# lars-uav/lars-image-processing

Measured on AMD Instinct MI355X. Metric: Mpixels/sec NDVI+stats on 4096x4096 RGNir tiles; achieved HBM GB/s, higher is better.
Workload: dtype f32

## Files before the change

include/lars_hip.h:

```cpp
#ifndef LARS_HIP_H
#define LARS_HIP_H

#include <stddef.h>
#include <stdint.h>

#ifdef __cplusplus
extern "C" {
#endif

#define LARS_ABI_VERSION 1
#define LARS_HIST_BINS 50

typedef enum lars_status {
    LARS_OK = 0,
    LARS_ERR_INVALID = -1,
    LARS_ERR_NO_DEVICE = -2,
    LARS_ERR_HIP = -3,
    LARS_ERR_OOM = -4,
    LARS_ERR_RCCL = -5,
    LARS_ERR_UNSUPPORTED = -6
} lars_status;

#define LARS_U8  1
#define LARS_U16 2

#define LARS_NDVI  0
#define LARS_GNDVI 1
#define LARS_NDWI  2
#define LARS_MASK_NDVI  1u
#define LARS_MASK_GNDVI 2u
#define LARS_MASK_NDWI  4u
#define LARS_MASK_ALL   7u

#define LARS_F_STATS 1u
#define LARS_F_HIST  2u
#define LARS_F_SUMSQ 4u
#define LARS_F_RAW   8u

typedef struct lars_stats {
    double   sum;
    double   sumsq;
    uint64_t count;
    uint64_t above;
    uint64_t nans;
    double   min;
    double   max;
    double   threshold;
    uint32_t index_id;
    uint32_t reserved;
    uint64_t hist[LARS_HIST_BINS];
} lars_stats;

int         lars_abi_version(void);
const char *lars_last_error(void);
int         lars_device_count(int *count);
int         lars_set_device(int ordinal);
int         lars_get_device(int *ordinal);
int         lars_device_name(char *buf, size_t buflen);
int         lars_malloc(void **dptr, size_t bytes);
int         lars_free(void *dptr);
int         lars_memset(void *dptr, int value, size_t bytes, void *stream);
int         lars_memcpy_h2d(void *dst_dev, const void *src_host, size_t bytes);
int         lars_memcpy_d2h(void *dst_host, const void *src_dev, size_t bytes);
int         lars_memcpy_d2d(void *dst_dev, const void *src_dev, size_t bytes, void *stream);
int         lars_stream_create(void **stream);
int         lars_stream_destroy(void *stream);
int         lars_synchronize(void *stream);
int         lars_mem_info(size_t *free_bytes, size_t *total_bytes);
int         lars_shutdown(void);
int         lars_event_create(void **event);
int         lars_event_destroy(void *event);
int         lars_event_record(void *event, void *stream);
int         lars_event_elapsed_ms(void *start, void *stop, float *ms);
int         lars_stream_wait_event(void *stream, void *event);


int lars_d_channel_hist(const void *tiles, int64_t ntiles, int64_t npix, int channels,
                        int dtype, uint32_t *hist, void *stream);

int lars_d_wb_table(const uint32_t *hist, int64_t ntiles, int64_t npix, int dtype,
                    uint8_t *table, double *percentiles, int rgn_variant, void *stream);

size_t lars_wb_table_bytes(int dtype);

int lars_d_wb_prepare(const void *tiles, int64_t ntiles, int64_t npix, int channels, int dtype,
                      uint8_t *table, double *percentiles, int rgn_variant, void *stream);
int lars_u16_window_report(int64_t ntiles, uint32_t *flags, uint32_t *windows);

typedef struct lars_fused_args {
    const void    *tiles;
    int64_t        ntiles;
    int64_t        npix;
    int32_t        channels;
    int32_t        dtype;
    const uint8_t *wb_table;
    uint32_t       index_mask;
    uint32_t       flags;
    float         *out_index[3];
    uint8_t       *out_wb;
    uint8_t       *out_rgba[3];
    const uint8_t *cmap_lut[3];
    lars_stats    *stats;
    void          *stream;
} lars_fused_args;

int lars_d_fused(const lars_fused_args *args);
int lars_d_stats_begin(lars_stats *stats, int64_t ntiles, uint32_t index_mask, void *stream);
int lars_d_stats_end(lars_stats *stats, int64_t ntiles, uint32_t index_mask, int64_t npix, void *stream);

int lars_d_index_planes_f32(const float *red, const float *green, const float *nir,
                            int64_t n, int index_id, float *out, void *stream);

int lars_d_ndvi_f64(const void *img, int64_t npix, int channels, int dtype,
                    double *out, void *stream);

int lars_d_array_stats_f32(const float *x, int64_t n, float threshold, int want_hist,
                           lars_stats *out_dev, void *stream);
int lars_d_array_stats_f64(const double *x, int64_t n, double threshold, int want_hist,
                           lars_stats *out_dev, double *out_sumsqdev_dev, void *stream);

size_t lars_select_scratch_bytes(void);
int lars_d_median_pair_f32(const float *x, int64_t n, float *out_dev, void *scratch, void *stream);
int lars_d_median_pair_f64(const double *x, int64_t n, double *out_dev, void *scratch, void *stream);
int lars_d_median_pair_batch_f32(const float *x, int64_t n, int64_t items, int64_t stride, float *out_dev,
                                 void *scratch, void *stream);

int lars_d_quotient_select_hist(const void *tiles, int64_t ntiles, int64_t npix, int channels, int dtype,
                                const uint8_t *wb_table, uint32_t streams , int first,
                                const uint32_t bucket[4], uint64_t *hist, void *stream);
size_t lars_quotient_median_scratch_bytes(int64_t ntiles);
int lars_d_stats_medians(const lars_fused_args *a, float *out_pairs, void *scratch);
int lars_d_quotient_median_pairs(const void *tiles, int64_t ntiles, int64_t npix, int channels, int dtype,
                                 const uint8_t *wb_table, uint32_t streams ,
                                 float *out_pairs, void *scratch, void *stream);

size_t lars_joint_scratch_bytes(int64_t ntiles, int64_t npix, uint32_t index_mask);
int lars_d_stats_joint(const lars_fused_args *a, int white_balance, int rgn_variant, double *percentiles, uint32_t *hist,
                       float *out_pairs, void *scratch, size_t scratch_bytes);
int lars_joint_window_report(const void *scratch, int64_t ntiles, int64_t *windowed, int64_t *recounted);
int lars_joint_window_modes(const void *scratch, int64_t ntiles, int64_t counts[3]);

int lars_d_threshold_mask_f32(const float *x, int64_t n, float threshold, uint8_t *out_mask, void *stream);

int lars_d_colormap_f32(const float *x, int64_t n, const uint8_t *lut_rgba, uint8_t *out_rgba,
                        void *stream);
int lars_d_colormap_entry_f32(const float *x, int64_t n, uint8_t *out_entry, void *stream);

int lars_d_gray_c128(const uint8_t *img, int64_t npix, int channels, double *out_c128, void *stream);
size_t lars_phase_scratch_bytes(void);
int lars_d_phase_correlation(double *fixed_c128, double *moving_c128, int64_t h, int64_t w, int64_t *shift_dev,
                             void *scratch, void *stream);
int lars_d_shift_reflect_u8(const uint8_t *img, int64_t h, int64_t w, int channels, const int64_t *shift_dev,
                            uint8_t *out, void *stream);
int lars_d_diff_f32(const float *early, const float *late, int64_t n, float *out_diff, void *stream);
int lars_d_colormap_norm_f32(const float *x, int64_t n, float vmin, float vmax, const uint8_t *lut_rgba,
                             uint8_t *out_rgba, void *stream);

int lars_d_synth_u8(uint8_t *tiles, int64_t ntiles, int64_t first_tile, int64_t npix, int channels,
                    uint32_t seed, int profile, void *stream);

int lars_set_tuning(const char *key, int value);
int lars_get_tuning(const char *key, int *value);

#define LARS_BUILD_LAB_LAYOUT 1u
#define LARS_BUILD_IEEE_DIV 2u
#define LARS_BUILD_COUNT_MODE 4u
#define LARS_BUILD_STATS_GEOMETRY 8u
unsigned int lars_build_flags(void);

int lars_d_quot_selfcheck(uint32_t max_den, uint64_t *mismatches, uint32_t first_bad[2]);

int lars_stats_merge(const lars_stats *records, int64_t n, lars_stats *out);
int lars_d_stats_fold(const lars_stats *tile_records, int64_t ntiles, uint32_t index_mask, lars_stats *out, void *stream);


int lars_h_fix_white_balance(const void *img, int64_t h, int64_t w, int channels, int dtype,
                             int variant, uint8_t *out, double *percentiles );
int lars_h_fix_white_balance_f32(const float *img, int64_t h, int64_t w, int channels, uint8_t *out,
                                 double *percentiles );

int lars_h_calculate_index(const void *img, int64_t h, int64_t w, int channels, int dtype,
                           uint32_t index_mask, float *const out[3],
                           lars_stats *stats , int want_hist);

int lars_h_calculate_index_planes(const float *red, const float *green, const float *nir,
                                  int64_t n, int index_id, float *out);

int lars_h_ndvi_f64(const void *img, int64_t h, int64_t w, int channels, int dtype, double *out);

int lars_h_analyze_f32(const float *x, int64_t n, float threshold, int want_hist,
                       lars_stats *out, float median_pair[2]);
int lars_h_analyze_f64(const double *x, int64_t n, double threshold, int want_hist,
                       lars_stats *out, double median_pair[2], double *sumsqdev);

int lars_h_process_image(const void *img, int64_t h, int64_t w, int channels, int dtype,
                         int apply_wb, uint32_t index_mask, int want_hist,
                         uint8_t *out_wb, float *const out_index[3],
                         lars_stats *stats , float *medians ,
                         uint8_t *const out_rgba[3], const uint8_t *const cmap_lut[3]);

int lars_h_colormap_f32(const float *x, int64_t n, const uint8_t *lut_rgba, uint8_t *out_rgba);
int lars_h_threshold_mask_f32(const float *x, int64_t n, float threshold, uint8_t *out_mask);

int lars_h_resize_lanczos_u8(const uint8_t *img, int64_t h, int64_t w, int channels, int64_t new_h, int64_t new_w,
                             uint8_t *out);
int lars_h_thumbnail_u8(const uint8_t *img, int64_t h, int64_t w, int channels, int fx, int fy, const int reduce_box[4],
                        const float box[4], int64_t new_h, int64_t new_w, int vertical_first, uint8_t *out);

int lars_h_align_images(const uint8_t *fixed, const uint8_t *moving, int64_t h, int64_t w, int channels,
                        uint8_t *out_aligned, double shift[2]);
int lars_h_change_detection(const uint8_t *early, const uint8_t *late, int64_t h, int64_t w, int channels,
                            int wb_early, int wb_late, int align, int index_id,
                            float *out_early, float *out_late, float *out_diff,
                            uint8_t *out_rgba_diff, const uint8_t *lut_rgba, float vmin, float vmax,
                            uint8_t *out_aligned_late, double shift[2]);
int lars_h_colormap_norm_f32(const float *x, int64_t n, float vmin, float vmax, const uint8_t *lut_rgba,
                             uint8_t *out_rgba);

size_t lars_png_bound(int64_t h, int64_t w, int channels);
size_t lars_png_scratch_bytes(int64_t h, int64_t w, int channels);
int lars_d_encode_png_u8(const uint8_t *img, int64_t h, int64_t w, int channels, const uint8_t *palette_rgba, int palette_len,
                         uint8_t *out, size_t out_cap, int64_t *out_len_dev, void *scratch, void *stream);
int lars_h_encode_png_u8(const uint8_t *img, int64_t h, int64_t w, int channels, const uint8_t *palette_rgba, int palette_len,
                         uint8_t *out, size_t out_cap, int64_t *out_len);
int lars_h_process_image_png(const void *img, int64_t h, int64_t w, int channels, int dtype,
                             int apply_wb, uint32_t index_mask, int want_hist,
                             uint8_t *out_wb, float *const out_index[3],
                             lars_stats *stats , float *medians ,
                             const uint8_t *const cmap_lut[3], int png_mode,
                             uint8_t *const out_png[3], size_t png_cap, int64_t png_len[3]);

#define LARS_PNG_INFO_N 10
enum {
    LARS_PNG_INFO_WIDTH = 0,
    LARS_PNG_INFO_HEIGHT = 1,
    LARS_PNG_INFO_BIT_DEPTH = 2,
    LARS_PNG_INFO_COLOR_TYPE = 3,
    LARS_PNG_INFO_INTERLACE = 4,
    LARS_PNG_INFO_CHANNELS = 5,
    LARS_PNG_INFO_IDAT_BYTES = 6,
    LARS_PNG_INFO_IDAT_COUNT = 7,
    LARS_PNG_INFO_APNG = 8,
    LARS_PNG_INFO_SUPPORTED = 9
};
enum {
    LARS_PNGD_OK = 0,
    LARS_PNGD_CRC = 1,
    LARS_PNGD_ZLIB_HEADER = 2,
    LARS_PNGD_DEFLATE = 3,
    LARS_PNGD_FAR = 4,
    LARS_PNGD_SHORT = 5,
    LARS_PNGD_ADLER = 6,
    LARS_PNGD_FILTER = 7,
    LARS_PNGD_INTERNAL = 8
};
int lars_png_info(const uint8_t *file, int64_t len, int64_t info[LARS_PNG_INFO_N], int64_t *idat_table, int64_t idat_cap);
size_t lars_png_decode_scratch_bytes(int64_t h, int64_t w, int channels, int64_t idat_bytes, int64_t idat_count);
int lars_d_decode_png_u8(const uint8_t *file, const int64_t *idat_table, int64_t idat_count, int64_t idat_bytes, int64_t h,
                         int64_t w, int channels, uint8_t *out, int32_t *status_dev, void *scratch, void *stream);
int lars_h_decode_png_u8(const uint8_t *file, int64_t len, uint8_t *out, size_t out_cap);
int lars_h_thumbnail_png_u8(const uint8_t *file, int64_t len, int fx, int fy, const int reduce_box[4], const float box[4],
// ... 408 lines not shown
```

lars_image_processing_amd/_ffi.py:

```python
from __future__ import annotations

import contextlib
import ctypes as C
import os
import threading
from typing import NamedTuple

import numpy as np

_HERE = os.path.dirname(os.path.abspath(__file__))
LIB_PATH = os.environ.get("LARS_HIP_LIB", os.path.join(_HERE, "liblars_hip.so"))

HIST_BINS = 50
U8, U16 = 1, 2
NDVI, GNDVI, NDWI = 0, 1, 2
INDEX_IDS = {"NDVI": NDVI, "GNDVI": GNDVI, "NDWI": NDWI}
INDEX_NAMES = ("NDVI", "GNDVI", "NDWI")
F_STATS, F_HIST, F_SUMSQ, F_RAW = 1, 2, 4, 8
COMM_ID_BYTES = 128


class LarsError(RuntimeError):

    def __init__(self, code, message):
        super().__init__(f"liblars_hip error {code}: {message}")
        self.code = code


class Stats(C.Structure):
    _fields_ = [
        ("sum", C.c_double), ("sumsq", C.c_double),
        ("count", C.c_uint64), ("above", C.c_uint64), ("nans", C.c_uint64),
        ("min", C.c_double), ("max", C.c_double), ("threshold", C.c_double),
        ("index_id", C.c_uint32), ("reserved", C.c_uint32),
        ("hist", C.c_uint64 * HIST_BINS),
    ]


STATS_DTYPE = np.dtype([
    ("sum", "<f8"), ("sumsq", "<f8"), ("count", "<u8"), ("above", "<u8"), ("nans", "<u8"),
    ("min", "<f8"), ("max", "<f8"), ("threshold", "<f8"), ("index_id", "<u4"), ("reserved", "<u4"),
    ("hist", "<u8", (HIST_BINS,)),
])
assert STATS_DTYPE.itemsize == C.sizeof(Stats) == 472

REGION_DTYPE = np.dtype([("area", "<i8"), ("bbox", "<i4", (4,)), ("row_sum", "<u8"), ("col_sum", "<u8")])
assert REGION_DTYPE.itemsize == 40

RING_DTYPE = np.dtype([("label", "<i4"), ("key", "<i4"), ("start", "<i4"), ("count", "<i4"), ("area2", "<i8")])
assert RING_DTYPE.itemsize == 24


class Outlines(C.Structure):
    _fields_ = [
        ("rings", C.c_void_p), ("ring_capacity", C.c_int64), ("verts", C.c_void_p), ("vert_capacity", C.c_int64),
        ("n_rings", C.c_int64), ("n_vertices", C.c_int64), ("n_edges", C.c_int64),
    ]


class FusedArgs(C.Structure):
    _fields_ = [
        ("tiles", C.c_void_p), ("ntiles", C.c_int64), ("npix", C.c_int64),
        ("channels", C.c_int32), ("dtype", C.c_int32),
        ("wb_table", C.c_void_p), ("index_mask", C.c_uint32), ("flags", C.c_uint32),
        ("out_index", C.c_void_p * 3), ("out_wb", C.c_void_p),
        ("out_rgba", C.c_void_p * 3), ("cmap_lut", C.c_void_p * 3),
        ("stats", C.c_void_p), ("stream", C.c_void_p),
    ]


class PngInfo(NamedTuple):
    width: int
    height: int
    bit_depth: int
    color_type: int
    interlace: int
    channels: int
    idat_bytes: int
    idat_count: int
    apng: int
    supported: int

    @classmethod
    def array(cls):
        return (C.c_int64 * len(cls._fields))()


class JpegInfo(NamedTuple):
    width: int
    height: int
    components: int
    frame: int
    precision: int
    h0: int
    v0: int
    h1: int
    v1: int
    h2: int
    v2: int
    restart_interval: int
    entropy_offset: int
    entropy_bytes: int
    supported: int
    reason: int

    @classmethod
    def array(cls):
        return (C.c_int64 * len(cls._fields))()

    @property
    def sampling(self):
        return ((self.h0, self.v0), (self.h1, self.v1), (self.h2, self.v2))


class TiffInfo(NamedTuple):
    width: int
    height: int
    samples: int
    bits: int
    compression: int
    predictor: int
    planar: int
    big_endian: int
    photometric: int
    extra_samples: int
    tiled: int
    chunk_w: int
    chunk_h: int
    chunks: int
    supported: int
    reason: int

    @classmethod
    def array(cls):
        return (C.c_int64 * len(cls._fields))()


_P, _I, _I64, _U32, _SZ, _F, _D = C.c_void_p, C.c_int, C.c_int64, C.c_uint32, C.c_size_t, C.c_float, C.c_double
SIGNATURES = {
    "lars_abi_version": (_I, []),
    "lars_last_error": (C.c_char_p, []),
    "lars_device_count": (_I, [C.POINTER(_I)]),
    "lars_set_device": (_I, [_I]),
    "lars_get_device": (_I, [C.POINTER(_I)]),
    "lars_device_name": (_I, [C.c_char_p, _SZ]),
    "lars_malloc": (_I, [C.POINTER(_P), _SZ]),
    "lars_free": (_I, [_P]),
    "lars_memset": (_I, [_P, _I, _SZ, _P]),
    "lars_memcpy_h2d": (_I, [_P, _P, _SZ]),
    "lars_memcpy_d2h": (_I, [_P, _P, _SZ]),
    "lars_memcpy_d2d": (_I, [_P, _P, _SZ, _P]),
    "lars_stream_create": (_I, [C.POINTER(_P)]),
    "lars_stream_destroy": (_I, [_P]),
    "lars_synchronize": (_I, [_P]),
    "lars_shutdown": (_I, []),
    "lars_mem_info": (_I, [C.POINTER(_SZ), C.POINTER(_SZ)]),
    "lars_event_create": (_I, [C.POINTER(_P)]),
    "lars_event_destroy": (_I, [_P]),
    "lars_event_record": (_I, [_P, _P]),
    "lars_event_elapsed_ms": (_I, [_P, _P, C.POINTER(_F)]),
    "lars_stream_wait_event": (_I, [_P, _P]),
    "lars_d_channel_hist": (_I, [_P, _I64, _I64, _I, _I, _P, _P]),
    "lars_d_wb_table": (_I, [_P, _I64, _I64, _I, _P, _P, _I, _P]),
    "lars_wb_table_bytes": (_SZ, [_I]),
    "lars_d_wb_prepare": (_I, [_P, _I64, _I64, _I, _I, _P, _P, _I, _P]),
    "lars_u16_window_report": (_I, [_I64, _P, _P]),
    "lars_d_fused": (_I, [C.POINTER(FusedArgs)]),
    "lars_d_stats_begin": (_I, [_P, _I64, _U32, _P]),
    "lars_d_stats_end": (_I, [_P, _I64, _U32, _I64, _P]),
    "lars_d_index_planes_f32": (_I, [_P, _P, _P, _I64, _I, _P, _P]),
    "lars_d_ndvi_f64": (_I, [_P, _I64, _I, _I, _P, _P]),
    "lars_d_array_stats_f32": (_I, [_P, _I64, _F, _I, _P, _P]),
    "lars_d_array_stats_f64": (_I, [_P, _I64, _D, _I, _P, _P, _P]),
    "lars_select_scratch_bytes": (_SZ, []),
    "lars_d_median_pair_f32": (_I, [_P, _I64, _P, _P, _P]),
    "lars_d_median_pair_f64": (_I, [_P, _I64, _P, _P, _P]),
    "lars_d_median_pair_batch_f32": (_I, [_P, _I64, _I64, _I64, _P, _P, _P]),
    "lars_d_colormap_f32": (_I, [_P, _I64, _P, _P, _P]),
    "lars_d_colormap_entry_f32": (_I, [_P, _I64, _P, _P]),
    "lars_quotient_median_scratch_bytes": (_SZ, [_I64]),
    "lars_d_stats_medians": (_I, [C.POINTER(FusedArgs), _P, _P]),
    "lars_d_quotient_median_pairs": (_I, [_P, _I64, _I64, _I, _I, _P, _U32, _P, _P, _P]),
    "lars_joint_scratch_bytes": (_SZ, [_I64, _I64, _U32]),
    "lars_d_stats_joint": (_I, [C.POINTER(FusedArgs), _I, _I, _P, _P, _P, _P, _SZ]),
    "lars_joint_window_report": (_I, [_P, _I64, C.POINTER(_I64), C.POINTER(_I64)]),
    "lars_joint_window_modes": (_I, [_P, _I64, C.POINTER(_I64)]),
    "lars_h_tiff_lzw_decode": (_I, [_P, _I64, _P, _I64, C.POINTER(_I64)]),
    "lars_h_tiff_lzw_decode_chunks": (_I, [_P, _I64, _P, _P, _I64, _P, _I64, _P, _I]),
    "lars_d_quotient_select_hist": (_I, [_P, _I64, _I64, _I, _I, _P, _U32, _I, _P, _P, _P]),
    "lars_d_synth_u8": (_I, [_P, _I64, _I64, _I64, _I, _U32, _I, _P]),
    "lars_stats_merge": (_I, [_P, _I64, _P]),
    "lars_d_stats_fold": (_I, [_P, _I64, _U32, _P, _P]),
    "lars_build_flags": (C.c_uint, []),
    "lars_set_tuning": (_I, [C.c_char_p, _I]),
    "lars_get_tuning": (_I, [C.c_char_p, C.POINTER(_I)]),
    "lars_d_quot_selfcheck": (_I, [_U32, C.POINTER(C.c_uint64), C.POINTER(_U32 * 2)]),
    "lars_h_fix_white_balance": (_I, [_P, _I64, _I64, _I, _I, _I, _P, _P]),
    "lars_h_fix_white_balance_f32": (_I, [_P, _I64, _I64, _I, _P, _P]),
    "lars_h_calculate_index": (_I, [_P, _I64, _I64, _I, _I, _U32, C.POINTER(_P * 3), _P, _I]),
    "lars_h_calculate_index_planes": (_I, [_P, _P, _P, _I64, _I, _P]),
    "lars_h_ndvi_f64": (_I, [_P, _I64, _I64, _I, _I, _P]),
    "lars_h_analyze_f32": (_I, [_P, _I64, _F, _I, _P, _P]),
    "lars_h_analyze_f64": (_I, [_P, _I64, _D, _I, _P, _P, _P]),
    "lars_h_process_image": (_I, [_P, _I64, _I64, _I, _I, _I, _U32, _I, _P, C.POINTER(_P * 3), _P, _P,
                                  C.POINTER(_P * 3), C.POINTER(_P * 3)]),
    "lars_h_colormap_f32": (_I, [_P, _I64, _P, _P]),
    "lars_h_threshold_mask_f32": (_I, [_P, _I64, _F, _P]),
    "lars_d_threshold_mask_f32": (_I, [_P, _I64, _F, _P, _P]),
    "lars_h_colormap_norm_f32": (_I, [_P, _I64, _F, _F, _P, _P]),
    "lars_h_align_images": (_I, [_P, _P, _I64, _I64, _I, _P, _P]),
    "lars_h_change_detection": (_I, [_P, _P, _I64, _I64, _I, _I, _I, _I, _I, _P, _P, _P, _P, _P, _F, _F, _P, _P]),
    "lars_d_gray_c128": (_I, [_P, _I64, _I, _P, _P]),
    "lars_phase_scratch_bytes": (_SZ, []),
    "lars_d_phase_correlation": (_I, [_P, _P, _I64, _I64, _P, _P, _P]),
    "lars_d_shift_reflect_u8": (_I, [_P, _I64, _I64, _I, _P, _P, _P]),
    "lars_d_diff_f32": (_I, [_P, _P, _I64, _P, _P]),
    "lars_d_colormap_norm_f32": (_I, [_P, _I64, _F, _F, _P, _P, _P]),
    "lars_h_resize_lanczos_u8": (_I, [_P, _I64, _I64, _I, _I64, _I64, _P]),
    "lars_h_thumbnail_u8": (_I, [_P, _I64, _I64, _I, _I, _I, C.POINTER(_I), C.POINTER(_F), _I64, _I64, _I, _P]),
    "lars_png_bound": (_SZ, [_I64, _I64, _I]),
    "lars_png_scratch_bytes": (_SZ, [_I64, _I64, _I]),
    "lars_d_encode_png_u8": (_I, [_P, _I64, _I64, _I, _P, _I, _P, _SZ, _P, _P, _P]),
    "lars_h_encode_png_u8": (_I, [_P, _I64, _I64, _I, _P, _I, _P, _SZ, C.POINTER(_I64)]),
    "lars_h_process_image_png": (_I, [_P, _I64, _I64, _I, _I, _I, _U32, _I, _P, C.POINTER(_P * 3), _P, _P,
                                      C.POINTER(_P * 3), _I, C.POINTER(_P * 3), _SZ, _P]),
    "lars_png_info": (_I, [_P, _I64, _P, _P, _I64]),
    "lars_png_decode_scratch_bytes": (_SZ, [_I64, _I64, _I, _I64, _I64]),
    "lars_d_decode_png_u8": (_I, [_P, _P, _I64, _I64, _I64, _I64, _I, _P, _P, _P, _P]),
    "lars_h_decode_png_u8": (_I, [_P, _I64, _P, _SZ]),
    "lars_h_thumbnail_png_u8": (_I, [_P, _I64, _I, _I, C.POINTER(_I), C.POINTER(_F), _I64, _I64, _I, _P]),
    "lars_png_out_format": (_I, [_I, _I, C.POINTER(_I), C.POINTER(_I)]),
    "lars_png_layout": (_I, [_I64, _I64, _I, _I, _I, _P, C.POINTER(_I64), C.POINTER(_I64)]),
    "lars_png_decode_ex_scratch_bytes": (_SZ, [_I64, _I64, _I, _I, _I, _I64, _I64]),
    "lars_d_decode_png_ex": (_I, [_P, _P, _I64, _I64, _I64, _I64, _I, _I, _I, _P, _P, _P, _P]),
    "lars_h_decode_png_ex": (_I, [_P, _I64, _P, _SZ]),
    "lars_h_thumbnail_png_ex": (_I, [_P, _I64, _I, _I, C.POINTER(_I), C.POINTER(_F), _I64, _I64, _I, _P]),
    "lars_jpeg_info": (_I, [_P, _I64, _P]),
    "lars_jpeg_decode_scratch_bytes": (_SZ, [_P]),
    "lars_d_decode_jpeg_u8": (_I, [_P, _P, _P, _P, _P, _P, _P]),
    "lars_h_decode_jpeg_u8": (_I, [_P, _I64, _P, _SZ]),
    "lars_h_thumbnail_jpeg_u8": (_I, [_P, _I64, _I, _I, C.POINTER(_I), C.POINTER(_F), _I64, _I64, _I, _P]),
    "lars_jpeg_decode_scaled_scratch_bytes": (_SZ, [_P, _I]),
    "lars_d_decode_jpeg_scaled_u8": (_I, [_P, _P, _P, _I, _P, _P, _P, _P]),
    "lars_h_decode_jpeg_scaled_u8": (_I, [_P, _I64, _I, _P, _SZ]),
    "lars_h_thumbnail_jpeg_scaled_u8": (_I, [_P, _I64, _I, _I, _I, C.POINTER(_I), C.POINTER(_F), _I64, _I64, _I, _P]),
    "lars_tiff_info": (_I, [_P, _I64, _P, _P, _I64]),
    "lars_h_decode_tiff": (_I, [_P, _I64, _P, _SZ]),
    "lars_h_thumbnail_tiff_u8": (_I, [_P, _I64, _I, _I, C.POINTER(_I), C.POINTER(_F), _I64, _I64, _I, _P]),
    "lars_tiff_info_deflate": (_I, [_P, _I64, _P, _P, _I64]),
    "lars_h_decode_tiff_deflate": (_I, [_P, _I64, _P, _SZ]),
    "lars_h_thumbnail_tiff_deflate_u8": (_I, [_P, _I64, _I, _I, C.POINTER(_I), C.POINTER(_F), _I64, _I64, _I, _P]),
    "lars_tiff_bound": (_SZ, [_I64, _I64, _I, _I, _I64]),
    "lars_tiff_encode_scratch_bytes": (_SZ, [_I64, _I64, _I, _I, _I64]),
    "lars_d_encode_tiff": (_I, [_P, _I64, _I64, _I, _I, _I64, _I, _P, _SZ, _P, _P, _P, _P]),
    "lars_h_encode_tiff": (_I, [_P, _I64, _I64, _I, _I, _I64, _I, _P, _SZ, C.POINTER(_I64)]),
    "lars_tiff_f32_bound": (_SZ, [_I64, _I64, _I, _I64]),
    "lars_tiff_f32_encode_scratch_bytes": (_SZ, [_I64, _I64, _I, _I64]),
    "lars_d_encode_tiff_f32": (_I, [_P, _I64, _I64, _I, _I64, _I, _P, _SZ, _P, _P, _P, _P]),
    "lars_h_encode_tiff_f32": (_I, [_P, _I64, _I64, _I, _I64, _I, _P, _SZ, C.POINTER(_I64)]),
    "lars_h_process_image_tiff_f32": (_I, [_P, _I64, _I64, _I, _I, _I, _U32, _I, _P, C.POINTER(_P * 3), _P, _P,
                                           C.POINTER(_P * 3), C.POINTER(_P * 3), _I, _I64, C.POINTER(_P * 3), _SZ, _P]),
    "lars_tiff_deflate_bound": (_SZ, [_I64, _I64, _I, _I, _I64]),
    "lars_tiff_deflate_encode_scratch_bytes": (_SZ, [_I64, _I64, _I, _I, _I64]),
    "lars_d_encode_tiff_deflate": (_I, [_P, _I64, _I64, _I, _I, _I64, _I, _P, _SZ, _P, _P, _P, _P]),
    "lars_h_encode_tiff_deflate": (_I, [_P, _I64, _I64, _I, _I, _I64, _I, _P, _SZ, C.POINTER(_I64)]),
    "lars_tiff_float32_deflate_bound": (_SZ, [_I64, _I64, _I, _I64]),
    "lars_tiff_float32_deflate_encode_scratch_bytes": (_SZ, [_I64, _I64, _I, _I64]),
    "lars_d_encode_tiff_deflate_float32": (_I, [_P, _I64, _I64, _I, _I64, _I, _P, _SZ, _P, _P, _P, _P]),
    "lars_h_encode_tiff_deflate_float32": (_I, [_P, _I64, _I64, _I, _I64, _I, _P, _SZ, C.POINTER(_I64)]),
    "lars_h_process_image_tiff_float32": (_I, [_P, _I64, _I64, _I, _I, _I, _U32, _I, _P, C.POINTER(_P * 3), _P, _P,
                                                       C.POINTER(_P * 3), C.POINTER(_P * 3), _I, _I, _I64, C.POINTER(_P * 3), _SZ, _P]),
    "lars_d_valid_mask": (_I, [_P, _I64, _I, _I, _P, _I, _I, _I, _P, _P, _P]),
    "lars_d_masked_channel_hist": (_I, [_P, _I64, _I, _I, _P, _P, _P]),
    "lars_d_masked_fused": (_I, [C.POINTER(FusedArgs), _P, C.POINTER(_P * 3), _P]),
    "lars_h_valid_mask": (_I, [_P, _I64, _I64, _I, _I, _I, _I, _I, _P, C.POINTER(_I64)]),
    "lars_h_process_image_masked": (_I, [_P, _I64, _I64, _I, _I, _I, _U32, _I, _P, C.POINTER(_P * 3), _P, _P,
                                         C.POINTER(_P * 3), C.POINTER(_P * 3), _P, _I, _I, _I, C.POINTER(_I64),
                                         _I, _I, _I64, C.POINTER(_P * 3), _SZ, _P]),
    "lars_d_zone_count": (_I, [_P, _I, _P, _I64, _I64, _P, _P, _P]),
    "lars_d_zone_offsets": (_I, [_P, _I64, _P, _P, _P]),
    "lars_d_zone_scatter": (_I, [C.POINTER(_P * 3), _U32, _P, _I, _P, _I64, _I64, _P, _P, C.POINTER(_P * 3), _P]),
    "lars_d_zone_stats": (_I, [_P, _P, _P, _I64, _F, _I, _I64, _P, _P, _P]),
    "lars_h_zonal_stats_f32": (_I, [_P, _P, _I, _P, _I64, _I64, _I64, _F, _I, _P, _P, C.POINTER(_I64)]),
    "lars_h_process_image_zones": (_I, [_P, _I64, _I64, _I, _I, _I, _U32, _I, _P, C.POINTER(_P * 3), _P, _P,
                                        C.POINTER(_P * 3), C.POINTER(_P * 3), _P, _I, _I, _I, C.POINTER(_I64),
                                        _P, _I, _I64, _P, _P, C.POINTER(_I64)]),
    "lars_zone_rasterize_scratch_bytes": (_SZ, [_I64]),
    "lars_d_zone_rasterize": (_I, [_P, _I64, _P, _I64, _P, _I64, _I64, _I64, _P, _P, _P]),
    "lars_d_zone_labels_narrow": (_I, [_P, _I64, _I, _P, _P]),
    "lars_h_rasterize_zones": (_I, [_P, _I64, _P, _I64, _P, _I64, _I64, _I64, _I, _P]),
    "lars_h_zonal_stats_polygons_f32": (_I, [_P, _P, _I64, _P, _I64, _P, _I64, _P, _I64, _I64, _F, _I, _P, _P, _P, _I]),
    "lars_h_process_image_zones_polygons": (_I, [_P, _I64, _I64, _I, _I, _I, _U32, _I, _P, C.POINTER(_P * 3), _P, _P,
                                                 C.POINTER(_P * 3), C.POINTER(_P * 3), _P, _I, _I, _I, C.POINTER(_I64),
                                                 _P, _I64, _P, _I64, _P, _I64, _P, _P, _P, _I]),
    "lars_region_label_scratch_bytes": (_SZ, [_I64, _I64]),
    "lars_d_region_label": (_I, [_P, _I64, _I64, _I, _I64, _P, _P, _I64, _P, _P, _P]),
    "lars_d_region_mask_f32": (_I, [_P, _P, _P, _I64, _F, _I, _P, _P]),
    "lars_h_label_regions": (_I, [_P, _I64, _I64, _I, _I64, _I, _P, C.POINTER(_I), _P, _I64, C.POINTER(_I64)]),
    "lars_h_zonal_stats_regions_f32": (_I, [_P, _P, _I, _F, _I, _I64, _P, _I64, _I64, _F, _I, _I64, _P, _P, _P, C.POINTER(_I64), _P, _I,
                                            C.POINTER(_I)]),
    "lars_h_process_image_regions": (_I, [_P, _I64, _I64, _I, _I, _I, _U32, _I, _P, C.POINTER(_P * 3), _P, _P,
                                          C.POINTER(_P * 3), C.POINTER(_P * 3), _P, _I, _I, _I, C.POINTER(_I64),
                                          _P, _I, _I, _F, _I, _I64, _I64, _P, _P, _P, C.POINTER(_I64), _P, _I, C.POINTER(_I)]),
    "lars_region_outline_scratch_bytes": (_SZ, [_I64, _I64, _I64]),
    "lars_d_region_outline_count": (_I, [_P, _I64, _I64, _P, _P]),
    "lars_d_region_outline": (_I, [_P, _I64, _I64, _I, _I64, _I64, _P, _I64, _P, _I64, _P, _P, _P]),
    "lars_h_region_outlines": (_I, [_P, _I64, _I64, _I, _I64, _I, _P, C.POINTER(_I), _P, _I64, C.POINTER(_I64), C.POINTER(Outlines)]),
    "lars_h_zonal_stats_regions_outlines_f32": (_I, [_P, _P, _I, _F, _I, _I64, _P, _I64, _I64, _F, _I, _I64, _P, _P, _P, C.POINTER(_I64), _P, _I,
                                                     C.POINTER(_I), C.POINTER(Outlines)]),
    "lars_h_process_image_regions_outlines": (_I, [_P, _I64, _I64, _I, _I, _I, _U32, _I, _P, C.POINTER(_P * 3), _P, _P,
                                                   C.POINTER(_P * 3), C.POINTER(_P * 3), _P, _I, _I, _I, C.POINTER(_I64),
                                                   _P, _I, _I, _F, _I, _I64, _I64, _P, _P, _P, C.POINTER(_I64), _P, _I, C.POINTER(_I),
                                                   C.POINTER(Outlines)]),
    "lars_d_zone_shrink": (_I, [_P, _I, _I64, _I64, _I64, _P, _P, _P]),
    "lars_h_shrink_zones": (_I, [_P, _I, _I64, _I64, _I64, _I64, _P, C.POINTER(_I64)]),
    "lars_h_rasterize_zones_margin": (_I, [_P, _I64, _P, _I64, _P, _I64, _I64, _I64, _I, _P, _I64]),
    "lars_h_zonal_stats_margin_f32": (_I, [_P, _P, _I, _P, _I64, _I64, _I64, _F, _I, _P, _P, C.POINTER(_I64), _I64]),
    "lars_h_zonal_stats_polygons_margin_f32": (_I, [_P, _P, _I64, _P, _I64, _P, _I64, _P, _I64, _I64, _F, _I, _P, _P, _P, _I, _I64]),
    "lars_h_zonal_stats_regions_margin_f32": (_I, [_P, _P, _I, _F, _I, _I64, _P, _I64, _I64, _F, _I, _I64, _P, _P, _P, C.POINTER(_I64), _P, _I,
                                                   C.POINTER(_I), _I64]),
    "lars_h_process_image_zones_margin": (_I, [_P, _I64, _I64, _I, _I, _I, _U32, _I, _P, C.POINTER(_P * 3), _P, _P,
                                               C.POINTER(_P * 3), C.POINTER(_P * 3), _P, _I, _I, _I, C.POINTER(_I64),
# ... 183 lines not shown
```

lars_image_processing_amd/batch.py:

```python
from __future__ import annotations

import ctypes as C
import os

import numpy as np

from . import _ffi
from . import arena as _arena
from ._ffi import FusedArgs, INDEX_IDS, INDEX_NAMES, STATS_DTYPE, DeviceBuffer, DeviceSlice
from .arena import arena_placements

MAX_TILES_PER_LAUNCH = 65535


_STATS_ROUTE = os.environ.get("LARS_STATS_ROUTE", "auto")


def set_stats_route(route):
    global _STATS_ROUTE
    if route not in ("auto", "joint", "classic"):
        raise ValueError("route must be auto, joint or classic")
    _STATS_ROUTE = route


def get_stats_route():
    return _STATS_ROUTE


def index_mask(indices):
    mask = 0
    for t in indices:
        mask |= 1 << INDEX_IDS[t]
    return mask


def joint_serves(code, channels, ntiles, npix):
    return code == _ffi.U8 and channels in (3, 4) and (ntiles == 1 or npix % 4 == 0)


def plan_process(code, channels, ntiles, npix, indices, white_balance, hist, medians, sumsq, route,
                 outputs=False, wb_plane=False, reuse=False):
    if route not in ("auto", "joint", "classic"):
        raise ValueError(f"route must be auto, joint or classic, not {route!r}")
    if reuse and not outputs and route == "joint":
        raise ValueError("route='joint' derives the tables from its own counts: it cannot honour recompute_tables=False")
    one_read = route != "classic" and not reuse and joint_serves(code, channels, ntiles, npix) and bool(indices)
    if one_read and not outputs:
        return "measure" if route == "auto" and not medians and not sumsq else "one-read"
    if route == "joint" and not outputs:
        raise ValueError("route='joint' serves uint8 tiles with 3 or 4 channels (4-byte aligned) only")
    if one_read and not wb_plane and (medians or hist or select_streams(indices) in (1, 2)):
        return "one-read+planes"
    if medians and code == _ffi.U8 and channels == 3 and npix * 6 < (1 << 30) and (ntiles == 1 or npix % 4 == 0):
        return "select" if not outputs and index_mask(indices) in (1, 2, 4, 7) else "per-pixel+select"
    return "per-pixel+radix" if medians else "per-pixel"


def channels_of(indices, whole_image=False):
    if whole_image:
        return {0, 1, 2}
    need = set()
    for t in indices:
        need |= {2, 0} if t == "NDVI" else {2, 1}
    return need


def shard_range(ntiles, rank, world):
    base, rem = divmod(int(ntiles), int(world))
    start = rank * base + min(rank, rem)
    return start, start + base + (1 if rank < rem else 0)


class TileBatch:

    def __init__(self, ntiles, h, w, channels=3, dtype=np.uint8, first_tile=0):
        self.ntiles, self.h, self.w, self.channels = int(ntiles), int(h), int(w), int(channels)
        self.dtype = np.dtype(dtype)
        self.code = _ffi.dtype_code(self.dtype)
        if self.code is None:
            raise TypeError("tiles must be uint8 or uint16")
        if self.ntiles < 1 or self.ntiles > MAX_TILES_PER_LAUNCH:
            raise ValueError(f"1 <= ntiles <= {MAX_TILES_PER_LAUNCH} per batch")
        self.first_tile = int(first_tile)
        self.npix = self.h * self.w
        self.nvalues = 256 if self.code == _ffi.U8 else 65536
        self.table_bytes = int(_ffi.load().lars_wb_table_bytes(self.code))
        self.tile_bytes = self.npix * self.channels * self.dtype.itemsize
        self.tiles = DeviceBuffer(self.ntiles * self.tile_bytes)
        self.hist = None
        self.table = None
        self.percentiles = None
        self._table_channels = set()
        self._hist_channels = set()
        self._rgn_variant = 0
        self._joint_scratch = None
        self._joint_tiles = self.ntiles
        self._selq = None
        self.last_route = None

    @classmethod
    def from_host(cls, array, first_tile=0):
        arr = np.ascontiguousarray(array)
        if arr.ndim != 4 or arr.shape[3] < 3:
            raise ValueError("expected [ntiles, H, W, C>=3]")
        b = cls(arr.shape[0], arr.shape[1], arr.shape[2], arr.shape[3], arr.dtype, first_tile)
        b.tiles.upload(arr)
        return b

    @classmethod
    def synthetic(cls, ntiles, h, w, seed=1234, profile="uniform", first_tile=0, channels=3):
        b = cls(ntiles, h, w, channels, np.uint8, first_tile)
        _ffi.call("lars_d_synth_u8", C.c_void_p(b.tiles.ptr), b.ntiles, b.first_tile, b.npix, b.channels,
                  int(seed) & 0xFFFFFFFF, {"uniform": 0, "vegetation": 1}[profile], None)
        _ffi.call("lars_synchronize", None)
        return b

    def host_tiles(self, start=0, count=None):
        count = self.ntiles - start if count is None else count
        return self.tiles.download(self.dtype, (count, self.h, self.w, self.channels), start * self.tile_bytes)

    def compute_wb_tables(self, stream=None, rgn_variant=0):
        if self.table is None:
            self.table = DeviceBuffer(self.ntiles * self.table_bytes)
            self.percentiles = DeviceBuffer(self.ntiles * 3 * 2 * 8)
        if self.code == _ffi.U8:
            if self.hist is None:
                self.hist = DeviceBuffer(self.ntiles * 3 * 256 * 4)
            _ffi.call("lars_d_channel_hist", C.c_void_p(self.tiles.ptr), self.ntiles, self.npix, self.channels,
                      self.code, C.c_void_p(self.hist.ptr), stream)
            _ffi.call("lars_d_wb_table", C.c_void_p(self.hist.ptr), self.ntiles, self.npix, self.code,
                      C.c_void_p(self.table.ptr), C.c_void_p(self.percentiles.ptr), int(rgn_variant), stream)
        else:
            _ffi.call("lars_d_wb_prepare", C.c_void_p(self.tiles.ptr), self.ntiles, self.npix, self.channels,
                      self.code, C.c_void_p(self.table.ptr), C.c_void_p(self.percentiles.ptr), int(rgn_variant), stream)
        self._table_channels = {0, 1, 2}
        self._hist_channels = {0, 1, 2} if self.code == _ffi.U8 else set()
        self._rgn_variant = int(rgn_variant)
        return self

    def u16_window_report(self):
        if self.code != _ffi.U16:
            raise _ffi.LarsError(-1, "lars_u16_window_report: a uint8 batch's pre-pass does not take the value-window route")
        flags = np.zeros(self.ntiles, np.uint32)
        windows = np.zeros((self.ntiles, 3, 4), np.uint32)
        _ffi.call("lars_u16_window_report", self.ntiles, _ffi.ptr(flags), _ffi.ptr(windows))
        return flags, windows

    def _need_channels(self, partial):
        if self.table is None:
            raise RuntimeError("compute_wb_tables() first")
        if not partial and self._table_channels != {0, 1, 2}:
            missing = sorted({0, 1, 2} - self._table_channels)
            raise RuntimeError(f"white-balance tables of channel(s) {missing} are not valid: the last pass computed only the "
                               f"channels its indices read (compute_wb_tables() for all three, or partial=True)")

    def host_tables(self, partial=False):
        self._need_channels(partial)
        blob = self.table.download(np.uint8, (self.ntiles, self.table_bytes))
        return np.ascontiguousarray(blob[:, :3 * self.nvalues]).reshape(self.ntiles, 3, self.nvalues)

    def host_percentiles(self, partial=False):
        self._need_channels(partial)
        return self.percentiles.download(np.float64, (self.ntiles, 3, 2))

    def host_hist(self, partial=False):
        self._need_channels(partial)
        if self.hist is None or (not partial and self._hist_channels != {0, 1, 2}):
            missing = sorted({0, 1, 2} - self._hist_channels)
            raise RuntimeError(f"channel histograms of channel(s) {missing} are not valid: the last one-read pass was not asked for them "
                               f"(compute_wb_tables(), or run_joint(..., channel_hist=True); partial=True hands out what there is)")
        return self.hist.download(np.uint32, (self.ntiles, 3, 256))

    def make_outputs(self, indices=INDEX_NAMES, index=False, wb=False, rgba=False, ring=None, placement_trials=None, arena="auto",
                     pick="fastest"):
        outs = BatchOutputs(self, indices, index, wb, rgba, ring, allocate=False)
        nplanes = len(outs._index_ids) + len(outs._rgba_ids)
        plan = _arena.plan_arena(nplanes, outs.plane_bytes, outs.slots * self.npix * 4, arena, placement_trials, pick)
        if plan.kind != "search":
            if plan.kind == "packed":
                outs.adopt_arena(DeviceBuffer(nplanes * outs.plane_bytes))
            outs.arena_report = _arena.unsearched_report(plan)
            return outs

        def free_bytes():
            free_b, total_b = C.c_size_t(), C.c_size_t()
            _ffi.call("lars_mem_info", C.byref(free_b), C.byref(total_b))
            return free_b.value

        stats = self.new_stats()
        try:
            found = _arena.search(outs, plan, pick, alloc=DeviceBuffer, free_bytes=free_bytes,
                                  probe=lambda placement, warm_ms: self._probe_arena(outs, indices, stats, warm_ms),
                                  synchronize=lambda: _ffi.call("lars_synchronize", None))
        finally:
            stats.free()
        outs.placement_ms, outs.arena_report = _arena.report(found)
        return outs

    def _probe_arena(self, outs, indices, stats, warm_ms=_arena.ARENA_WARM_MS):
        count = min(outs.slots, self.ntiles)
        starts = list(range(0, self.ntiles, count))
        if len(starts) > 16:
            starts = [starts[int(round(i * (len(starts) - 1) / 15.0))] for i in range(16)]
        mask = index_mask(indices)
        wb_on = self.table is not None
        launches = [self.fused_args(indices, wb_on, stats, False, outs, None, st, min(count, self.ntiles - st), raw=True) for st in starts]
        while len(launches) < 4:
            launches = launches + launches
        ev = [C.c_void_p(), C.c_void_p()]
        for e in ev:
            _ffi.call("lars_event_create", C.byref(e))
        ms = C.c_float(0)

        def one_pass():
            _ffi.call("lars_event_record", ev[0], None)
            for a in launches:
                self.run_fused(a)
            _ffi.call("lars_event_record", ev[1], None)
            _ffi.call("lars_event_elapsed_ms", ev[0], ev[1], C.byref(ms))
            return float(ms.value)

        try:
            _ffi.call("lars_d_stats_begin", C.c_void_p(stats.ptr), self.ntiles, mask, None)
            warmed, passes = 0.0, 0
            while warmed < warm_ms and passes < 8:
                warmed += one_pass()
                passes += 1
            timed = one_pass()
            _ffi.call("lars_d_stats_end", C.c_void_p(stats.ptr), self.ntiles, mask, self.npix, None)
            _ffi.call("lars_synchronize", None)
        finally:
            for e in ev:
                _ffi.call("lars_event_destroy", e)
        return timed / len(launches)

    def fused_args(self, indices=INDEX_NAMES, white_balance=True, stats=None, hist=False, outputs=None,
                   stream=None, tile_start=0, tile_count=None, sumsq=False, raw=False):
        tile_count = self.ntiles - tile_start if tile_count is None else tile_count
        a = FusedArgs()
        a.tiles = self.tiles.ptr + tile_start * self.tile_bytes
        a.ntiles, a.npix, a.channels, a.dtype = tile_count, self.npix, self.channels, self.code
        if white_balance:
            if self.table is None:
                raise RuntimeError("compute_wb_tables() first")
            a.wb_table = self.table.ptr + tile_start * self.table_bytes
        a.index_mask = index_mask(indices)
        a.flags = ((_ffi.F_STATS if stats is not None else 0) | (_ffi.F_HIST if (stats is not None and hist) else 0) |
                   (_ffi.F_SUMSQ if (stats is not None and sumsq) else 0) | (_ffi.F_RAW if (stats is not None and raw) else 0))
        if stats is not None:
            a.stats = stats.ptr + tile_start * 3 * STATS_DTYPE.itemsize
        if outputs is not None:
            slot = tile_start % outputs.slots
            if slot + tile_count > outputs.slots:
                raise ValueError("tile range wraps the output ring")
            for k in range(3):
                if outputs.index[k] is not None:
                    a.out_index[k] = outputs.index[k].ptr + slot * self.npix * 4
                if outputs.rgba[k] is not None:
                    a.out_rgba[k] = outputs.rgba[k].ptr + slot * self.npix * 4
                    a.cmap_lut[k] = outputs.luts[k].ptr
            if outputs.wb is not None:
                a.out_wb = outputs.wb.ptr + slot * self.npix * self.channels
        a.stream = stream
        return a

    def new_stats(self):
        return DeviceBuffer(self.ntiles * 3 * STATS_DTYPE.itemsize)

    def fold_stats(self, stats, indices=INDEX_NAMES, out=None, stream=None):
        if out is None:
            out = DeviceBuffer(3 * STATS_DTYPE.itemsize)
            out.zero(stream)
        _ffi.call("lars_d_stats_fold", C.c_void_p(stats.ptr), self.ntiles, index_mask(indices), C.c_void_p(out.ptr), stream)
        return out

    def run_fused_chunks(self, indices, white_balance, stats, hist, outputs, stream=None, sumsq=False, launch_events=None):
        chunk = self.ntiles if outputs is None else outputs.slots
        if chunk >= self.ntiles:
            if launch_events:
                _ffi.call("lars_event_record", launch_events[0], stream)
            self.run_fused(self.fused_args(indices, white_balance, stats, hist, outputs, stream, sumsq=sumsq))
            if launch_events and len(launch_events) > 1:
                _ffi.call("lars_event_record", launch_events[1], stream)
            return 1
        mask = index_mask(indices)
        if stats is not None:
            _ffi.call("lars_d_stats_begin", C.c_void_p(stats.ptr), self.ntiles, mask, stream)
        launches = 0
        if launch_events:
            _ffi.call("lars_event_record", launch_events[0], stream)
        for start in range(0, self.ntiles, chunk):
            count = min(chunk, self.ntiles - start)
            self.run_fused(self.fused_args(indices, white_balance, stats, hist, outputs, stream, start, count, sumsq=sumsq,
                                           raw=stats is not None))
            launches += 1
            if launch_events and launches < len(launch_events):
                _ffi.call("lars_event_record", launch_events[launches], stream)
        if stats is not None:
            _ffi.call("lars_d_stats_end", C.c_void_p(stats.ptr), self.ntiles, mask, self.npix, stream)
        return launches

    def run_fused(self, args):
        _ffi.call("lars_d_fused", C.byref(args))

    def can_joint(self):
        return joint_serves(self.code, self.channels, self.ntiles, self.npix)

    def run_joint(self, indices, white_balance, stats, hist=False, sumsq=False, pairs=None, stream=None, rgn_variant=0,
                  tile_count=None, channel_hist=False):
        mask = index_mask(indices)
        need = int(_ffi.load().lars_joint_scratch_bytes(self.ntiles, self.npix, mask))
        if self._joint_scratch is None or self._joint_scratch.nbytes < need:
            if self._joint_scratch is not None:
                _ffi.call("lars_synchronize", stream)
                self._joint_scratch.free()
            self._joint_scratch = DeviceBuffer(need)
        if white_balance:
            if self.table is None:
                self.table = DeviceBuffer(self.ntiles * self.table_bytes)
                self.percentiles = DeviceBuffer(self.ntiles * 3 * 2 * 8)
                self.table.zero(stream)
                self.percentiles.zero(stream)
            if channel_hist and self.hist is None:
                self.hist = DeviceBuffer(self.ntiles * 3 * 256 * 4)
                self.hist.zero(stream)
                self._hist_channels = set()
            if tile_count is None or int(tile_count) == self.ntiles:
                keep = self._table_channels if int(rgn_variant) == self._rgn_variant else set()
                self._table_channels = keep | channels_of(indices)
                self._rgn_variant = int(rgn_variant)
                if channel_hist:
                    self._hist_channels = self._hist_channels | channels_of(indices)
            else:
                self._table_channels = set()
                self._hist_channels = set()
        a = FusedArgs()
        a.tiles = self.tiles.ptr
        a.ntiles, a.npix, a.channels, a.dtype = (self.ntiles if tile_count is None else int(tile_count)), self.npix, self.channels, self.code
        a.wb_table = self.table.ptr if white_balance else None
        a.index_mask = mask
        a.flags = _ffi.F_STATS | (_ffi.F_HIST if hist else 0) | (_ffi.F_SUMSQ if sumsq else 0)
        a.stats = stats.ptr
        a.stream = stream
        self._joint_tiles = int(a.ntiles)
        _ffi.call("lars_d_stats_joint", C.byref(a), 1 if white_balance else 0, int(rgn_variant),
                  C.c_void_p(self.percentiles.ptr) if white_balance else None,
                  C.c_void_p(self.hist.ptr) if white_balance and channel_hist else None,
                  C.c_void_p(pairs.ptr) if pairs is not None else None, C.c_void_p(self._joint_scratch.ptr), self._joint_scratch.nbytes)

    def joint_window_report(self):
        w, r = C.c_int64(0), C.c_int64(0)
        if self._joint_scratch is None:
            return 0, 0
        _ffi.call("lars_joint_window_report", C.c_void_p(self._joint_scratch.ptr), self._joint_tiles, C.byref(w), C.byref(r))
        return int(w.value), int(r.value)

    def joint_window_modes(self):
        if self._joint_scratch is None:
            return 0, 0, 0
        counts = (C.c_int64 * 3)()
        _ffi.call("lars_joint_window_modes", C.c_void_p(self._joint_scratch.ptr), self._joint_tiles, counts)
        return int(counts[0]), int(counts[1]), int(counts[2])

    def check_joint(self, stream=None):
        _ffi.call("lars_synchronize", stream)
        if self._joint_scratch is not None and int(self._joint_scratch.download(np.uint32, (1,))[0]):
            raise RuntimeError("lars_d_stats_joint: a workgroup's hand-over list overflowed (a chunk of more than 2^24 pixels?)")

    def pick_stats_route(self, indices, white_balance=True, sample=256, min_pixels=1 << 29):
        key = (tuple(sorted(INDEX_IDS[t] for t in indices)), bool(white_balance))
        cache = self.__dict__.setdefault("_route_cache", {})
        if key in cache:
            return cache[key]
        sample = min(int(sample), self.ntiles)
        if sample * self.npix < int(min_pixels) or self.channels != 3:
            cache[key] = "joint"
            return "joint"
        saved = (self.table, self.percentiles, self.hist, set(self._table_channels), self._rgn_variant, set(self._hist_channels))
        self.table = self.percentiles = self.hist = None
        self._table_channels = set()
        self._hist_channels = set()
        ev = [C.c_void_p() for _ in range(3)]
        for e in ev:
            _ffi.call("lars_event_create", C.byref(e))
        stats = self.new_stats()
        ms = {}
        try:
            for _ in range(2):
                _ffi.call("lars_event_record", ev[0], None)
                self.run_joint(indices, white_balance, stats, tile_count=sample)
                _ffi.call("lars_event_record", ev[1], None)
                if white_balance:
                    if self.hist is None:
                        self.hist = DeviceBuffer(self.ntiles * 3 * 256 * 4)
                    _ffi.call("lars_d_channel_hist", C.c_void_p(self.tiles.ptr), sample, self.npix, self.channels, self.code,
                              C.c_void_p(self.hist.ptr), None)
                    _ffi.call("lars_d_wb_table", C.c_void_p(self.hist.ptr), sample, self.npix, self.code, C.c_void_p(self.table.ptr),
                              C.c_void_p(self.percentiles.ptr), 0, None)
                self.run_fused(self.fused_args(indices, white_balance, stats, False, None, None, 0, sample))
                _ffi.call("lars_event_record", ev[2], None)
                t = C.c_float(0)
                _ffi.call("lars_event_elapsed_ms", ev[0], ev[1], C.byref(t)); ms["joint"] = t.value
                _ffi.call("lars_event_elapsed_ms", ev[1], ev[2], C.byref(t)); ms["classic"] = t.value
            self.check_joint()
        finally:
            _ffi.call("lars_synchronize", None)
            for e in ev:
                _ffi.call("lars_event_destroy", e)
            stats.free()
            for buf in (self.table, self.percentiles, self.hist):
                if buf is not None:
                    buf.free()
            self.table, self.percentiles, self.hist, self._table_channels, self._rgn_variant, self._hist_channels = saved
        cache[key] = "joint" if ms["joint"] <= ms["classic"] else "classic"
        self._route_ms = dict(ms)
        return cache[key]

    def process(self, indices=INDEX_NAMES, white_balance=True, hist=False, outputs=None, stream=None,
                recompute_tables=True, medians=False, sumsq=False, route=None, rgn_variant=None, channel_hist=False):
        route = _STATS_ROUTE if route is None else route
        variant = 0 if rgn_variant is None else int(rgn_variant)
        wb_plane = outputs is not None and outputs.wb is not None
        reuse = (white_balance and not recompute_tables and self.table is not None
                 and channels_of(indices, wb_plane) <= self._table_channels and (rgn_variant is None or variant == self._rgn_variant))

        def plan(r):
            return plan_process(self.code, self.channels, self.ntiles, self.npix, indices, white_balance, hist, medians, sumsq, r,
                                outputs is not None, wb_plane, reuse)

        taken = plan(route)
        if taken == "measure":
            taken = plan(self.pick_stats_route(indices, white_balance))
        self.last_route = taken
        if taken in ("one-read", "one-read+planes"):
            return self._run_one_read(indices, white_balance, hist, sumsq, medians, outputs, stream, variant, channel_hist)
        if white_balance and not reuse:
            self.compute_wb_tables(stream, rgn_variant=variant)
        stats = self.new_stats()
        stats.zero(stream)
        run = {"select": self._run_select, "per-pixel+select": self._run_fused_select, "per-pixel": self._run_fused,
               "per-pixel+radix": self._run_fused_radix}[taken]
        return run(indices, white_balance, stats, hist, sumsq, outputs, stream)

    def _records(self, stats):
        rec = stats.download(STATS_DTYPE, (self.ntiles, 3))
        stats.free()
        return rec

    def _run_one_read(self, indices, white_balance, hist, sumsq, medians, outputs, stream, variant, channel_hist):
        stats = self.new_stats()
        stats.zero(stream)
        pairs = DeviceBuffer(self.ntiles * 4 * 4) if medians else None
        self.run_joint(indices, white_balance, stats, hist, sumsq, pairs, stream, rgn_variant=variant, channel_hist=channel_hist)
        if outputs is not None:
            self.run_fused_chunks(indices, white_balance, None, False, outputs, stream)
        self.check_joint(stream)
        rec = self._records(stats)
        if not medians:
            return rec
        med = self._medians_from_pairs(pairs.download(np.float32, (self.ntiles, 2, 2)), indices)
        pairs.free()
        return rec, med

    def _run_select(self, indices, white_balance, stats, hist, sumsq, outputs, stream):
        args = self.fused_args(indices, white_balance, stats, hist, None, stream, sumsq=sumsq)
        med = self._per_tile_select(indices, stream, lambda pairs, scratch: _ffi.call("lars_d_stats_medians", C.byref(args), pairs, scratch))
        return self._records(stats), med

    def _run_fused_select(self, indices, white_balance, stats, hist, sumsq, outputs, stream):
        self.run_fused_chunks(indices, white_balance, stats, hist, outputs, stream, sumsq)
        med = self.tile_medians(indices, white_balance, stream)
        return self._records(stats), med

    def _run_fused(self, indices, white_balance, stats, hist, sumsq, outputs, stream):
        self.run_fused_chunks(indices, white_balance, stats, hist, outputs, stream, sumsq)
        _ffi.call("lars_synchronize", stream)
        return self._records(stats)

    def _run_fused_radix(self, indices, white_balance, stats, hist, sumsq, outputs, stream):
        own_outputs = None
        if outputs is None or any(outputs.index[INDEX_IDS[t]] is None for t in indices):
            own_outputs = outputs = self.make_outputs(indices=indices, index=True, ring=min(self.ntiles, 16), arena="plain")
        pairs = DeviceBuffer(self.ntiles * 3 * 2 * 4)
        pairs.zero(stream)
        sel = DeviceBuffer(outputs.slots * int(_ffi.load().lars_select_scratch_bytes()))
        for start in range(0, self.ntiles, outputs.slots):
            count = min(outputs.slots, self.ntiles - start)
            self.run_fused(self.fused_args(indices, white_balance, stats, hist, outputs, stream, start, count, sumsq=sumsq))
            for t in indices:
                k = INDEX_IDS[t]
                _ffi.call("lars_d_median_pair_batch_f32", C.c_void_p(outputs.index[k].ptr), self.npix, count, self.npix,
                          C.c_void_p(pairs.ptr + (k * self.ntiles + start) * 8), C.c_void_p(sel.ptr), stream)
        _ffi.call("lars_synchronize", stream)
        rec = self._records(stats)
        med = pair_medians(pairs.download(np.float32, (3, self.ntiles, 2)), indices, per_index=True)
        pairs.free()
        sel.free()
        if own_outputs is not None:
            own_outputs.free()
        return rec, med

    def free(self):
        for b in (self.tiles, self.hist, self.table, self.percentiles, self._joint_scratch, self._selq):
            if b is not None:
                b.free()

    def tile_medians(self, indices=INDEX_NAMES, white_balance=True, stream=None):
        if white_balance and (self.table is None or not channels_of(indices) <= self._table_channels):
            raise RuntimeError("compute_wb_tables() first")
        return self._per_tile_select(indices, stream, lambda pairs, scratch: _ffi.call(
            "lars_d_quotient_median_pairs", C.c_void_p(self.tiles.ptr), self.ntiles, self.npix, self.channels, self.code,
            C.c_void_p(self.table.ptr) if white_balance else None, select_streams(indices), pairs, scratch, stream))

    def _per_tile_select(self, indices, stream, launch):
        pairs = DeviceBuffer(self.ntiles * 4 * 4)
        scratch = DeviceBuffer(int(_ffi.load().lars_quotient_median_scratch_bytes(self.ntiles)))
        launch(C.c_void_p(pairs.ptr), C.c_void_p(scratch.ptr))
        _ffi.call("lars_synchronize", stream)
        med = self._medians_from_pairs(pairs.download(np.float32, (self.ntiles, 2, 2)), indices)
        pairs.free()
        scratch.free()
        return med

    def _medians_from_pairs(self, pairs, indices):
        med = pair_medians(pairs, indices)
        if any(np.isnan(med[:, INDEX_IDS[t]]).any() for t in indices):
            raise RuntimeError("exact median select did not settle (values outside the uint8 quotient domain?)")
        return med

    def select_histogram(self, first, buckets, white_balance=True, stream=None, streams=3):
        if self.code != _ffi.U8 or self.channels != 3:
            raise TypeError("exact batch medians need uint8 tiles with 3 channels")
        if white_balance and self.table is None:
            raise RuntimeError("compute_wb_tables() first")
        if self._selq is None:
            self._selq = DeviceBuffer(2 * 2 * SELECT_BINS * 8)
        self._selq.zero(stream)
        b = np.ascontiguousarray(np.asarray(buckets, dtype=np.int64) & 0xFFFFFFFF, dtype=np.uint32).reshape(4)
        _ffi.call("lars_d_quotient_select_hist", C.c_void_p(self.tiles.ptr), self.ntiles, self.npix, self.channels, self.code,
                  C.c_void_p(self.table.ptr) if white_balance else None, int(streams), int(first), _ffi.ptr(b),
                  C.c_void_p(self._selq.ptr), stream)
        _ffi.call("lars_synchronize", stream)
        return self._selq.download(np.uint64, (2, 2, SELECT_BINS))

    def global_medians(self, indices=INDEX_NAMES, white_balance=True, comm=None, recompute_tables=False):
        if white_balance and (recompute_tables or self.table is None or not channels_of(indices) <= self._table_channels):
            self.compute_wb_tables()
        n_local = self.ntiles * self.npix
        streams = select_streams(indices)
        values = select_order_statistics(lambda first, buckets: self.select_histogram(first, buckets, white_balance, None, streams),
                                         n_local, comm, streams)
        return medians_from_pairs(values, indices)


class BatchOutputs:

    def __init__(self, batch, indices, index, wb, rgba, ring=None, allocate=True):
        from .api import colormap_lut, _colormap_for
        self.slots = batch.ntiles if not ring else min(int(ring), batch.ntiles)
        self.index, self.rgba, self.luts = [None] * 3, [None] * 3, [None] * 3
        self.batch = batch
        self.plane_bytes = (self.slots * batch.npix * 4 + 255) & ~255
        self._index_ids = sorted(INDEX_IDS[t] for t in indices) if index else []
        self._rgba_ids = sorted(INDEX_IDS[t] for t in indices) if rgba else []
        self.arena = None
        self.arena2 = None
        self.arena_report = None
        if allocate and (self._index_ids or self._rgba_ids):
            self.adopt_arena(DeviceBuffer((len(self._index_ids) + len(self._rgba_ids)) * self.plane_bytes))
        for t in indices:
            k = INDEX_IDS[t]
            if rgba:
                self.luts[k] = DeviceBuffer(1024)
                self.luts[k].upload(colormap_lut(_colormap_for(t)))
        self.wb = DeviceBuffer(self.slots * batch.npix * batch.channels) if wb else None

    def adopt(self, buffers, placement):
        placement = tuple((int(i), int(o)) for i, o in placement)
        assert len(placement) == len(self._index_ids) + len(self._rgba_ids)
        used = list(dict.fromkeys(i for i, _ in placement))
        assert len(used) <= 2
        for i in used:
            inside = sorted(o for a, o in placement if a == i)
            assert all(o % 256 == 0 and o + self.plane_bytes <= buffers[i].nbytes for o in inside)
            assert all(b - a >= self.plane_bytes for a, b in zip(inside, inside[1:])), "planes overlap"
        self.arena = buffers[used[0]] if used else None
        self.arena2 = buffers[used[1]] if len(used) > 1 else None
        self.plane_offsets = tuple(o for _, o in placement)
        slices = [DeviceSlice(buffers[i], o, self.plane_bytes) for i, o in placement]
        for j, k in enumerate(self._index_ids):
            self.index[k] = slices[j]
        for j, k in enumerate(self._rgba_ids):
            self.rgba[k] = slices[len(self._index_ids) + j]

    def adopt_arena(self, arena, offsets=None):
        if offsets is None:
            offsets = _arena.packed(len(self._index_ids) + len(self._rgba_ids), self.plane_bytes)
        self.adopt([arena], [(0, o) for o in offsets])

    def adopt_two_arenas(self, arena, offsets, arena2, offsets2):
        self.adopt([arena, arena2], [(0, o) for o in offsets] + [(1, o) for o in offsets2])

    def forget_planes(self):
        self.index, self.rgba, self.arena, self.arena2 = [None] * 3, [None] * 3, None, None

    def host_index(self, index_type, slot=0, count=1):
        k = INDEX_IDS[index_type]
        b = self.batch
        return self.index[k].download(np.float32, (count, b.h, b.w), slot * b.npix * 4)

    def host_rgba(self, index_type, slot=0, count=1):
        k = INDEX_IDS[index_type]
        b = self.batch
        return self.rgba[k].download(np.uint8, (count, b.h, b.w, 4), slot * b.npix * 4)

    def host_wb(self, slot=0, count=1):
        b = self.batch
        return self.wb.download(np.uint8, (count, b.h, b.w, b.channels), slot * b.npix * b.channels)

    def free(self):
        for b in self.index + self.rgba + self.luts + [self.wb, self.arena, self.arena2]:
            if b is not None:
                b.free()
        self.forget_planes()


def merge_records(records):
    rec = np.ascontiguousarray(records, dtype=STATS_DTYPE).reshape(-1)
    out = np.zeros(1, dtype=STATS_DTYPE)
    _ffi.call("lars_stats_merge", _ffi.ptr(rec), rec.size, _ffi.ptr(out))
    return out[0]


def summarize(record):
    count = int(record["count"])
    mean = float(record["sum"]) / count
    sumsq = float(record["sumsq"])
    have_sq = sumsq != 0.0 or (float(record["min"]) == 0.0 and float(record["max"]) == 0.0)
    var = max(sumsq / count - mean * mean, 0.0)
    return {
        "count": count,
        "mean": mean,
        "std": var ** 0.5 if have_sq else None,
        "min": float(record["min"]),
        "max": float(record["max"]),
        "coverage": int(record["above"]) / count * 100.0,
        "hist": np.array(record["hist"], dtype=np.int64),
    }


def local_fold(tile_records, indices=INDEX_NAMES):
    out = np.zeros(3, dtype=STATS_DTYPE)
    for t in indices:
        k = INDEX_IDS[t]
        out[k] = merge_records(tile_records[:, k])
    return out


def timeseries_rows(records, medians, index_type, dates=None):
    k = INDEX_IDS[index_type]
    feature = "Water" if index_type == "NDWI" else "Vegetation"
    rows = []
    for i in range(records.shape[0]):
        r = records[i, k]
        count = int(r["count"])
        rows.append({
            "Date": None if dates is None else dates[i],
            "Mean": float(r["sum"]) / count,
            "Median": float(medians[i, k]),
            "Min": float(r["min"]),
            "Max": float(r["max"]),
            f"{feature} Coverage (%)": int(r["above"]) / count * 100,
        })
    return rows


SELECT_BINS = 2048
SELECT_SLOTS = 1024
MAX_BYTE_SUM = 510


def select_position(x):
    t = (np.asarray(x, dtype=np.float32).astype(np.float64) * 1023.5 + 3071.5).astype(np.float32)
    m = np.ascontiguousarray(t).view(np.uint32) - np.uint32(0x45000000)
    return (m >> np.uint32(12)).astype(np.int64), ((m & np.uint32(0xFFF)) >> np.uint32(2)).astype(np.int64)


# ... 135 lines not shown
```

lars_image_processing_amd/csrc/common.h:

```cpp
#pragma once
#include <hip/hip_runtime.h>
#include <stdint.h>
#include <stdio.h>
#include <string>

#include "host_common.h"

namespace lars {


#define LARS_HIP_TRY(expr)                                                          \
    do {                                                                            \
        hipError_t _e = (expr);                                                     \
        if (_e != hipSuccess)                                                       \
            return ::lars::fail(_e == hipErrorOutOfMemory ? LARS_ERR_OOM : LARS_ERR_HIP, \
                                "%s failed: %s (%s:%d)", #expr, hipGetErrorString(_e), \
                                __FILE__, __LINE__);                                \
    } while (0)

struct ThreadCtx {
    int device = -1;
    hipStream_t stream = nullptr;
    void *ws = nullptr;
    size_t ws_bytes = 0;
    void *scratch = nullptr;
    size_t scratch_bytes = 0;
    void *outline = nullptr;
    size_t outline_bytes = 0;
    int64_t u16_win_tiles = 0;
};

int ensure_ctx(ThreadCtx **out);
int ws_reserve(ThreadCtx *c, size_t bytes);
int scratch_reserve(ThreadCtx *c, size_t bytes);
int outline_reserve(ThreadCtx *c, size_t bytes);

struct Carver {
    char *base;
    size_t off = 0;
    explicit Carver(void *b) : base(static_cast<char *>(b)) {}
    template <typename T>
    T *take(size_t count)
    {
        off = (off + 255) & ~(size_t)255;
        T *p = base ? reinterpret_cast<T *>(base + off) : nullptr;
        off += count * sizeof(T);
        return p;
    }
    size_t bytes() const { return (off + 255) & ~(size_t)255; }
};

template <typename Plan>
int ws_plan(ThreadCtx *c, Plan &&plan)
{
    Carver size(nullptr);
    plan(size);
    LARS_TRY(ws_reserve(c, size.bytes() + 256));
    Carver cv(c->ws);
    plan(cv);
    return LARS_OK;
}
inline hipStream_t pick_stream(ThreadCtx *c, void *stream) {
    return stream ? reinterpret_cast<hipStream_t>(stream) : c->stream;
}

#define LARS_FX_SCALE 4294967296.0
#define LARS_FX_INV (1.0 / 4294967296.0)

struct StatsAccView {
    unsigned long long sum_fx;
    unsigned long long sumsq_fx;
    unsigned long long count;
    unsigned long long above;
    unsigned long long nans;
    unsigned long long min_key;
    unsigned long long max_key;
    double threshold;
    unsigned int index_id;
    unsigned int reserved;
    unsigned long long hist[LARS_HIST_BINS];
};
static_assert(sizeof(StatsAccView) == sizeof(lars_stats), "accumulator view must alias lars_stats");

__host__ __device__ inline unsigned int f32_key(float x) {
    unsigned int b = __builtin_bit_cast(unsigned int, x);
    return (b & 0x80000000u) ? ~b : (b | 0x80000000u);
}
__host__ __device__ inline float key_f32(unsigned int k) {
    unsigned int b = (k & 0x80000000u) ? (k & 0x7FFFFFFFu) : ~k;
    return __builtin_bit_cast(float, b);
}
__host__ __device__ inline unsigned long long f64_key(double x) {
    unsigned long long b = __builtin_bit_cast(unsigned long long, x);
    return (b >> 63) ? ~b : (b | 0x8000000000000000ull);
}
__host__ __device__ inline double key_f64(unsigned long long k) {
    unsigned long long b = (k >> 63) ? (k & 0x7FFFFFFFFFFFFFFFull) : ~k;
    return __builtin_bit_cast(double, b);
}

__host__ __device__ inline double hist_edge_f64(int i) {
    return i >= LARS_HIST_BINS ? 1.0 : (double)i * (2.0 / 50.0) + (-1.0);
}

#define LARS_U16_THR_OFFSET 196608
#define LARS_U16_PAR_OFFSET (196608 + 3 * 260 * 4)
#define LARS_U16_BLOB_BYTES (196608 + 4096)

int launch_check(const char *what);
void align_release();

struct Tuning {
    int fused_impl = 0;
    int hist_impl = 2;
    int nt_stores = 0;
    int blocks_per_tile = 0;
    int load_policy = 0;
    int selq_window = 1;
    int selq_list_wgs = 0;
    int last_fused_kernel = 0;
    int u16_hist_impl = 5;
    int out_stride_planes = 0;
    int joint_depth = 6;
    int joint_win_depth = 15;
    int jpeg_subseq_bits = 512;
    int jpeg_last_rounds = 0;
    int tiff_strip_bytes = 65536;
    int deflate_matching = 0;
    int joint_window = 1;
    int zone_split_pixels = 131072;
};
Tuning &tuning();
inline bool stream_loads_nt(bool kernel_default_nt)
{
    const int k = tuning().load_policy;
    return k == 0 ? kernel_default_nt : k == 2;
}

struct FusedParams;
#ifndef LARS_V2_STATS_THREADS
#define LARS_V2_STATS_THREADS 1024
#endif
#ifndef LARS_V2_STATS_WAVES
#define LARS_V2_STATS_WAVES 8
#endif
int fused_v2_threads(bool any_out);
void fused_v2_launch(unsigned mask, bool wb, int stats, bool nt, dim3 grid, hipStream_t s, const FusedParams &P);
void chan_hist_v2_launch(const uint8_t *tiles, long long npix, unsigned int *hist, dim3 grid, hipStream_t s, int channels = 3);
int selq_pass_launch(const uint8_t *tiles, const uint8_t *wb_table, long long ntiles, long long npix, int first,
                     const unsigned int bucket[4], unsigned long long *hist, hipStream_t s, unsigned streams);
size_t selq_tile_scratch_bytes(long long ntiles);
int selq_tile_medians_launch(const uint8_t *tiles, const uint8_t *wb_table, long long ntiles, long long npix, float *out_pairs,
                             void *scratch, hipStream_t s, bool first_pass_done, unsigned streams, bool windowed = false);
int selq_tile_prepare(void *scratch, long long ntiles, long long npix, hipStream_t s, unsigned int streams);
unsigned int *selq_tile_hist32(void *scratch, long long ntiles);
void fused_v2_sel_launch(unsigned mask, bool wb, int stats, dim3 grid, hipStream_t s, const FusedParams &P);
int blocks_per_tile(long long work_items, long long ntiles, int threads = 256, long long target_total = 8192);
void stats_init_launch(lars_stats *stats, long long nrec, unsigned int mask, hipStream_t s);
void stats_finalize_launch(lars_stats *stats, long long nrec, unsigned int mask, long long npix, hipStream_t s);
int quot_check_launch(unsigned int max_den, unsigned long long *mismatches_dev, unsigned int *first_bad_dev, hipStream_t s);

}
```

lars_image_processing_amd/csrc/fused.hip:

```cpp
#include <string.h>

#include "common.h"
#include "device_common.h"
#include "fused_device.h"
#include "wg_device.h"

namespace lars {

__global__ __launch_bounds__(256) void k_chan_hist_u8c3(const uint8_t *__restrict__ tiles,
                                                        long long npix, unsigned int *__restrict__ hist)
{
    __shared__ unsigned int s_h[4][3 * 256];
    const int tid = threadIdx.x;
    const int wave = tid >> 6;
    for (int i = tid; i < 4 * 768; i += 256) (&s_h[0][0])[i] = 0;
    __syncthreads();

    const long long tile = blockIdx.y;
    const uint8_t *base = tiles + tile * npix * 3;
    const long long nquads = npix >> 2;
    unsigned int *h = s_h[wave];
    for (long long q = (long long)blockIdx.x * 256 + tid; q < nquads; q += (long long)gridDim.x * 256) {
        const unsigned int *p = reinterpret_cast<const unsigned int *>(base + q * 12);
        unsigned int w0 = p[0], w1 = p[1], w2 = p[2];
        atomicAdd(&h[0 * 256 + (w0 & 0xFF)], 1u);
        atomicAdd(&h[1 * 256 + ((w0 >> 8) & 0xFF)], 1u);
        atomicAdd(&h[2 * 256 + ((w0 >> 16) & 0xFF)], 1u);
        atomicAdd(&h[0 * 256 + (w0 >> 24)], 1u);
        atomicAdd(&h[1 * 256 + (w1 & 0xFF)], 1u);
        atomicAdd(&h[2 * 256 + ((w1 >> 8) & 0xFF)], 1u);
        atomicAdd(&h[0 * 256 + ((w1 >> 16) & 0xFF)], 1u);
        atomicAdd(&h[1 * 256 + (w1 >> 24)], 1u);
        atomicAdd(&h[2 * 256 + (w2 & 0xFF)], 1u);
        atomicAdd(&h[0 * 256 + ((w2 >> 8) & 0xFF)], 1u);
        atomicAdd(&h[1 * 256 + ((w2 >> 16) & 0xFF)], 1u);
        atomicAdd(&h[2 * 256 + (w2 >> 24)], 1u);
    }
    if (blockIdx.x == 0 && tid < (int)(npix & 3)) {
        const uint8_t *p = base + (nquads * 4 + tid) * 3;
        atomicAdd(&h[p[0]], 1u);
        atomicAdd(&h[256 + p[1]], 1u);
        atomicAdd(&h[512 + p[2]], 1u);
    }
    __syncthreads();
    unsigned int *gh = hist + tile * 768;
    for (int i = tid; i < 768; i += 256) {
        unsigned int v = s_h[0][i] + s_h[1][i] + s_h[2][i] + s_h[3][i];
        if (v) atomicAdd(&gh[i], v);
    }
}

template <typename PIX, int NVAL>
__global__ __launch_bounds__(256) void k_chan_hist_generic(const PIX *__restrict__ tiles, long long npix,
                                                           int channels, unsigned int *__restrict__ hist)
{
    const long long tile = blockIdx.y;
    const PIX *base = tiles + tile * npix * channels;
    unsigned int *gh = hist + tile * 3 * (long long)NVAL;
    if (NVAL == 256) {
        __shared__ unsigned int s_h[3 * 256];
        for (int i = threadIdx.x; i < 768; i += 256) s_h[i] = 0;
        __syncthreads();
        for (long long i = (long long)blockIdx.x * 256 + threadIdx.x; i < npix; i += (long long)gridDim.x * 256) {
            const PIX *p = base + i * channels;
            atomicAdd(&s_h[(unsigned)p[0]], 1u);
            atomicAdd(&s_h[256 + (unsigned)p[1]], 1u);
            atomicAdd(&s_h[512 + (unsigned)p[2]], 1u);
        }
        __syncthreads();
        for (int i = threadIdx.x; i < 768; i += 256)
            if (s_h[i]) atomicAdd(&gh[i], s_h[i]);
    } else {
        for (long long i = (long long)blockIdx.x * 256 + threadIdx.x; i < npix; i += (long long)gridDim.x * 256) {
            const PIX *p = base + i * channels;
            atomicAdd(&gh[(unsigned)p[0]], 1u);
            atomicAdd(&gh[NVAL + (unsigned)p[1]], 1u);
            atomicAdd(&gh[2 * NVAL + (unsigned)p[2]], 1u);
        }
    }
}

template <int NVAL>
__global__ __launch_bounds__(256) void k_wb_table(const unsigned int *__restrict__ hist, long long npix,
                                                  uint8_t *__restrict__ table, double *__restrict__ pcts,
                                                  int rgn_variant)
{
    constexpr int PER = NVAL / 256;
    __shared__ unsigned long long s_scan[4];
    __shared__ double s_val[4];
    __shared__ double s_p[2];
    __shared__ unsigned int s_thr[NVAL == 256 ? 4 : 260];

    const int tid = threadIdx.x;
    const long long slot = (long long)blockIdx.y * 3 + blockIdx.x;
    const unsigned int *h = hist + slot * NVAL;

    unsigned long long local = 0;
    for (int j = 0; j < PER; ++j) local += h[tid * PER + j];
    const unsigned long long before = wg_exscan<256>(local, s_scan);

    const double nm1 = (double)(npix - 1);
    double tq[2];
    long long rank[4];
    for (int k = 0; k < 2; ++k) {
        const double q = (k == 0 ? 2.0 : 98.0) / 100.0;
        const double vi = nm1 * q;
        const double fl = floor(vi);
        long long lo = (long long)fl;
        long long hi = lo + 1;
        if (hi > npix - 1) hi = npix - 1;
        rank[2 * k] = lo;
        rank[2 * k + 1] = hi;
        tq[k] = vi - fl;
    }
    unsigned long long cum = before;
    for (int j = 0; j < PER; ++j) {
        const unsigned long long c = h[tid * PER + j];
        if (c) {
            for (int r = 0; r < 4; ++r)
                if ((unsigned long long)rank[r] >= cum && (unsigned long long)rank[r] < cum + c)
                    s_val[r] = (double)(tid * PER + j);
        }
        cum += c;
    }
    __syncthreads();
    if (tid < 2) {
        const double a = s_val[2 * tid], b = s_val[2 * tid + 1], t = tq[tid];
        const double d = b - a;
        double r = a + d * t;
        if (t >= 0.5) r = b - d * (1.0 - t);
        s_p[tid] = r;
        if (pcts) pcts[slot * 2 + tid] = r;
    }
    __syncthreads();
    const double p_lo = s_p[0], p_hi = s_p[1];
    if (NVAL == 256) {
        uint8_t *out = table + slot * 256;
        out[tid] = (uint8_t)wb_level(tid, p_lo, p_hi, rgn_variant);
    } else {
        u16_fill_blob(table + (long long)blockIdx.y * LARS_U16_BLOB_BYTES, (int)blockIdx.x, p_lo, p_hi, rgn_variant, s_thr, tid);
    }
}

__global__ void k_stats_init(lars_stats *stats, long long nrec, unsigned int mask)
{
    const long long i = (long long)blockIdx.x * blockDim.x + threadIdx.x;
    if (i >= nrec) return;
    const int k = (int)(i % 3);
    if (!((mask >> k) & 1u)) return;
    StatsAccView *a = reinterpret_cast<StatsAccView *>(stats + i);
    a->sum_fx = 0; a->sumsq_fx = 0; a->count = 0; a->above = 0; a->nans = 0;
    a->min_key = ~0ull; a->max_key = 0ull;
    a->threshold = (k == LARS_NDWI) ? 0.0 : (double)0.2f;
    a->index_id = (unsigned)k; a->reserved = 0;
    for (int b = 0; b < LARS_HIST_BINS; ++b) a->hist[b] = 0;
}

__global__ void k_stats_finalize(lars_stats *stats, long long nrec, unsigned int mask, long long npix)
{
    const long long i = (long long)blockIdx.x * blockDim.x + threadIdx.x;
    if (i >= nrec) return;
    const int k = (int)(i % 3);
    if (!((mask >> k) & 1u)) return;
    StatsAccView *a = reinterpret_cast<StatsAccView *>(stats + i);
    const long long s = (long long)a->sum_fx, s2 = (long long)a->sumsq_fx;
    const unsigned long long mnk = a->min_key, mxk = a->max_key;
    lars_stats *o = stats + i;
    o->sum = (double)s * LARS_FX_INV;
    o->sumsq = (double)s2 * LARS_FX_INV;
    o->count = (uint64_t)npix;
    o->min = key_f64(mnk);
    o->max = key_f64(mxk);
}

__global__ __launch_bounds__(256) void k_stats_fold(const lars_stats *__restrict__ rec, long long ntiles, unsigned int mask,
                                                    lars_stats *__restrict__ out)
{
    const int k = blockIdx.x;
    if (!((mask >> k) & 1u)) return;
    __shared__ double s_sum[256], s_sq[256];
    __shared__ double s_mn[4], s_mx[4];
    __shared__ unsigned long long s_cnt[4][3];
    const int tid = threadIdx.x;
    double sum = 0.0, sq = 0.0;
    double mn = __builtin_inf(), mx = -__builtin_inf();
    unsigned long long cnt = 0, above = 0, nans = 0;
    __shared__ unsigned long long s_hist[LARS_HIST_BINS];
    if (tid < LARS_HIST_BINS) s_hist[tid] = 0ull;
    __syncthreads();
    for (long long t = tid; t < ntiles; t += 256) {
        const unsigned long long *h = reinterpret_cast<const unsigned long long *>(rec[t * 3 + k].hist);
        unsigned long long v[LARS_HIST_BINS];
#pragma unroll
        for (int b = 0; b < LARS_HIST_BINS; ++b) v[b] = h[b];
#pragma unroll
        for (int b = 0; b < LARS_HIST_BINS; ++b)
            if (v[b]) atomicAdd(&s_hist[b], v[b]);
    }
    for (long long base = 0; base < ntiles; base += 256) {
        const long long t = base + tid;
        if (t < ntiles) {
            const lars_stats *r = rec + t * 3 + k;
            s_sum[tid] = r->sum; s_sq[tid] = r->sumsq;
            cnt += r->count; above += r->above; nans += r->nans;
            mn = fmin(mn, r->min); mx = fmax(mx, r->max);
        }
        __syncthreads();
        const int n = (int)(ntiles - base < 256 ? ntiles - base : 256);
        if (tid == 0) {
            int i = 0;
            if (base == 0) { sum = s_sum[0]; sq = s_sq[0]; i = 1; }
            for (; i < n && (i & 7); ++i) { sum += s_sum[i]; sq += s_sq[i]; }
            for (; i + 8 <= n; i += 8) {
                double a[8], b[8];
#pragma unroll
                for (int j = 0; j < 8; ++j) { a[j] = s_sum[i + j]; b[j] = s_sq[i + j]; }
#pragma unroll
                for (int j = 0; j < 8; ++j) { sum += a[j]; sq += b[j]; }
            }
            for (; i < n; ++i) { sum += s_sum[i]; sq += s_sq[i]; }
        }
        __syncthreads();
    }
    for (int off = 32; off >= 1; off >>= 1) {
        cnt += __shfl_xor(cnt, off); above += __shfl_xor(above, off); nans += __shfl_xor(nans, off);
        mn = fmin(mn, __shfl_xor(mn, off)); mx = fmax(mx, __shfl_xor(mx, off));
    }
    if ((tid & 63) == 0) {
        const int w = tid >> 6;
        s_cnt[w][0] = cnt; s_cnt[w][1] = above; s_cnt[w][2] = nans; s_mn[w] = mn; s_mx[w] = mx;
    }
    __syncthreads();
    lars_stats *o = out + k;
    if (tid == 0) {
        o->sum = sum; o->sumsq = sq;
        o->count = s_cnt[0][0] + s_cnt[1][0] + s_cnt[2][0] + s_cnt[3][0];
        o->above = s_cnt[0][1] + s_cnt[1][1] + s_cnt[2][1] + s_cnt[3][1];
        o->nans = s_cnt[0][2] + s_cnt[1][2] + s_cnt[2][2] + s_cnt[3][2];
        o->min = fmin(fmin(s_mn[0], s_mn[1]), fmin(s_mn[2], s_mn[3]));
        o->max = fmax(fmax(s_mx[0], s_mx[1]), fmax(s_mx[2], s_mx[3]));
        o->threshold = rec[k].threshold; o->index_id = rec[k].index_id; o->reserved = rec[k].reserved;
    }
    if (tid < LARS_HIST_BINS) o->hist[tid] = s_hist[tid];
}

__device__ inline void acc_flush(Acc a, StatsAccView *rec, double (*s_red)[4], int tid)
{
    for (int off = 32; off >= 1; off >>= 1) {
        a.mn = fminf(a.mn, __shfl_xor(a.mn, off));
        a.mx = fmaxf(a.mx, __shfl_xor(a.mx, off));
        a.sum += __shfl_xor(a.sum, off);
        a.sumsq += __shfl_xor(a.sumsq, off);
        a.above += __shfl_xor(a.above, off);
    }
    const int wave = tid >> 6, lane = tid & 63;
    __syncthreads();
    if (lane == 0) {
        s_red[0][wave] = a.sum;
        s_red[1][wave] = a.sumsq;
        s_red[2][wave] = (double)a.above;
        s_red[3][wave] = __builtin_bit_cast(double, ((unsigned long long)f32_key(a.mx) << 32) | f32_key(a.mn));
    }
    __syncthreads();
    if (tid == 0) {
        double sum = 0, sumsq = 0, above = 0;
        unsigned int mnk = 0xFFFFFFFFu, mxk = 0;
        for (int w = 0; w < 4; ++w) {
            sum += s_red[0][w];
            sumsq += s_red[1][w];
            above += s_red[2][w];
            const unsigned long long kk = __builtin_bit_cast(unsigned long long, s_red[3][w]);
            const unsigned int kmn = (unsigned int)kk, kmx = (unsigned int)(kk >> 32);
            mnk = kmn < mnk ? kmn : mnk;
            mxk = kmx > mxk ? kmx : mxk;
        }
        atomicAdd(&rec->sum_fx, (unsigned long long)__double2ll_rn(sum * LARS_FX_SCALE));
        atomicAdd(&rec->sumsq_fx, (unsigned long long)__double2ll_rn(sumsq * LARS_FX_SCALE));
        atomicAdd(&rec->above, (unsigned long long)above);
        atomicMin(&rec->min_key, f64_key((double)key_f32(mnk)));
        atomicMax(&rec->max_key, f64_key((double)key_f32(mxk)));
    }
}


template <typename PIX, unsigned MASK, bool WB, int STATS, int CH = 3, int POLICY = LOAD_PLAIN>
__global__ __launch_bounds__(256)
__attribute__((amdgpu_waves_per_eu(1, (sizeof(PIX) == 1 && CH == 3 && MASK != 0u && STATS <= 1) ? 3 : 8))) void k_fused_u8c3(FusedParams P)
{
    constexpr bool U16 = sizeof(PIX) == 2;
    static_assert(CH == 3 || (CH == 4 && !U16), "4-channel fast path: uint8 tiles");
    __shared__ uint8_t s_lut[U16 ? 16 : 3 * 256];
    __shared__ unsigned int s_thr[U16 ? 3 * 260 : 4];
    __shared__ double s_par[U16 ? 6 : 1];
    constexpr int HIST_COPIES = 16;
    __shared__ unsigned int s_hist_all[HIST_COPIES * 3 * LARS_HIST_BINS];
    __shared__ HistCell<float> s_edges[LARS_HIST_CELLS];
    __shared__ double s_red[4][4];

    const int tid = threadIdx.x;
    unsigned int *const s_hist = s_hist_all + (tid & (HIST_COPIES - 1));
    const unsigned int bx = blockIdx.x, gx = gridDim.x;
    const long long tile = blockIdx.y;
    const long long npix = P.npix;
    const PIX *base = static_cast<const PIX *>(P.tiles) + tile * npix * CH;

    if (WB) {
        if (U16) {
            const uint8_t *blob = P.wb_table + tile * LARS_U16_BLOB_BYTES;
            const unsigned int *thr = reinterpret_cast<const unsigned int *>(blob + LARS_U16_THR_OFFSET);
            const double *par = reinterpret_cast<const double *>(blob + LARS_U16_PAR_OFFSET);
            for (int i = tid; i < 3 * 260; i += 256) s_thr[i] = thr[i];
            if (tid < 6) s_par[tid] = par[tid];
        } else {
            const uint8_t *t = P.wb_table + tile * 768;
            for (int i = tid; i < 768; i += 256) s_lut[i] = t[i];
        }
    }
    if (STATS >= 2) {
        for (int i = tid; i < HIST_COPIES * 3 * LARS_HIST_BINS; i += 256) s_hist_all[i] = 0;
        hist_cells_init<float>(s_edges, tid);
    }
    if (WB || STATS >= 2) __syncthreads();

    auto wb_map = [&](unsigned int v, int c) -> unsigned int {
        if (!U16) return s_lut[c * 256 + v];
        const double y = ((double)v - s_par[2 * c]) * s_par[2 * c + 1];
        int g = (int)y;
        g = g < 0 ? 0 : (g > 255 ? 255 : g);
        const unsigned int *t = s_thr + c * 260;
        g += (v >= t[g + 1] ? 1 : 0) - (v < t[g] ? 1 : 0);
        return (unsigned int)g;
    };

    Acc acc[3];
    acc_init(acc[0]); acc_init(acc[1]); acc_init(acc[2]);

#ifdef LARS_LAB_LAYOUT
    const long long ots = P.out_tile_stride;
#else
    const long long ots = npix;
#endif
    float *const oi0 = P.out_index[0] ? P.out_index[0] + tile * ots : nullptr;
    float *const oi1 = P.out_index[1] ? P.out_index[1] + tile * ots : nullptr;
    float *const oi2 = P.out_index[2] ? P.out_index[2] + tile * ots : nullptr;
    uint8_t *const owb = P.out_wb ? P.out_wb + tile * npix * CH : nullptr;
    uint8_t *const oc0 = P.out_rgba[0] ? P.out_rgba[0] + tile * npix * 4 : nullptr;
    uint8_t *const oc1 = P.out_rgba[1] ? P.out_rgba[1] + tile * npix * 4 : nullptr;
    uint8_t *const oc2 = P.out_rgba[2] ? P.out_rgba[2] + tile * npix * 4 : nullptr;
    const unsigned int *lut0 = reinterpret_cast<const unsigned int *>(P.cmap_lut[0]);
    const unsigned int *lut1 = reinterpret_cast<const unsigned int *>(P.cmap_lut[1]);
    const unsigned int *lut2 = reinterpret_cast<const unsigned int *>(P.cmap_lut[2]);

    const long long nquads = npix >> 2;
    const bool nt_st = (P.flags & 0x20000000u) != 0;
    __amdgpu_buffer_rsrc_t rsrc16;
    if (U16) rsrc16 = __builtin_amdgcn_make_buffer_rsrc(const_cast<PIX *>(base), 0, (int)(nquads * 24), 0x00020000);
    constexpr int NW = U16 ? 6 : 3;

    auto load_quad = [&](long long q, unsigned int (&w)[NW]) {
        if (U16) {
            const unsigned int off = (unsigned int)q * 24u;
            const fu32x4 a4 = stream_load_b128<POLICY>(rsrc16, off, 0);
            const fu32x2 a2 = stream_load_b64<POLICY>(rsrc16, off + 16u, 0);
            w[0] = a4.x; w[1] = a4.y; w[2] = a4.z; w[NW - 3] = a4.w; w[NW - 2] = a2.x; w[NW - 1] = a2.y;
        } else if (CH == 4) {
            const sl_u32x3 a = rgba_quad_to_rgb(
                stream_load_ptr<POLICY>(reinterpret_cast<const sl_u32x4 *>(reinterpret_cast<const uint8_t *>(base) + q * 16)));
            w[0] = a.x; w[1] = a.y; w[2] = a.z;
        } else {
            const unsigned int *p = reinterpret_cast<const unsigned int *>(reinterpret_cast<const uint8_t *>(base) + q * 12);
            w[0] = stream_load_ptr<POLICY>(p); w[1] = stream_load_ptr<POLICY>(p + 1); w[2] = stream_load_ptr<POLICY>(p + 2);
        }
    };
    auto do_quad = [&](long long q, const unsigned int (&w)[NW]) {
        unsigned int b[12];
        if (U16) {
#pragma unroll
            for (int i = 0; i < 6; ++i) { b[2 * i] = w[i % NW] & 0xFFFFu; b[2 * i + 1] = w[i % NW] >> 16; }
        } else {
            const unsigned int w0 = w[0], w1 = w[1], w2 = w[2];
            const unsigned int t[12] = {w0 & 0xFF, (w0 >> 8) & 0xFF, (w0 >> 16) & 0xFF, w0 >> 24,
                                        w1 & 0xFF, (w1 >> 8) & 0xFF, (w1 >> 16) & 0xFF, w1 >> 24,
                                        w2 & 0xFF, (w2 >> 8) & 0xFF, (w2 >> 16) & 0xFF, w2 >> 24};
#pragma unroll
            for (int i = 0; i < 12; ++i) b[i] = t[i];
        }
        if (WB) {
            const bool need_r = (MASK & 1u) || owb, need_g = (MASK & 6u) || owb;
#pragma unroll
            for (int i = 0; i < 12; ++i)
                if (i % 3 == 2 || (i % 3 == 0 && need_r) || (i % 3 == 1 && need_g)) b[i] = wb_map(b[i], i % 3);
            if (owb && CH == 4) {
                *reinterpret_cast<uint4 *>(owb + q * 16) = make_uint4(b[0] | (b[1] << 8) | (b[2] << 16), b[3] | (b[4] << 8) | (b[5] << 16),
                                                                      b[6] | (b[7] << 8) | (b[8] << 16), b[9] | (b[10] << 8) | (b[11] << 16));
            } else if (owb) {
                unsigned int *o = reinterpret_cast<unsigned int *>(owb + q * 12);
                o[0] = b[0] | (b[1] << 8) | (b[2] << 16) | (b[3] << 24);
                o[1] = b[4] | (b[5] << 8) | (b[6] << 16) | (b[7] << 24);
                o[2] = b[8] | (b[9] << 8) | (b[10] << 16) | (b[11] << 24);
            }
        }
        float v0[4], v1[4], v2[4];
#pragma unroll
        for (int px = 0; px < 4; ++px) {
            v0[px] = v1[px] = v2[px] = 0.0f;
            pixel_math<MASK, STATS, false, !U16, HIST_COPIES>((float)b[3 * px], (float)b[3 * px + 1], (float)b[3 * px + 2], 0u,
                                                            v0[px], v1[px], v2[px], acc, s_hist, s_edges);
        }
        if ((MASK & 1u) && oi0) store_plane4(oi0 + q * 4, v0, nt_st);
        if ((MASK & 2u) && oi1) store_plane4(oi1 + q * 4, v1, nt_st);
        if ((MASK & 4u) && oi2) store_plane4(oi2 + q * 4, v2, nt_st);
        if ((MASK & 1u) && oc0)
            *reinterpret_cast<uint4 *>(oc0 + q * 16) = make_uint4(lut0[cmap_index(v0[0])], lut0[cmap_index(v0[1])],
                                                                  lut0[cmap_index(v0[2])], lut0[cmap_index(v0[3])]);
        if ((MASK & 2u) && oc1)
            *reinterpret_cast<uint4 *>(oc1 + q * 16) = make_uint4(lut1[cmap_index(v1[0])], lut1[cmap_index(v1[1])],
                                                                  lut1[cmap_index(v1[2])], lut1[cmap_index(v1[3])]);
        if ((MASK & 4u) && oc2)
            *reinterpret_cast<uint4 *>(oc2 + q * 16) = make_uint4(lut2[cmap_index(v2[0])], lut2[cmap_index(v2[1])],
                                                                  lut2[cmap_index(v2[2])], lut2[cmap_index(v2[3])]);
    };

    constexpr int RUN = (!U16 && CH == 3 && MASK == 7u && STATS == 1) ? 16 : (U16 && MASK == 1u && STATS <= 1) ? 8 : 4;
    const long long nsteps = (nquads + 64 * RUN - 1) / (64 * RUN);
    const long long wstride = (long long)gx * 4;
    const unsigned int lane = (unsigned int)tid & 63u;
    for (long long st = (long long)bx * 4 + (tid >> 6); st < nsteps; st += wstride) {
        const long long q0 = st * (64 * RUN) + lane;
        unsigned int w[RUN][NW];
        if (st * (64 * RUN) + 64 * RUN <= nquads) {
#pragma unroll
            for (int j = 0; j < RUN; ++j) load_quad(q0 + 64 * j, w[j]);
            __builtin_amdgcn_sched_barrier(0);
#pragma unroll
            for (int j = 0; j < RUN; ++j) {
                do_quad(q0 + 64 * j, w[j]);
                __builtin_amdgcn_sched_barrier(0);
            }
        } else {
            for (int j = 0; j < RUN; ++j) {
                const long long q = q0 + 64 * j;
                if (q < nquads) { load_quad(q, w[0]); do_quad(q, w[0]); }
            }
        }
    }
    if (bx == 0 && tid < (int)(npix & 3)) {
        const long long i = nquads * 4 + tid;
        unsigned int r = base[i * CH], g = base[i * CH + 1], n = base[i * CH + 2];
        if (WB) { r = wb_map(r, 0); g = wb_map(g, 1); n = wb_map(n, 2); }
        if (WB && owb) {
            owb[i * CH] = (uint8_t)r; owb[i * CH + 1] = (uint8_t)g; owb[i * CH + 2] = (uint8_t)n;
            if (CH == 4) owb[i * CH + 3] = 0;
        }
        float a = 0, bq = 0, c = 0;
        pixel_math<MASK, STATS, false, !U16, HIST_COPIES>((float)r, (float)g, (float)n, 0u, a, bq, c, acc, s_hist, s_edges);
        if ((MASK & 1u) && oi0) oi0[i] = a;
        if ((MASK & 2u) && oi1) oi1[i] = bq;
        if ((MASK & 4u) && oi2) oi2[i] = c;
        if ((MASK & 1u) && oc0) reinterpret_cast<unsigned int *>(oc0)[i] = lut0[cmap_index(a)];
        if ((MASK & 2u) && oc1) reinterpret_cast<unsigned int *>(oc1)[i] = lut1[cmap_index(bq)];
        if ((MASK & 4u) && oc2) reinterpret_cast<unsigned int *>(oc2)[i] = lut2[cmap_index(c)];
    }

    if (STATS >= 1) {
        StatsAccView *rec = reinterpret_cast<StatsAccView *>(P.stats + tile * 3);
#pragma unroll
        for (int k = 0; k < 3; ++k)
            if ((MASK & (1u << k)) && (P.mask & (1u << k))) acc_flush(acc[k], rec + k, s_red, tid);
        if (STATS >= 2) {
            __syncthreads();
            for (int i = tid; i < 3 * LARS_HIST_BINS; i += 256) {
                const int k = i / LARS_HIST_BINS;
                unsigned int v = 0;
#pragma unroll
                for (int c = 0; c < HIST_COPIES; ++c) v += s_hist_all[i * HIST_COPIES + ((c + i) & (HIST_COPIES - 1))];
                if ((MASK & (1u << k)) && (P.mask & (1u << k)) && v) atomicAdd(&rec[k].hist[i - k * LARS_HIST_BINS], (unsigned long long)v);
            }
        }
    }
}

template <typename PIX, int NVAL>
__global__ __launch_bounds__(256) void k_fused_generic(FusedParams P)
{
    __shared__ unsigned int s_hist[3 * LARS_HIST_BINS];
    __shared__ HistCell<float> s_edges[LARS_HIST_CELLS];
    __shared__ double s_red[4][4];

    const int tid = threadIdx.x;
    const long long tile = blockIdx.y;
    const long long npix = P.npix;
    const int C = P.channels;
    const unsigned mask = P.mask;
    const bool stats = P.flags & (LARS_F_STATS | LARS_F_HIST | LARS_F_SUMSQ);
    const bool hist = P.flags & (LARS_F_HIST | LARS_F_SUMSQ);
    const bool sumsq = P.flags & LARS_F_SUMSQ;
    const PIX *base = static_cast<const PIX *>(P.tiles) + tile * npix * C;
    const uint8_t *tab = P.wb_table ? P.wb_table + tile * (NVAL == 256 ? 768ll : (long long)LARS_U16_BLOB_BYTES) : nullptr;

    for (int i = tid; i < 3 * LARS_HIST_BINS; i += 256) s_hist[i] = 0;
    hist_cells_init<float>(s_edges, tid);
    __syncthreads();

    Acc acc[3];
    acc_init(acc[0]); acc_init(acc[1]); acc_init(acc[2]);
    float *const oi0 = P.out_index[0] ? P.out_index[0] + tile * npix : nullptr;
    float *const oi1 = P.out_index[1] ? P.out_index[1] + tile * npix : nullptr;
    float *const oi2 = P.out_index[2] ? P.out_index[2] + tile * npix : nullptr;
    uint8_t *const owb = P.out_wb ? P.out_wb + tile * npix * C : nullptr;
    unsigned int *const oc0 = P.out_rgba[0] ? reinterpret_cast<unsigned int *>(P.out_rgba[0]) + tile * npix : nullptr;
    unsigned int *const oc1 = P.out_rgba[1] ? reinterpret_cast<unsigned int *>(P.out_rgba[1]) + tile * npix : nullptr;
    unsigned int *const oc2 = P.out_rgba[2] ? reinterpret_cast<unsigned int *>(P.out_rgba[2]) + tile * npix : nullptr;
    const unsigned int *lut0 = reinterpret_cast<const unsigned int *>(P.cmap_lut[0]);
    const unsigned int *lut1 = reinterpret_cast<const unsigned int *>(P.cmap_lut[1]);
    const unsigned int *lut2 = reinterpret_cast<const unsigned int *>(P.cmap_lut[2]);

    for (long long i = (long long)blockIdx.x * 256 + tid; i < npix; i += (long long)gridDim.x * 256) {
        const PIX *p = base + i * C;
        unsigned int r = p[0], g = p[1], n = p[2];
        if (tab) {
            r = tab[r]; g = tab[NVAL + g]; n = tab[2 * NVAL + n];
            if (owb) {
                uint8_t *o = owb + i * C;
                o[0] = (uint8_t)r; o[1] = (uint8_t)g; o[2] = (uint8_t)n;
                for (int c = 3; c < C; ++c) o[c] = 0;
            }
        }
        float a = 0, b = 0, c = 0;
        if (stats) {
            if (sumsq) pixel_math<7u, 3, true>((float)r, (float)g, (float)n, mask, a, b, c, acc, s_hist, s_edges);
            else if (hist) pixel_math<7u, 2, true>((float)r, (float)g, (float)n, mask, a, b, c, acc, s_hist, s_edges);
            else pixel_math<7u, 1, true>((float)r, (float)g, (float)n, mask, a, b, c, acc, s_hist, s_edges);
        } else {
            pixel_math<7u, 0, true>((float)r, (float)g, (float)n, mask, a, b, c, acc, s_hist, s_edges);
        }
        if ((mask & 1u) && oi0) oi0[i] = a;
        if ((mask & 2u) && oi1) oi1[i] = b;
        if ((mask & 4u) && oi2) oi2[i] = c;
        if ((mask & 1u) && oc0) oc0[i] = lut0[cmap_index(a)];
        if ((mask & 2u) && oc1) oc1[i] = lut1[cmap_index(b)];
        if ((mask & 4u) && oc2) oc2[i] = lut2[cmap_index(c)];
    }
    if (stats) {
        StatsAccView *rec = reinterpret_cast<StatsAccView *>(P.stats + tile * 3);
        for (int k = 0; k < 3; ++k)
            if (mask & (1u << k)) acc_flush(acc[k], rec + k, s_red, tid);
        if (hist) {
            __syncthreads();
            for (int i = tid; i < 3 * LARS_HIST_BINS; i += 256) {
                const int k = i / LARS_HIST_BINS;
                if ((mask & (1u << k)) && s_hist[i])
                    atomicAdd(&rec[k].hist[i - k * LARS_HIST_BINS], (unsigned long long)s_hist[i]);
            }
        }
    }
}

__device__ inline unsigned int mix32(unsigned int x)
{
    x ^= x >> 16; x *= 0x7FEB352Du; x ^= x >> 15; x *= 0x846CA68Bu; x ^= x >> 16;
    return x;
}
__device__ inline unsigned int veg_byte(unsigned int v, int ch)
{
    return ch == 0 ? 20u + (v * 3u) / 8u : ch == 1 ? 40u + v / 2u : ch == 2 ? 60u + (v * 3u) / 4u : v;
}

__global__ __launch_bounds__(256) void k_synth_u8(uint8_t *tiles, long long first_tile, long long nbytes,
                                                  int channels, unsigned int seed, int profile)
{
    const long long tile_local = blockIdx.y;
    const unsigned int salt = (unsigned int)(first_tile + tile_local) * 0x9E3779B9u;
    uint8_t *base = tiles + tile_local * nbytes;
    const long long nwords = (nbytes + 3) >> 2;
    for (long long k = (long long)blockIdx.x * 256 + threadIdx.x; k < nwords; k += (long long)gridDim.x * 256) {
        unsigned int w = mix32(mix32((unsigned int)k + seed) ^ salt);
        if (profile == 1) {
            unsigned int o = 0;
            for (int j = 0; j < 4; ++j) {
                const int ch = (int)((k * 4 + j) % channels);
                o |= (veg_byte((w >> (8 * j)) & 0xFF, ch) & 0xFF) << (8 * j);
            }
            w = o;
        }
        const long long off = k * 4;
        if (off + 4 <= nbytes && ((reinterpret_cast<uintptr_t>(base + off) & 3) == 0)) {
            *reinterpret_cast<unsigned int *>(base + off) = w;
        } else {
            for (int j = 0; j < 4 && off + j < nbytes; ++j) base[off + j] = (uint8_t)(w >> (8 * j));
        }
    }
}

}

using namespace lars;

namespace lars {
int blocks_per_tile(long long work_items, long long ntiles, int threads, long long target_total)
{
    long long want = (target_total * 256 / threads + ntiles - 1) / ntiles;
    if (tuning().blocks_per_tile > 0) want = tuning().blocks_per_tile;
    long long cap = work_items / ((long long)threads * 16);
    if (cap < 1) cap = 1;
    if (want > cap && tuning().blocks_per_tile <= 0) want = cap;
    const long long hard = (work_items + threads - 1) / threads;
    if (want > hard) want = hard;
    if (want < 1) want = 1;
    if (want > 65535) want = 65535;
    return (int)want;
}
}

extern "C" int lars_d_channel_hist(const void *tiles, int64_t ntiles, int64_t npix, int channels, int dtype,
                                   uint32_t *hist, void *stream)
{
    ThreadCtx *c;
    LARS_TRY(ensure_ctx(&c));
    if (!tiles || !hist || ntiles <= 0 || npix <= 0 || channels < 3)
        return fail(LARS_ERR_INVALID, "lars_d_channel_hist: bad arguments");
    if (ntiles > 65535) return fail(LARS_ERR_INVALID, "lars_d_channel_hist: ntiles > 65535 per call");
    hipStream_t s = pick_stream(c, stream);
    const int nval = dtype == LARS_U8 ? 256 : 65536;
    if (dtype != LARS_U8 && dtype != LARS_U16) return fail(LARS_ERR_INVALID, "lars_d_channel_hist: dtype");
    LARS_HIP_TRY(hipMemsetAsync(hist, 0, (size_t)ntiles * 3 * nval * sizeof(uint32_t), s));
    const bool fast = dtype == LARS_U8 && channels == 3 && (ntiles == 1 || (npix & 3) == 0) &&
                      ((reinterpret_cast<uintptr_t>(tiles) & 3) == 0);
    const bool fast4 = dtype == LARS_U8 && channels == 4 && (reinterpret_cast<uintptr_t>(tiles) & 15) == 0 &&
                       (ntiles == 1 || (npix & 3) == 0) && (long long)npix * 4 < (1ll << 30);
    if ((fast && tuning().hist_impl != 1 && (long long)npix * 3 < (1ll << 30)) || fast4) {
        long long want = tuning().blocks_per_tile > 0 ? tuning().blocks_per_tile : (1024 + ntiles - 1) / ntiles;
        const long long cap = (npix / 4 + 1023) / 1024;
        if (want > cap) want = cap;
        if (want < 1) want = 1;
        dim3 grid((unsigned)want, (unsigned)ntiles);
        chan_hist_v2_launch(static_cast<const uint8_t *>(tiles), (long long)npix, hist, grid, s, channels);
    } else if (fast) {
        dim3 grid(blocks_per_tile(npix / 4 + 1, ntiles), (unsigned)ntiles);
        hipLaunchKernelGGL(k_chan_hist_u8c3, grid, dim3(256), 0, s, static_cast<const uint8_t *>(tiles),
                           (long long)npix, hist);
    } else if (dtype == LARS_U8) {
        dim3 grid(blocks_per_tile(npix, ntiles), (unsigned)ntiles);
        hipLaunchKernelGGL((k_chan_hist_generic<uint8_t, 256>), grid, dim3(256), 0, s,
                           static_cast<const uint8_t *>(tiles), (long long)npix, channels, hist);
    } else {
        dim3 grid(blocks_per_tile(npix, ntiles), (unsigned)ntiles);
        hipLaunchKernelGGL((k_chan_hist_generic<uint16_t, 65536>), grid, dim3(256), 0, s,
                           static_cast<const uint16_t *>(tiles), (long long)npix, channels, hist);
    }
    return launch_check("lars_d_channel_hist");
}

extern "C" int lars_d_wb_table(const uint32_t *hist, int64_t ntiles, int64_t npix, int dtype, uint8_t *table,
                               double *percentiles, int rgn_variant, void *stream)
{
    ThreadCtx *c;
    LARS_TRY(ensure_ctx(&c));
    if (!hist || !table || ntiles <= 0 || npix <= 0) return fail(LARS_ERR_INVALID, "lars_d_wb_table: bad arguments");
    if (ntiles > 65535) return fail(LARS_ERR_INVALID, "lars_d_wb_table: ntiles > 65535 per call");
    hipStream_t s = pick_stream(c, stream);
    dim3 grid(3, (unsigned)ntiles);
    if (dtype == LARS_U8)
        hipLaunchKernelGGL((k_wb_table<256>), grid, dim3(256), 0, s, hist, (long long)npix, table, percentiles, rgn_variant);
    else if (dtype == LARS_U16)
        hipLaunchKernelGGL((k_wb_table<65536>), grid, dim3(256), 0, s, hist, (long long)npix, table, percentiles, rgn_variant);
    else
        return fail(LARS_ERR_INVALID, "lars_d_wb_table: dtype");
    return launch_check("lars_d_wb_table");
}

template <typename PIX, unsigned MASK, bool WB, int CH, int POLICY>
static void launch_fast_stats(int stats_mode, dim3 grid, hipStream_t s, const FusedParams &P)
{
    if (stats_mode == 0) hipLaunchKernelGGL((k_fused_u8c3<PIX, MASK, WB, 0, CH, POLICY>), grid, dim3(256), 0, s, P);
    else if (stats_mode == 1) hipLaunchKernelGGL((k_fused_u8c3<PIX, MASK, WB, 1, CH, POLICY>), grid, dim3(256), 0, s, P);
    else if (stats_mode == 3) hipLaunchKernelGGL((k_fused_u8c3<PIX, MASK, WB, 3, CH, POLICY>), grid, dim3(256), 0, s, P);
    else hipLaunchKernelGGL((k_fused_u8c3<PIX, MASK, WB, 2, CH, POLICY>), grid, dim3(256), 0, s, P);
}
template <typename PIX, unsigned MASK, int CH, int POLICY>
static void launch_fast_wb(bool wb, int stats_mode, dim3 grid, hipStream_t s, const FusedParams &P)
{
    if (wb) launch_fast_stats<PIX, MASK, true, CH, POLICY>(stats_mode, grid, s, P);
    else launch_fast_stats<PIX, MASK, false, CH, POLICY>(stats_mode, grid, s, P);
}
template <typename PIX, int CH, int POLICY>
static void launch_fast_policy(unsigned mask, bool wb, int stats_mode, dim3 grid, hipStream_t s, const FusedParams &P)
{
    switch (mask) {
    case 0u: hipLaunchKernelGGL((k_fused_u8c3<PIX, 0u, true, 0, CH, POLICY>), grid, dim3(256), 0, s, P); break;
    case 1u: launch_fast_wb<PIX, 1u, CH, POLICY>(wb, stats_mode, grid, s, P); break;
    case 2u: launch_fast_wb<PIX, 2u, CH, POLICY>(wb, stats_mode, grid, s, P); break;
    case 4u: launch_fast_wb<PIX, 4u, CH, POLICY>(wb, stats_mode, grid, s, P); break;
    default: launch_fast_wb<PIX, 7u, CH, POLICY>(wb, stats_mode, grid, s, P); break;
    }
}
template <typename PIX, int CH = 3>
static void launch_fast(unsigned mask, bool wb, int stats_mode, dim3 grid, hipStream_t s, const FusedParams &P, bool default_nt = false)
{
    if (stream_loads_nt(default_nt)) launch_fast_policy<PIX, CH, LOAD_NT>(mask, wb, stats_mode, grid, s, P);
    else launch_fast_policy<PIX, CH, LOAD_PLAIN>(mask, wb, stats_mode, grid, s, P);
}

extern "C" int lars_d_fused(const lars_fused_args *a)
{
    ThreadCtx *c;
    LARS_TRY(ensure_ctx(&c));
    if (!a || !a->tiles || a->ntiles <= 0 || a->npix <= 0 || a->channels < 3)
        return fail(LARS_ERR_INVALID, "lars_d_fused: bad arguments");
    if (a->ntiles > 65535) return fail(LARS_ERR_INVALID, "lars_d_fused: ntiles > 65535 per call");
    if (a->dtype != LARS_U8 && a->dtype != LARS_U16) return fail(LARS_ERR_INVALID, "lars_d_fused: dtype");
    const unsigned mask = a->index_mask & LARS_MASK_ALL;
    if (a->index_mask & ~LARS_MASK_ALL) return fail(LARS_ERR_INVALID, "lars_d_fused: unknown index bits in mask");
    const int stats_mode = (a->flags & LARS_F_SUMSQ) ? 3 : (a->flags & LARS_F_HIST) ? 2 : (a->flags & LARS_F_STATS) ? 1 : 0;
    if (stats_mode && !a->stats) return fail(LARS_ERR_INVALID, "lars_d_fused: stats requested but stats == NULL");
    if (a->out_wb && !a->wb_table) return fail(LARS_ERR_INVALID, "lars_d_fused: out_wb needs wb_table");
    for (int k = 0; k < 3; ++k)
        if (a->out_rgba[k] && !a->cmap_lut[k]) return fail(LARS_ERR_INVALID, "lars_d_fused: out_rgba needs cmap_lut");
    if (mask == 0 && !a->out_wb) return fail(LARS_ERR_INVALID, "lars_d_fused: nothing to do");
    hipStream_t s = pick_stream(c, a->stream);

    FusedParams P;
    P.tiles = a->tiles; P.npix = a->npix; P.channels = a->channels; P.wb_table = a->wb_table;
    for (int k = 0; k < 3; ++k) {
        const bool on = (mask >> k) & 1u;
        P.out_index[k] = on ? a->out_index[k] : nullptr;
        P.out_rgba[k] = on ? a->out_rgba[k] : nullptr;
        P.cmap_lut[k] = a->cmap_lut[k];
    }
    P.out_wb = a->out_wb; P.stats = a->stats; P.mask = mask; P.sel_hist = nullptr; P.sel_win = nullptr; P.sel_win_hist = nullptr; P.sel_below = nullptr;
    P.flags = (a->flags & 7u) | (tuning().nt_stores ? 0x20000000u : 0u);
#ifdef LARS_LAB_LAYOUT
    P.out_tile_stride = a->npix * (tuning().out_stride_planes > 1 ? tuning().out_stride_planes : 1);
#endif

    const long long nrec = a->ntiles * 3;
    const bool raw = (a->flags & LARS_F_RAW) != 0;
    if (stats_mode && !raw)
        hipLaunchKernelGGL(k_stats_init, dim3((unsigned)((nrec + 255) / 256)), dim3(256), 0, s, a->stats, nrec, mask);

    const bool aligned = (reinterpret_cast<uintptr_t>(a->tiles) & 3) == 0 &&
                         (!a->out_wb || (reinterpret_cast<uintptr_t>(a->out_wb) & 3) == 0) &&
                         (!P.out_index[0] || (reinterpret_cast<uintptr_t>(P.out_index[0]) & 15) == 0) &&
                         (!P.out_index[1] || (reinterpret_cast<uintptr_t>(P.out_index[1]) & 15) == 0) &&
                         (!P.out_index[2] || (reinterpret_cast<uintptr_t>(P.out_index[2]) & 15) == 0) &&
                         (!P.out_rgba[0] || (reinterpret_cast<uintptr_t>(P.out_rgba[0]) & 15) == 0) &&
                         (!P.out_rgba[1] || (reinterpret_cast<uintptr_t>(P.out_rgba[1]) & 15) == 0) &&
                         (!P.out_rgba[2] || (reinterpret_cast<uintptr_t>(P.out_rgba[2]) & 15) == 0);
    const unsigned tmask = (mask == 3u || mask == 5u || mask == 6u) ? 7u : mask;
    const bool ch_ok = a->channels == 3 || (a->channels == 4 && a->dtype == LARS_U8 && (reinterpret_cast<uintptr_t>(a->tiles) & 15) == 0 &&
                                            (!a->out_wb || (reinterpret_cast<uintptr_t>(a->out_wb) & 15) == 0));
    const bool fast = ch_ok && aligned && (a->ntiles == 1 || (a->npix & 3) == 0);
    const bool any_out = P.out_wb || P.out_index[0] || P.out_index[1] || P.out_index[2] || P.out_rgba[0] ||
                         P.out_rgba[1] || P.out_rgba[2];
    int impl = tuning().fused_impl;
    if (impl == 0) impl = (any_out && mask != 0u) ? 1 : 2;
    const bool small_tile = (long long)a->npix * 6 < (1ll << 30);
    int &ran = tuning().last_fused_kernel;
    if (fast && a->dtype == LARS_U8 && a->channels == 3 && impl >= 2 && small_tile) {
        dim3 grid(blocks_per_tile(a->npix / 4 + 1, a->ntiles, fused_v2_threads(any_out || mask == 0u)), (unsigned)a->ntiles);
        fused_v2_launch(tmask, a->wb_table != nullptr, stats_mode, tuning().nt_stores != 0, grid, s, P);
        ran = 2;
    } else if (fast && a->dtype == LARS_U8 && a->channels == 4) {
        dim3 grid(blocks_per_tile(a->npix / 4 + 1, a->ntiles, 256, 32768), (unsigned)a->ntiles);
        launch_fast<uint8_t, 4>(tmask, a->wb_table != nullptr, stats_mode, grid, s, P);
        ran = 5;
    } else if (fast && a->dtype == LARS_U8) {
        dim3 grid(blocks_per_tile(a->npix / 4 + 1, a->ntiles, 256, 32768), (unsigned)a->ntiles);
        const bool three_planes_stats = tmask == 7u && stats_mode == 1 && a->wb_table && P.out_index[0] && P.out_index[1] && P.out_index[2];
        launch_fast<uint8_t>(tmask, a->wb_table != nullptr, stats_mode, grid, s, P, three_planes_stats);
        ran = 1;
    } else if (fast && a->dtype == LARS_U16 && small_tile) {
        dim3 grid(blocks_per_tile(a->npix / 4 + 1, a->ntiles, 256, 32768), (unsigned)a->ntiles);
        launch_fast<uint16_t>(tmask, a->wb_table != nullptr, stats_mode, grid, s, P);
        ran = 3;
    } else {
        dim3 grid(blocks_per_tile(a->npix, a->ntiles), (unsigned)a->ntiles);
        if (a->dtype == LARS_U8) hipLaunchKernelGGL((k_fused_generic<uint8_t, 256>), grid, dim3(256), 0, s, P);
        else hipLaunchKernelGGL((k_fused_generic<uint16_t, 65536>), grid, dim3(256), 0, s, P);
        ran = 4;
    }
    if (stats_mode && !raw)
        hipLaunchKernelGGL(k_stats_finalize, dim3((unsigned)((nrec + 255) / 256)), dim3(256), 0, s, a->stats, nrec, mask,
                           (long long)a->npix);
    return launch_check("lars_d_fused");
}

extern "C" int lars_d_stats_begin(lars_stats *stats, int64_t ntiles, uint32_t index_mask, void *stream)
{
    ThreadCtx *c;
    LARS_TRY(ensure_ctx(&c));
    if (!stats || ntiles <= 0 || (index_mask & ~LARS_MASK_ALL)) return fail(LARS_ERR_INVALID, "lars_d_stats_begin: bad arguments");
    stats_init_launch(stats, ntiles * 3, index_mask & LARS_MASK_ALL, pick_stream(c, stream));
    return launch_check("lars_d_stats_begin");
}
extern "C" int lars_d_stats_end(lars_stats *stats, int64_t ntiles, uint32_t index_mask, int64_t npix, void *stream)
{
    ThreadCtx *c;
    LARS_TRY(ensure_ctx(&c));
    if (!stats || ntiles <= 0 || npix <= 0 || (index_mask & ~LARS_MASK_ALL)) return fail(LARS_ERR_INVALID, "lars_d_stats_end: bad arguments");
    stats_finalize_launch(stats, ntiles * 3, index_mask & LARS_MASK_ALL, (long long)npix, pick_stream(c, stream));
    return launch_check("lars_d_stats_end");
}

extern "C" int lars_d_stats_fold(const lars_stats *tile_records, int64_t ntiles, uint32_t index_mask, lars_stats *out, void *stream)
{
    ThreadCtx *c;
    LARS_TRY(ensure_ctx(&c));
    if (!tile_records || !out || ntiles <= 0 || !(index_mask & LARS_MASK_ALL) || (index_mask & ~LARS_MASK_ALL))
        return fail(LARS_ERR_INVALID, "lars_d_stats_fold: bad arguments");
    hipLaunchKernelGGL(k_stats_fold, dim3(3), dim3(256), 0, pick_stream(c, stream), tile_records, (long long)ntiles,
                       index_mask & LARS_MASK_ALL, out);
    return launch_check("lars_d_stats_fold");
}

extern "C" int lars_d_synth_u8(uint8_t *tiles, int64_t ntiles, int64_t first_tile, int64_t npix, int channels,
                               uint32_t seed, int profile, void *stream)
{
    ThreadCtx *c;
    LARS_TRY(ensure_ctx(&c));
    if (!tiles || ntiles <= 0 || npix <= 0 || channels < 1 || ntiles > 65535)
        return fail(LARS_ERR_INVALID, "lars_d_synth_u8: bad arguments");
    hipStream_t s = pick_stream(c, stream);
    const long long nbytes = (long long)npix * channels;
    dim3 grid(blocks_per_tile((nbytes + 3) / 4, ntiles), (unsigned)ntiles);
    hipLaunchKernelGGL(k_synth_u8, grid, dim3(256), 0, s, tiles, (long long)first_tile, nbytes, channels, seed, profile);
    return launch_check("lars_d_synth_u8");
}

namespace lars {
void stats_init_launch(lars_stats *stats, long long nrec, unsigned int mask, hipStream_t s)
{
    hipLaunchKernelGGL(k_stats_init, dim3((unsigned)((nrec + 255) / 256)), dim3(256), 0, s, stats, nrec, mask);
}
void stats_finalize_launch(lars_stats *stats, long long nrec, unsigned int mask, long long npix, hipStream_t s)
{
    hipLaunchKernelGGL(k_stats_finalize, dim3((unsigned)((nrec + 255) / 256)), dim3(256), 0, s, stats, nrec, mask, npix);
}
}
```

lars_image_processing_amd/csrc/fused_v2.hip:

```cpp
#include <string.h>

#include <type_traits>

#include "v2_device.h"

namespace lars {

__global__ __launch_bounds__(256) void k_quot_check(unsigned int max_den, unsigned long long *mismatches,
                                                    unsigned int *first_bad)
{
    unsigned long long bad = 0;
    for (unsigned int den = blockIdx.x + 1; den <= max_den; den += gridDim.x) {
        const float fd = (float)den;
        for (long long num = -(long long)den + threadIdx.x; num <= (long long)den; num += 256) {
            const float fn = (float)num;
            const float want = fn / fd;
            const float got = exact_quot(fn, fd);
            if (__builtin_bit_cast(unsigned int, want) != __builtin_bit_cast(unsigned int, got)) {
                if (!bad) { first_bad[0] = den; first_bad[1] = (unsigned int)(int)num; }
                ++bad;
            }
        }
    }
    if (bad) atomicAdd(mismatches, bad);
}

template <int CH, int POLICY = LOAD_PLAIN>
__global__ __launch_bounds__(1024) void k_chan_hist_u8c3_v2(const uint8_t *__restrict__ tiles, long long npix,
                                                            unsigned int *__restrict__ hist)
{
    __shared__ unsigned int s_h[3 * 256 * 32];
    const int tid = threadIdx.x;
    for (int i = tid; i < 3 * 256 * 32; i += 1024) s_h[i] = 0;
    __syncthreads();

    const long long tile = blockIdx.y;
    const uint8_t *base = tiles + tile * npix * CH;
    const long long nquads = npix >> 2;
    const unsigned int lane_off = (tid & 31) << 2;
    char *hb = reinterpret_cast<char *>(s_h);
#define HADD(word, shift, ch)                                                                          \
    atomicAdd(reinterpret_cast<unsigned int *>(hb + (ch) * 32768 + ((((word) >> (shift)) & 0xFFu) << 7) + lane_off), 1u)
    const long long step = (long long)gridDim.x * 1024;
    const long long q0 = (long long)blockIdx.x * 1024 + tid;
    const long long niter = (nquads + step - 1) / step;
#define HQUAD(a0, a1, a2)                                                                              \
    HADD(a0, 0, 0); HADD(a0, 8, 1); HADD(a0, 16, 2); HADD(a0, 24, 0);                                 \
    HADD(a1, 0, 1); HADD(a1, 8, 2); HADD(a1, 16, 0); HADD(a1, 24, 1);                                 \
    HADD(a2, 0, 2); HADD(a2, 8, 0); HADD(a2, 16, 1); HADD(a2, 24, 2);
    if (niter > 0 && CH == 4) {
        const __amdgpu_buffer_rsrc_t rsrc =
            __builtin_amdgcn_make_buffer_rsrc(const_cast<uint8_t *>(base), 0, (int)(nquads * 16), 0x00020000);
        const unsigned int voff = (unsigned int)q0 * 16u;
        const unsigned int step_b = (unsigned int)step * 16u;
        sl_u32x4 w[4];
#define HQUAD4(p)                                                                                       \
        {                                                                                               \
            const u32x3 a = rgba_quad_to_rgb(p);                                                        \
            HQUAD(a.x, a.y, a.z)                                                                        \
        }
#pragma unroll
        for (int k = 0; k < 4; ++k) w[k] = stream_load_b128<POLICY>(rsrc, voff, (unsigned)k * step_b);
        long long it = 0;
        unsigned int soff = 4u * step_b;
        for (; it + 4 <= niter - 1; it += 4) {
#pragma unroll
            for (int k = 0; k < 4; ++k) {
                HQUAD4(w[k])
                __builtin_amdgcn_sched_barrier(0);
                w[k] = stream_load_b128<POLICY>(rsrc, voff, soff + (unsigned)k * step_b);
                __builtin_amdgcn_sched_barrier(0);
            }
            soff += 4u * step_b;
        }
#pragma unroll
        for (int k = 0; k < 4; ++k) {
            if (it + k < niter && q0 + (it + k) * step < nquads) { HQUAD4(w[k]) }
        }
#undef HQUAD4
    } else if (niter > 0) {
        const __amdgpu_buffer_rsrc_t rsrc =
            __builtin_amdgcn_make_buffer_rsrc(const_cast<uint8_t *>(base), 0, (int)(nquads * 12), 0x00020000);
        const unsigned int voff = (unsigned int)q0 * 12u;
        const unsigned int step_b = (unsigned int)step * 12u;
        u32x3 w[4];
#pragma unroll
        for (int k = 0; k < 4; ++k) w[k] = stream_load_b96<POLICY>(rsrc, voff, (unsigned)k * step_b);
        long long it = 0;
        unsigned int soff = 4u * step_b;
        for (; it + 4 <= niter - 1; it += 4) {
#pragma unroll
            for (int k = 0; k < 4; ++k) {
                HQUAD(w[k].x, w[k].y, w[k].z)
                __builtin_amdgcn_sched_barrier(0);
                w[k] = stream_load_b96<POLICY>(rsrc, voff, soff + (unsigned)k * step_b);
                __builtin_amdgcn_sched_barrier(0);
            }
            soff += 4u * step_b;
        }
#pragma unroll
        for (int k = 0; k < 4; ++k) {
            if (it + k < niter && q0 + (it + k) * step < nquads) { HQUAD(w[k].x, w[k].y, w[k].z) }
        }
    }
#undef HQUAD
    if (blockIdx.x == 0 && tid < (int)(npix & 3)) {
        const uint8_t *p = base + (nquads * 4 + tid) * CH;
        HADD((unsigned)p[0], 0, 0); HADD((unsigned)p[1], 0, 1); HADD((unsigned)p[2], 0, 2);
    }
#undef HADD
    __syncthreads();
    if (tid < 768) {
        const unsigned int *row = s_h + tid * 32;
        unsigned int v = 0;
        for (int j = 0; j < 32; ++j) v += row[(j + tid) & 31];
        if (v) atomicAdd(&hist[tile * 768 + tid], v);
    }
}

typedef float f32x4 __attribute__((ext_vector_type(4)));
template <bool NT>
__device__ inline void store4(float *dst, float a, float b, float c, float d)
{
    f32x4 v = {a, b, c, d};
    if (NT) __builtin_nontemporal_store(v, reinterpret_cast<f32x4 *>(dst));
    else *reinterpret_cast<f32x4 *>(dst) = v;
}

struct WaveAcc {
    float mn, mx;
    double sum, sumsq;
};

#define V2_HIST_COPIES 16
#define V2_HIST_SHIFT 6
#define V2_HIST_ROWS 51
#define V2_HIST_WORDS (3 * V2_HIST_ROWS * V2_HIST_COPIES)
#define V2_WIN_ROW (64 + SELQ_WIN_SLOTS + 64)

__device__ inline void count_gt(unsigned int &counter, float x, float thr)
{
    unsigned int c;
    asm volatile("v_cmp_lt_f32 vcc, %1, %2\n\ts_bcnt1_i32_b64 %0, vcc" : "=s"(c) : "s"(thr), "v"(x) : "vcc", "scc");
    counter += c;
}
__device__ inline void count_lt(unsigned int &counter, float x, float thr)
{
    unsigned int c;
    asm volatile("v_cmp_gt_f32 vcc, %1, %2\n\ts_bcnt1_i32_b64 %0, vcc" : "=s"(c) : "s"(thr), "v"(x) : "vcc", "scc");
    counter += c;
}

__device__ inline void count4_gt(unsigned int &counter, const float (&x)[4], float thr)
{
    unsigned int c;
    asm volatile("v_cmp_lt_f32 vcc, %1, %2\n\ts_bcnt1_i32_b64 %0, vcc\n\t"
                 "v_cmp_lt_f32 vcc, %1, %3\n\ts_bcnt1_i32_b64 vcc_lo, vcc\n\ts_add_u32 %0, %0, vcc_lo\n\t"
                 "v_cmp_lt_f32 vcc, %1, %4\n\ts_bcnt1_i32_b64 vcc_lo, vcc\n\ts_add_u32 %0, %0, vcc_lo\n\t"
                 "v_cmp_lt_f32 vcc, %1, %5\n\ts_bcnt1_i32_b64 vcc_lo, vcc\n\ts_add_u32 %0, %0, vcc_lo"
                 : "=&s"(c) : "s"(thr), "v"(x[0]), "v"(x[1]), "v"(x[2]), "v"(x[3]) : "vcc", "scc");
    counter += c;
}
__device__ inline void count4_lt(unsigned int &counter, const float (&x)[4], float thr)
{
    unsigned int c;
    asm volatile("v_cmp_gt_f32 vcc, %1, %2\n\ts_bcnt1_i32_b64 %0, vcc\n\t"
                 "v_cmp_gt_f32 vcc, %1, %3\n\ts_bcnt1_i32_b64 vcc_lo, vcc\n\ts_add_u32 %0, %0, vcc_lo\n\t"
                 "v_cmp_gt_f32 vcc, %1, %4\n\ts_bcnt1_i32_b64 vcc_lo, vcc\n\ts_add_u32 %0, %0, vcc_lo\n\t"
                 "v_cmp_gt_f32 vcc, %1, %5\n\ts_bcnt1_i32_b64 vcc_lo, vcc\n\ts_add_u32 %0, %0, vcc_lo"
                 : "=&s"(c) : "s"(thr), "v"(x[0]), "v"(x[1]), "v"(x[2]), "v"(x[3]) : "vcc", "scc");
    counter += c;
}

template <int STATS, bool COUNT = true>
__device__ inline void push(WaveAcc &a, unsigned int &above, float x, float thr)
{
    a.mn = fminf(a.mn, x);
    a.mx = fmaxf(a.mx, x);
    const double xd = (double)x;
    a.sum += xd;
    if (STATS >= 3) a.sumsq += xd * xd;
    if (COUNT) count_gt(above, x, thr);
}

// ... 179 lines not shown
                if (STATS >= 2) hist_add(x, 1.0f, hb1);
                if (oi1) oi1[i] = x;
                if (oc1) reinterpret_cast<unsigned int *>(oc1)[i] = lut1[cmap_index(x)];
            }
            if (WANT_NDWI) {
                const float w = 0.0f - x;
                if (STATS >= 2) hist_add(x, -1.0f, hb2);
                if (oi2) oi2[i] = w;
                if (oc2) reinterpret_cast<unsigned int *>(oc2)[i] = lut2[cmap_index(w)];
            }
        }
    }

    if (STATS >= 2 || SEL) asm volatile("s_waitcnt lgkmcnt(0)" ::: "memory");
    if (RED_ALIASES_TABLE) __syncthreads();
    if (STATS >= 1) {
        for (int off = 32; off >= 1; off >>= 1) {
            if (WANT_NDVI) {
                acc_v.mn = fminf(acc_v.mn, __shfl_xor(acc_v.mn, off)); acc_v.mx = fmaxf(acc_v.mx, __shfl_xor(acc_v.mx, off));
                acc_v.sum += __shfl_xor(acc_v.sum, off);
                if (STATS >= 3) acc_v.sumsq += __shfl_xor(acc_v.sumsq, off);
            }
            if (NEED_G) {
                acc_g.mn = fminf(acc_g.mn, __shfl_xor(acc_g.mn, off)); acc_g.mx = fmaxf(acc_g.mx, __shfl_xor(acc_g.mx, off));
                acc_g.sum += __shfl_xor(acc_g.sum, off);
                if (STATS >= 3) acc_g.sumsq += __shfl_xor(acc_g.sumsq, off);
            }
        }
        const int wave = tid >> 6;
        double *row = s_red + wave * 16;
        if (lane == 0) {
            row[0] = acc_v.sum; row[1] = acc_v.sumsq; row[2] = (double)acc_v.mn; row[3] = (double)acc_v.mx; row[4] = (double)above_v;
            row[5] = acc_g.sum; row[6] = acc_g.sumsq; row[7] = (double)acc_g.mn; row[8] = (double)acc_g.mx;
            row[9] = (double)above_g; row[10] = (double)above_w;
        }
        __syncthreads();
        if (tid < 11) {
            const bool is_min = tid == 2 || tid == 7, is_max = tid == 3 || tid == 8;
            double t = s_red[tid];
#pragma unroll 1
            for (int w = 1; w < NWAVES; ++w) {
                const double o = s_red[w * 16 + tid];
                t = is_min ? fmin(t, o) : is_max ? fmax(t, o) : t + o;
            }
            s_red[tid] = t;
        }
        __syncthreads();
        if (tid == 0) {
            double t[11];
            for (int j = 0; j < 11; ++j) t[j] = s_red[j];
            StatsAccView *rec = reinterpret_cast<StatsAccView *>(P.stats + tile * 3);
            if (WANT_NDVI && (P.mask & 1u)) {
                atomicAdd(&rec[0].sum_fx, (unsigned long long)__double2ll_rn(t[0] * LARS_FX_SCALE));
                if (STATS >= 3) atomicAdd(&rec[0].sumsq_fx, (unsigned long long)__double2ll_rn(t[1] * LARS_FX_SCALE));
                atomicAdd(&rec[0].above, (unsigned long long)t[4]);
                atomicMin(&rec[0].min_key, f64_key(t[2]));
                atomicMax(&rec[0].max_key, f64_key(t[3]));
            }
            if (WANT_GNDVI && (P.mask & 2u)) {
                atomicAdd(&rec[1].sum_fx, (unsigned long long)__double2ll_rn(t[5] * LARS_FX_SCALE));
                if (STATS >= 3) atomicAdd(&rec[1].sumsq_fx, (unsigned long long)__double2ll_rn(t[6] * LARS_FX_SCALE));
                atomicAdd(&rec[1].above, (unsigned long long)t[9]);
                atomicMin(&rec[1].min_key, f64_key(t[7]));
                atomicMax(&rec[1].max_key, f64_key(t[8]));
            }
            if (WANT_NDWI && (P.mask & 4u)) {
                atomicAdd(&rec[2].sum_fx, (unsigned long long)__double2ll_rn((0.0 - t[5]) * LARS_FX_SCALE));
                if (STATS >= 3) atomicAdd(&rec[2].sumsq_fx, (unsigned long long)__double2ll_rn(t[6] * LARS_FX_SCALE));
                atomicAdd(&rec[2].above, (unsigned long long)t[10]);
                atomicMin(&rec[2].min_key, f64_key(0.0 - t[8]));
                atomicMax(&rec[2].max_key, f64_key(0.0 - t[7]));
            }
        }
        if (STATS >= 2) {
            __syncthreads();
            StatsAccView *rec = reinterpret_cast<StatsAccView *>(P.stats + tile * 3);
            if (tid < 3 * LARS_HIST_BINS) {
                const int k = tid / LARS_HIST_BINS;
                if ((MASK & (1u << k)) && (P.mask & (1u << k))) {
                    const int b = tid - k * LARS_HIST_BINS;
                    const unsigned int *rowh = s_hist + (k * V2_HIST_ROWS + b) * V2_HIST_COPIES;
                    unsigned int v = 0;
                    const int nwords = (b == LARS_HIST_BINS - 1) ? 2 * V2_HIST_COPIES : V2_HIST_COPIES;
                    for (int j = 0; j < nwords; ++j) v += rowh[j];
                    if (v) atomicAdd(&rec[k].hist[b], (unsigned long long)v);
                }
            }
        }
        if (SEL == 1) {
            unsigned int *h = P.sel_hist + tile * (4 * SELQ_BINS);
            for (int i = tid; i < 2 * SELQ_BINS; i += NTHR) {
                const unsigned int v = s_sel[i];
                if (v) atomicAdd(&h[(i >> 11) * (2 * SELQ_BINS) + (i & (SELQ_BINS - 1))], v);
            }
        }
        if (SEL == 2) {
            for (int i = tid; i < 2 * V2_WIN_ROW; i += NTHR) {
                const unsigned int v = s_win[i];
                if (!v) continue;
                const int stream = i / V2_WIN_ROW, w = i % V2_WIN_ROW;
                if (w < 64) atomicAdd(&P.sel_below[tile * 2 + stream], v);
                else if (w < 64 + SELQ_WIN_SLOTS) atomicAdd(&P.sel_win_hist[(tile * 2 + stream) * SELQ_WIN_SLOTS + (w - 64)], v);
            }
        }
    }
}


}

using namespace lars;

namespace lars {


void fused_v2_sel_launch(unsigned mask, bool wb, int stats, dim3 grid, hipStream_t s, const FusedParams &P)
{
    const int what = (P.sel_win && stats == 1) ? 0 : stats >= 3 ? 3 : stats == 2 ? 2 : 1;
    with_constant<1u, 2u, 4u, 7u>((int)mask, [&](auto M) {
        with_constant<false, true>(wb, [&](auto W) {
            with_constant<0, 1, 2, 3>(what, [&](auto X) {
                constexpr int STATS = decltype(X)::value ? decltype(X)::value : 1, SEL = decltype(X)::value ? 1 : 2;
                hipLaunchKernelGGL((k_fused_v2<decltype(M)::value, decltype(W)::value, STATS, false, false, SEL>), grid,
                                   dim3(V2Block<false>::threads), 0, s, P);
            });
        });
    });
}

int fused_v2_threads(bool any_out) { return any_out ? V2Block<true>::threads : V2Block<false>::threads; }

void fused_v2_launch(unsigned mask, bool wb, int stats, bool nt, dim3 grid, hipStream_t s, const FusedParams &P)
{
    const bool out = P.out_wb || P.out_index[0] || P.out_index[1] || P.out_index[2] || P.out_rgba[0] || P.out_rgba[1] ||
                     P.out_rgba[2];
    if (mask == 0u) {
        hipLaunchKernelGGL((k_fused_v2<0u, true, 0, true, false>), grid, dim3(V2Block<true>::threads), 0, s, P);
        return;
    }
    const int planes = !out ? 0 : nt ? 2 : 1;
    with_constant<1u, 2u, 4u, 7u>((int)mask, [&](auto M) {
        with_constant<false, true>(wb, [&](auto W) {
            with_constant<0, 1, 2, 3>(stats, [&](auto S) {
                with_constant<0, 1, 2>(planes, [&](auto O) {
                    constexpr bool OUT = decltype(O)::value != 0, NT = decltype(O)::value == 2;
                    hipLaunchKernelGGL((k_fused_v2<decltype(M)::value, decltype(W)::value, decltype(S)::value, OUT, NT>), grid,
                                       dim3(V2Block<OUT>::threads), 0, s, P);
                });
            });
        });
    });
}

void chan_hist_v2_launch(const uint8_t *tiles, long long npix, unsigned int *hist, dim3 grid, hipStream_t s, int channels)
{
    const bool nt = stream_loads_nt(true);
    if (channels == 4 && nt) hipLaunchKernelGGL((k_chan_hist_u8c3_v2<4, LOAD_NT>), grid, dim3(1024), 0, s, tiles, npix, hist);
    else if (channels == 4) hipLaunchKernelGGL((k_chan_hist_u8c3_v2<4, LOAD_PLAIN>), grid, dim3(1024), 0, s, tiles, npix, hist);
    else if (nt) hipLaunchKernelGGL((k_chan_hist_u8c3_v2<3, LOAD_NT>), grid, dim3(1024), 0, s, tiles, npix, hist);
    else hipLaunchKernelGGL((k_chan_hist_u8c3_v2<3, LOAD_PLAIN>), grid, dim3(1024), 0, s, tiles, npix, hist);
}

int quot_check_launch(unsigned int max_den, unsigned long long *mismatches_dev, unsigned int *first_bad_dev, hipStream_t s)
{
    hipLaunchKernelGGL(k_quot_check, dim3(2048), dim3(256), 0, s, max_den, mismatches_dev, first_bad_dev);
    return launch_check("k_quot_check");
}

}
```

lars_image_processing_amd/csrc/runtime.cpp:

```cpp
#include <stdarg.h>
#include <stdlib.h>
#include <string.h>
#include <cmath>

#include "common.h"

namespace lars {

static thread_local ThreadCtx g_ctx;

static void release_ctx(ThreadCtx *c)
{
    if (c->device < 0) return;
    if (hipSetDevice(c->device) != hipSuccess) { c->device = -1; return; }
    align_release();
    if (c->stream) { hipStreamSynchronize(c->stream); hipStreamDestroy(c->stream); c->stream = nullptr; }
    if (c->ws) { hipFree(c->ws); c->ws = nullptr; c->ws_bytes = 0; }
    if (c->scratch) { hipFree(c->scratch); c->scratch = nullptr; c->scratch_bytes = 0; }
    if (c->outline) { hipFree(c->outline); c->outline = nullptr; c->outline_bytes = 0; }
    c->u16_win_tiles = 0;
    c->device = -1;
}
struct CtxGuard {
    ~CtxGuard() { release_ctx(&g_ctx); }
};
static thread_local CtxGuard g_ctx_guard;

static int bind_device(ThreadCtx *c, int ordinal)
{
    int count = 0;
    hipError_t e = hipGetDeviceCount(&count);
    if (e != hipSuccess || count <= 0)
        return fail(LARS_ERR_NO_DEVICE, "no HIP device available (%s); liblars_hip has no CPU fallback",
                    e == hipSuccess ? "device count 0" : hipGetErrorString(e));
    if (ordinal < 0 || ordinal >= count) return fail(LARS_ERR_INVALID, "device ordinal %d out of range [0,%d)", ordinal, count);
    hipDeviceProp_t prop;
    LARS_HIP_TRY(hipGetDeviceProperties(&prop, ordinal));
    if (strncmp(prop.gcnArchName, "gfx950", 6) != 0)
        return fail(LARS_ERR_NO_DEVICE, "device %d is %s; liblars_hip is built for gfx950 (MI355X) only", ordinal,
                    prop.gcnArchName);
    LARS_HIP_TRY(hipSetDevice(ordinal));
    if (c->stream) { hipStreamDestroy(c->stream); c->stream = nullptr; }
    if (c->ws) { hipFree(c->ws); c->ws = nullptr; c->ws_bytes = 0; }
    if (c->scratch) { hipFree(c->scratch); c->scratch = nullptr; c->scratch_bytes = 0; }
    if (c->outline) { hipFree(c->outline); c->outline = nullptr; c->outline_bytes = 0; }
    c->u16_win_tiles = 0;
    LARS_HIP_TRY(hipStreamCreateWithFlags(&c->stream, hipStreamNonBlocking));
    c->device = ordinal;
    (void)&g_ctx_guard;
    return LARS_OK;
}

int ensure_ctx(ThreadCtx **out)
{
    ThreadCtx *c = &g_ctx;
    if (c->device < 0) LARS_TRY(bind_device(c, 0));
    else LARS_HIP_TRY(hipSetDevice(c->device));
    *out = c;
    return LARS_OK;
}

static int reserve(void **p, size_t *have, size_t bytes, hipStream_t s)
{
    if (bytes <= *have) return LARS_OK;
    if (*p) {
        LARS_HIP_TRY(hipStreamSynchronize(s));
        LARS_HIP_TRY(hipFree(*p));
        *p = nullptr; *have = 0;
    }
    size_t want = bytes + (bytes >> 3);
    want = (want + 0xFFFFF) & ~(size_t)0xFFFFF;
    hipError_t e = hipMalloc(p, want);
    if (e != hipSuccess) {
        *p = nullptr;
        return fail(LARS_ERR_OOM, "hipMalloc(%zu) for the library workspace failed: %s", want, hipGetErrorString(e));
    }
    *have = want;
    return LARS_OK;
}
int ws_reserve(ThreadCtx *c, size_t bytes) { return reserve(&c->ws, &c->ws_bytes, bytes, c->stream); }
int scratch_reserve(ThreadCtx *c, size_t bytes)
{
    c->u16_win_tiles = 0;
    return reserve(&c->scratch, &c->scratch_bytes, bytes, c->stream);
}

int outline_reserve(ThreadCtx *c, size_t bytes) { return reserve(&c->outline, &c->outline_bytes, bytes, c->stream); }

static Tuning g_tuning;
Tuning &tuning() { return g_tuning; }

struct Knob {
    const char *name;
    int Tuning::*field;
    enum Access { SET, READ_ONLY, LAB_LAYOUT } access;
    bool (*allowed)(int);
    const char *domain;
};
#ifdef LARS_LAB_LAYOUT
static const bool kLabLayout = true;
#else
static const bool kLabLayout = false;
#endif
static const Knob KNOBS[] = {
    {"fused_impl", &Tuning::fused_impl, Knob::SET, nullptr, nullptr},
    {"hist_impl", &Tuning::hist_impl, Knob::SET, nullptr, nullptr},
    {"nt_stores", &Tuning::nt_stores, Knob::SET, nullptr, nullptr},
    {"blocks_per_tile", &Tuning::blocks_per_tile, Knob::SET, nullptr, nullptr},
    {"load_policy", &Tuning::load_policy, Knob::SET, [](int v) { return v >= 0 && v <= 2; }, "0 .. 2"},
    {"selq_window", &Tuning::selq_window, Knob::SET, nullptr, nullptr},
    {"selq_list_wgs", &Tuning::selq_list_wgs, Knob::SET, nullptr, nullptr},
    {"joint_depth", &Tuning::joint_depth, Knob::SET, [](int v) { return v == 4 || v == 6 || v == 8 || v == 12; }, "4, 6, 8 or 12"},
    {"joint_window", &Tuning::joint_window, Knob::SET, [](int v) { return v >= 0 && v <= 5; }, "0 .. 5"},
    {"joint_win_depth", &Tuning::joint_win_depth, Knob::SET, [](int v) { return v == 4 || v == 5 || v == 6 || v == 12 || v == 15; }, "4, 5, 6, 12 or 15"},
    {"out_stride_planes", &Tuning::out_stride_planes, Knob::LAB_LAYOUT, nullptr, nullptr},
    {"u16_hist_impl", &Tuning::u16_hist_impl, Knob::SET, [](int v) { return v == 5 || v == 1 || v == 3; }, "5, 1 or 3"},
    {"jpeg_subseq_bits", &Tuning::jpeg_subseq_bits, Knob::SET, [](int v) { return v >= 32 && v <= 65536; }, "32 .. 65536"},
    {"tiff_strip_bytes", &Tuning::tiff_strip_bytes, Knob::SET, [](int v) { return v >= 1 && v <= (1 << 30); }, "1 .. 1073741824"},
    {"deflate_matching", &Tuning::deflate_matching, Knob::SET, [](int v) { return v == 0 || v == 1; }, "0 or 1"},
    {"zone_split_pixels", &Tuning::zone_split_pixels, Knob::SET, [](int v) { return v >= 64 && v <= (1 << 30); }, "64 .. 1073741824"},
    {"last_fused_kernel", &Tuning::last_fused_kernel, Knob::READ_ONLY, nullptr, nullptr},
    {"jpeg_last_rounds", &Tuning::jpeg_last_rounds, Knob::READ_ONLY, nullptr, nullptr},
};
static const Knob *find_knob(const char *key)
{
    for (const Knob &k : KNOBS)
        if (!strcmp(key, k.name)) return &k;
    return nullptr;
}

int launch_check(const char *what)
{
    hipError_t e = hipGetLastError();
    if (e != hipSuccess) return fail(LARS_ERR_HIP, "%s: kernel launch failed: %s", what, hipGetErrorString(e));
    return LARS_OK;
}

}

using namespace lars;

extern "C" {


int lars_device_count(int *count)
{
    if (!count) return fail(LARS_ERR_INVALID, "lars_device_count: NULL");
    int n = 0;
    hipError_t e = hipGetDeviceCount(&n);
    if (e != hipSuccess) { *count = 0; return fail(LARS_ERR_NO_DEVICE, "hipGetDeviceCount: %s", hipGetErrorString(e)); }
    *count = n;
    return LARS_OK;
}

int lars_set_device(int ordinal) { return bind_device(&g_ctx, ordinal); }

int lars_get_device(int *ordinal)
{
    ThreadCtx *c;
    LARS_TRY(ensure_ctx(&c));
    if (ordinal) *ordinal = c->device;
    return LARS_OK;
}

int lars_device_name(char *buf, size_t buflen)
{
    ThreadCtx *c;
    LARS_TRY(ensure_ctx(&c));
    hipDeviceProp_t prop;
    LARS_HIP_TRY(hipGetDeviceProperties(&prop, c->device));
    snprintf(buf, buflen, "%s (%s, %d CUs, %.1f GiB)", prop.name, prop.gcnArchName, prop.multiProcessorCount,
             (double)prop.totalGlobalMem / (1024.0 * 1024.0 * 1024.0));
    return LARS_OK;
}

int lars_malloc(void **dptr, size_t bytes)
{
    ThreadCtx *c;
    LARS_TRY(ensure_ctx(&c));
    if (!dptr) return fail(LARS_ERR_INVALID, "lars_malloc: NULL");
    const hipError_t e = hipMalloc(dptr, bytes ? bytes : 1);
    if (e != hipSuccess) { *dptr = nullptr; return fail(LARS_ERR_OOM, "hipMalloc(%zu): %s", bytes, hipGetErrorString(e)); }
    return LARS_OK;
}
int lars_free(void *dptr)
{
    if (!dptr) return LARS_OK;
    ThreadCtx *c;
    LARS_TRY(ensure_ctx(&c));
    LARS_HIP_TRY(hipFree(dptr));
    return LARS_OK;
}
int lars_memset(void *dptr, int value, size_t bytes, void *stream)
{
    ThreadCtx *c;
    LARS_TRY(ensure_ctx(&c));
    LARS_HIP_TRY(hipMemsetAsync(dptr, value, bytes, pick_stream(c, stream)));
    return LARS_OK;
}
int lars_memcpy_h2d(void *dst, const void *src, size_t bytes)
{
    ThreadCtx *c;
    LARS_TRY(ensure_ctx(&c));
    LARS_HIP_TRY(hipMemcpyAsync(dst, src, bytes, hipMemcpyHostToDevice, c->stream));
    LARS_HIP_TRY(hipStreamSynchronize(c->stream));
    return LARS_OK;
}
int lars_memcpy_d2h(void *dst, const void *src, size_t bytes)
{
    ThreadCtx *c;
    LARS_TRY(ensure_ctx(&c));
    LARS_HIP_TRY(hipMemcpyAsync(dst, src, bytes, hipMemcpyDeviceToHost, c->stream));
    LARS_HIP_TRY(hipStreamSynchronize(c->stream));
    return LARS_OK;
}
int lars_memcpy_d2d(void *dst, const void *src, size_t bytes, void *stream)
{
    ThreadCtx *c;
    LARS_TRY(ensure_ctx(&c));
    LARS_HIP_TRY(hipMemcpyAsync(dst, src, bytes, hipMemcpyDeviceToDevice, pick_stream(c, stream)));
    return LARS_OK;
}
int lars_stream_create(void **stream)
{
    ThreadCtx *c;
    LARS_TRY(ensure_ctx(&c));
    hipStream_t s;
    LARS_HIP_TRY(hipStreamCreateWithFlags(&s, hipStreamNonBlocking));
    *stream = s;
    return LARS_OK;
}
int lars_stream_destroy(void *stream)
{
    if (stream) LARS_HIP_TRY(hipStreamDestroy(reinterpret_cast<hipStream_t>(stream)));
    return LARS_OK;
}
int lars_synchronize(void *stream)
{
    ThreadCtx *c;
    LARS_TRY(ensure_ctx(&c));
    LARS_HIP_TRY(hipStreamSynchronize(pick_stream(c, stream)));
    return LARS_OK;
}
int lars_shutdown(void)
{
    release_ctx(&g_ctx);
    return LARS_OK;
}

int lars_mem_info(size_t *free_bytes, size_t *total_bytes)
{
    ThreadCtx *c;
    LARS_TRY(ensure_ctx(&c));
    size_t f = 0, t = 0;
    LARS_HIP_TRY(hipMemGetInfo(&f, &t));
    if (free_bytes) *free_bytes = f;
    if (total_bytes) *total_bytes = t;
    return LARS_OK;
}

int lars_event_create(void **event)
{
    ThreadCtx *c;
    LARS_TRY(ensure_ctx(&c));
    hipEvent_t e;
    LARS_HIP_TRY(hipEventCreate(&e));
    *event = e;
    return LARS_OK;
}
int lars_event_destroy(void *event)
{
    if (event) LARS_HIP_TRY(hipEventDestroy(reinterpret_cast<hipEvent_t>(event)));
    return LARS_OK;
// ... 78 lines not shown
```

Baseline: 360,000.

## Predict white-balance percentiles from sampled histograms and verify inside the fused pass

Builds per-tile channel histograms from a sampled subset of segments and decides statistically whether the 2nd/98th percentiles are settled. Confident tiles get provisional WB tables without a full histogram read, and the fused pass counts values around the predicted marks to confirm them exactly. Tiles whose verification fails are recomputed with the exact histogram path. The aim is to avoid a full extra read of the image for the histogram pre-pass, at the cost of considerable complexity, extra counting work in the fused kernel, and lazy fix-up paths for host queries.

```diff
diff --git a/include/lars_hip.h b/include/lars_hip.h
--- a/include/lars_hip.h
+++ b/include/lars_hip.h
@@ -107,6 +107,22 @@
 int lars_d_fused(const lars_fused_args *args);
 int lars_d_stats_begin(lars_stats *stats, int64_t ntiles, uint32_t index_mask, void *stream);
 int lars_d_stats_end(lars_stats *stats, int64_t ntiles, uint32_t index_mask, int64_t npix, void *stream);
+
+typedef struct lars_wb_verify {
+    void     *scratch;
+    int64_t   batch_tiles;
+    int64_t   tile_start;
+    uint32_t *hist;
+    double   *percentiles;
+    int32_t   rgn_variant;
+} lars_wb_verify;
+size_t lars_wb_predict_scratch_bytes(int64_t ntiles);
+int lars_d_wb_predict(const void *tiles, int64_t ntiles, int64_t npix, int channels, int dtype, uint32_t *hist, uint8_t *table,
+                      double *percentiles, int rgn_variant, void *scratch, int *predicted, void *stream);
+int lars_d_fused_verified(const lars_fused_args *args, const lars_wb_verify *v);
+int lars_d_wb_settle(const void *tiles, int64_t ntiles, int64_t npix, uint32_t *hist, uint8_t *table, double *percentiles,
+                     int rgn_variant, void *scratch, void *stream);
+int lars_wb_predict_report(const void *scratch, int64_t ntiles, int64_t *confident, int64_t *missed);
 
 int lars_d_index_planes_f32(const float *red, const float *green, const float *nir,
                             int64_t n, int index_id, float *out, void *stream);
diff --git a/lars_image_processing_amd/_ffi.py b/lars_image_processing_amd/_ffi.py
--- a/lars_image_processing_amd/_ffi.py
+++ b/lars_image_processing_amd/_ffi.py
@@ -66,6 +66,13 @@
         ("out_index", C.c_void_p * 3), ("out_wb", C.c_void_p),
         ("out_rgba", C.c_void_p * 3), ("cmap_lut", C.c_void_p * 3),
         ("stats", C.c_void_p), ("stream", C.c_void_p),
+    ]
+
+
+class WbVerify(C.Structure):
+    _fields_ = [
+        ("scratch", C.c_void_p), ("batch_tiles", C.c_int64), ("tile_start", C.c_int64),
+        ("hist", C.c_void_p), ("percentiles", C.c_void_p), ("rgn_variant", C.c_int32),
     ]
 
 
@@ -168,6 +175,11 @@
     "lars_d_fused": (_I, [C.POINTER(FusedArgs)]),
     "lars_d_stats_begin": (_I, [_P, _I64, _U32, _P]),
     "lars_d_stats_end": (_I, [_P, _I64, _U32, _I64, _P]),
+    "lars_wb_predict_scratch_bytes": (_SZ, [_I64]),
+    "lars_d_wb_predict": (_I, [_P, _I64, _I64, _I, _I, _P, _P, _P, _I, _P, C.POINTER(_I), _P]),
+    "lars_d_fused_verified": (_I, [C.POINTER(FusedArgs), C.POINTER(WbVerify)]),
+    "lars_d_wb_settle": (_I, [_P, _I64, _I64, _P, _P, _P, _I, _P, _P]),
+    "lars_wb_predict_report": (_I, [_P, _I64, C.POINTER(_I64), C.POINTER(_I64)]),
     "lars_d_index_planes_f32": (_I, [_P, _P, _P, _I64, _I, _P, _P]),
     "lars_d_ndvi_f64": (_I, [_P, _I64, _I, _I, _P, _P]),
     "lars_d_array_stats_f32": (_I, [_P, _I64, _F, _I, _P, _P]),
diff --git a/lars_image_processing_amd/batch.py b/lars_image_processing_amd/batch.py
--- a/lars_image_processing_amd/batch.py
+++ b/lars_image_processing_amd/batch.py
@@ -54,6 +54,17 @@
     if medians and code == _ffi.U8 and channels == 3 and npix * 6 < (1 << 30) and (ntiles == 1 or npix % 4 == 0):
         return "select" if not outputs and index_mask(indices) in (1, 2, 4, 7) else "per-pixel+select"
     return "per-pixel+radix" if medians else "per-pixel"
+
+
+def _knob(name):
+    v = C.c_int(0)
+    if _ffi.load().lars_get_tuning(name.encode(), C.byref(v)) != 0:
+        raise _ffi.LarsError(-1, f"lars_get_tuning: unknown key {name}")
+    return v.value
+
+
+def wb_predict_serves(channels, npix):
+    return channels == 3 and _knob("wb_predict") != 0 and npix >= _knob("wb_predict_min_pixels")
 
 
 def channels_of(indices, whole_image=False):
@@ -97,6 +108,9 @@
         self._joint_tiles = self.ntiles
         self._selq = None
         self.last_route = None
+        self._wbp_scratch = None
+        self._provisional = False
+        self._hist_stale = False
 
     @classmethod
     def from_host(cls, array, first_tile=0):
@@ -126,10 +140,20 @@
         if self.code == _ffi.U8:
             if self.hist is None:
                 self.hist = DeviceBuffer(self.ntiles * 3 * 256 * 4)
-            _ffi.call("lars_d_channel_hist", C.c_void_p(self.tiles.ptr), self.ntiles, self.npix, self.channels,
-                      self.code, C.c_void_p(self.hist.ptr), stream)
-            _ffi.call("lars_d_wb_table", C.c_void_p(self.hist.ptr), self.ntiles, self.npix, self.code,
-                      C.c_void_p(self.table.ptr), C.c_void_p(self.percentiles.ptr), int(rgn_variant), stream)
+            self._provisional = self._hist_stale = False
+            if wb_predict_serves(self.channels, self.npix):
+                if self._wbp_scratch is None:
+                    self._wbp_scratch = DeviceBuffer(int(_ffi.load().lars_wb_predict_scratch_bytes(self.ntiles)))
+                predicted = C.c_int(0)
+                _ffi.call("lars_d_wb_predict", C.c_void_p(self.tiles.ptr), self.ntiles, self.npix, self.channels, self.code,
+                          C.c_void_p(self.hist.ptr), C.c_void_p(self.table.ptr), C.c_void_p(self.percentiles.ptr), int(rgn_variant),
+                          C.c_void_p(self._wbp_scratch.ptr), C.byref(predicted), stream)
+                self._provisional = bool(predicted.value)
+            else:
+                _ffi.call("lars_d_channel_hist", C.c_void_p(self.tiles.ptr), self.ntiles, self.npix, self.channels,
+                          self.code, C.c_void_p(self.hist.ptr), stream)
+                _ffi.call("lars_d_wb_table", C.c_void_p(self.hist.ptr), self.ntiles, self.npix, self.code,
+                          C.c_void_p(self.table.ptr), C.c_void_p(self.percentiles.ptr), int(rgn_variant), stream)
         else:
             _ffi.call("lars_d_wb_prepare", C.c_void_p(self.tiles.ptr), self.ntiles, self.npix, self.channels,
                       self.code, C.c_void_p(self.table.ptr), C.c_void_p(self.percentiles.ptr), int(rgn_variant), stream)
@@ -138,6 +162,20 @@
         self._rgn_variant = int(rgn_variant)
         return self
 
+    def settle_tables(self, stream=None):
+        if self._provisional:
+            _ffi.call("lars_d_wb_settle", C.c_void_p(self.tiles.ptr), self.ntiles, self.npix, C.c_void_p(self.hist.ptr),
+                      C.c_void_p(self.table.ptr), C.c_void_p(self.percentiles.ptr), self._rgn_variant, C.c_void_p(self._wbp_scratch.ptr), stream)
+            self._provisional = False
+        return self
+
+    def wb_predict_report(self):
+        conf, missed = C.c_int64(0), C.c_int64(0)
+        if self._wbp_scratch is None:
+            return 0, 0
+        _ffi.call("lars_wb_predict_report", C.c_void_p(self._wbp_scratch.ptr), self.ntiles, C.byref(conf), C.byref(missed))
+        return int(conf.value), int(missed.value)
+
     def u16_window_report(self):
         if self.code != _ffi.U16:
             raise _ffi.LarsError(-1, "lars_u16_window_report: a uint8 batch's pre-pass does not take the value-window route")
@@ -156,11 +194,13 @@
 
     def host_tables(self, partial=False):
         self._need_channels(partial)
+        self.settle_tables()
         blob = self.table.download(np.uint8, (self.ntiles, self.table_bytes))
         return np.ascontiguousarray(blob[:, :3 * self.nvalues]).reshape(self.ntiles, 3, self.nvalues)
 
     def host_percentiles(self, partial=False):
         self._need_channels(partial)
+        self.settle_tables()
         return self.percentiles.download(np.float64, (self.ntiles, 3, 2))
 
     def host_hist(self, partial=False):
@@ -169,6 +209,11 @@
             missing = sorted({0, 1, 2} - self._hist_channels)
             raise RuntimeError(f"channel histograms of channel(s) {missing} are not valid: the last one-read pass was not asked for them "
                                f"(compute_wb_tables(), or run_joint(..., channel_hist=True); partial=True hands out what there is)")
+        self.settle_tables()
+        if self._hist_stale:
+            _ffi.call("lars_d_channel_hist", C.c_void_p(self.tiles.ptr), self.ntiles, self.npix, self.channels, self.code,
+                      C.c_void_p(self.hist.ptr), None)
+            self._hist_stale = False
         return self.hist.download(np.uint32, (self.ntiles, 3, 256))
 
     def make_outputs(self, indices=INDEX_NAMES, index=False, wb=False, rgba=False, ring=None, placement_trials=None, arena="auto",
@@ -235,7 +280,9 @@
         return timed / len(launches)
 
     def fused_args(self, indices=INDEX_NAMES, white_balance=True, stats=None, hist=False, outputs=None,
-                   stream=None, tile_start=0, tile_count=None, sumsq=False, raw=False):
+                   stream=None, tile_start=0, tile_count=None, sumsq=False, raw=False, settle=True):
+        if white_balance and settle:
+            self.settle_tables(stream)
         tile_count = self.ntiles - tile_start if tile_count is None else tile_count
         a = FusedArgs()
         a.tiles = self.tiles.ptr + tile_start * self.tile_bytes
@@ -276,10 +323,13 @@
 
     def run_fused_chunks(self, indices, white_balance, stats, hist, outputs, stream=None, sumsq=False, launch_events=None):
         chunk = self.ntiles if outputs is None else outputs.slots
+        verify = bool(white_balance and self._provisional)
         if chunk >= self.ntiles:
             if launch_events:
                 _ffi.call("lars_event_record", launch_events[0], stream)
-            self.run_fused(self.fused_args(indices, white_balance, stats, hist, outputs, stream, sumsq=sumsq))
+            self.run_fused(self.fused_args(indices, white_balance, stats, hist, outputs, stream, sumsq=sumsq, settle=not verify),
+                           0 if verify else None)
+            self._verified_pass_done(verify)
             if launch_events and len(launch_events) > 1:
                 _ffi.call("lars_event_record", launch_events[1], stream)
             return 1
@@ -292,22 +342,35 @@
         for start in range(0, self.ntiles, chunk):
             count = min(chunk, self.ntiles - start)
             self.run_fused(self.fused_args(indices, white_balance, stats, hist, outputs, stream, start, count, sumsq=sumsq,
-                                           raw=stats is not None))
+                                           raw=stats is not None, settle=not verify), start if verify else None)
             launches += 1
             if launch_events and launches < len(launch_events):
                 _ffi.call("lars_event_record", launch_events[launches], stream)
         if stats is not None:
             _ffi.call("lars_d_stats_end", C.c_void_p(stats.ptr), self.ntiles, mask, self.npix, stream)
+        self._verified_pass_done(verify)
         return launches
 
-    def run_fused(self, args):
-        _ffi.call("lars_d_fused", C.byref(args))
+    def _verified_pass_done(self, verify):
+        if verify:
+            self._provisional = False
+            self._hist_stale = True
+
+    def run_fused(self, args, verify_start=None):
+        if verify_start is None:
+            _ffi.call("lars_d_fused", C.byref(args))
+            return
+        v = _ffi.WbVerify()
+        v.scratch, v.batch_tiles, v.tile_start = self._wbp_scratch.ptr, self.ntiles, int(verify_start)
+        v.hist, v.percentiles, v.rgn_variant = self.hist.ptr, self.percentiles.ptr, self._rgn_variant
+        _ffi.call("lars_d_fused_verified", C.byref(args), C.byref(v))
 
     def can_joint(self):
         return joint_serves(self.code, self.channels, self.ntiles, self.npix)
 
     def run_joint(self, indices, white_balance, stats, hist=False, sumsq=False, pairs=None, stream=None, rgn_variant=0,
                   tile_count=None, channel_hist=False):
+        self.settle_tables(stream)
         mask = index_mask(indices)
         need = int(_ffi.load().lars_joint_scratch_bytes(self.ntiles, self.npix, mask))
         if self._joint_scratch is None or self._joint_scratch.nbytes < need:
@@ -372,6 +435,7 @@
         cache = self.__dict__.setdefault("_route_cache", {})
         if key in cache:
             return cache[key]
+        self.settle_tables()
         sample = min(int(sample), self.ntiles)
         if sample * self.npix < int(min_pixels) or self.channels != 3:
             cache[key] = "joint"
@@ -501,13 +565,14 @@
         return rec, med
 
     def free(self):
-        for b in (self.tiles, self.hist, self.table, self.percentiles, self._joint_scratch, self._selq):
+        for b in (self.tiles, self.hist, self.table, self.percentiles, self._joint_scratch, self._selq, self._wbp_scratch):
             if b is not None:
                 b.free()
 
     def tile_medians(self, indices=INDEX_NAMES, white_balance=True, stream=None):
         if white_balance and (self.table is None or not channels_of(indices) <= self._table_channels):
             raise RuntimeError("compute_wb_tables() first")
+        self.settle_tables(stream)
         return self._per_tile_select(indices, stream, lambda pairs, scratch: _ffi.call(
             "lars_d_quotient_median_pairs", C.c_void_p(self.tiles.ptr), self.ntiles, self.npix, self.channels, self.code,
             C.c_void_p(self.table.ptr) if white_balance else None, select_streams(indices), pairs, scratch, stream))
@@ -533,6 +598,7 @@
             raise TypeError("exact batch medians need uint8 tiles with 3 channels")
         if white_balance and self.table is None:
             raise RuntimeError("compute_wb_tables() first")
+        self.settle_tables(stream)
         if self._selq is None:
             self._selq = DeviceBuffer(2 * 2 * SELECT_BINS * 8)
         self._selq.zero(stream)
diff --git a/lars_image_processing_amd/csrc/common.h b/lars_image_processing_amd/csrc/common.h
--- a/lars_image_processing_amd/csrc/common.h
+++ b/lars_image_processing_amd/csrc/common.h
@@ -129,6 +129,10 @@
     int deflate_matching = 0;
     int joint_window = 1;
     int zone_split_pixels = 131072;
+    int wb_predict = 1;
+    int wb_predict_sixteenths = 4;
+    int wb_predict_k = 3;
+    int wb_predict_min_pixels = 1 << 20;
 };
 Tuning &tuning();
 inline bool stream_loads_nt(bool kernel_default_nt)
@@ -144,9 +148,30 @@
 #ifndef LARS_V2_STATS_WAVES
 #define LARS_V2_STATS_WAVES 8
 #endif
+enum : int { WB_GATE_REFUSED = 0,
+             WB_GATE_PREDICTED = 1,
+             WB_GATE_MISSED = 2 };
+struct WbGate {
+    const unsigned int *pred = nullptr;
+    const uint8_t *predv = nullptr;
+    unsigned int *counts = nullptr;
+    int mode = WB_GATE_REFUSED;
+};
 int fused_v2_threads(bool any_out);
 void fused_v2_launch(unsigned mask, bool wb, int stats, bool nt, dim3 grid, hipStream_t s, const FusedParams &P);
-void chan_hist_v2_launch(const uint8_t *tiles, long long npix, unsigned int *hist, dim3 grid, hipStream_t s, int channels = 3);
+void chan_hist_v2_launch(const uint8_t *tiles, long long npix, unsigned int *hist, dim3 grid, hipStream_t s, int channels = 3,
+                         const WbGate &gate = WbGate());
+void wb_exact_gated_launch(const uint8_t *tiles, long long ntiles, long long npix, unsigned int *hist, uint8_t *table, double *pcts,
+                           int rgn_variant, const WbGate &gate, lars_stats *stats, unsigned int stats_mask, unsigned int *missed, hipStream_t s);
+struct WbPredictScratch {
+    unsigned int *head;
+    unsigned int *pred;
+    uint8_t *predv;
+    unsigned int *counts;
+    unsigned int *ghist;
+    size_t bytes;
+};
+WbPredictScratch wb_predict_carve(void *base, long long ntiles);
 int selq_pass_launch(const uint8_t *tiles, const uint8_t *wb_table, long long ntiles, long long npix, int first,
                      const unsigned int bucket[4], unsigned long long *hist, hipStream_t s, unsigned streams);
 size_t selq_tile_scratch_bytes(long long ntiles);
diff --git a/lars_image_processing_amd/csrc/fused.hip b/lars_image_processing_amd/csrc/fused.hip
--- a/lars_image_processing_amd/csrc/fused.hip
+++ b/lars_image_processing_amd/csrc/fused.hip
@@ -4,6 +4,7 @@
 #include "device_common.h"
 #include "fused_device.h"
 #include "wg_device.h"
+#include "wb_predict_device.h"
 
 namespace lars {
 
@@ -83,9 +84,16 @@
 template <int NVAL>
 __global__ __launch_bounds__(256) void k_wb_table(const unsigned int *__restrict__ hist, long long npix,
                                                   uint8_t *__restrict__ table, double *__restrict__ pcts,
-                                                  int rgn_variant)
+                                                  int rgn_variant, WbGate gate, lars_stats *stats, unsigned int stats_mask,
+                                                  unsigned int *missed)
 {
     constexpr int PER = NVAL / 256;
+    if (NVAL == 256 && !wb_gate_open(gate, npix, blockIdx.y)) return;
+    if (NVAL == 256 && blockIdx.x == 0) {
+        if (stats && threadIdx.x < 3 && ((stats_mask >> threadIdx.x) & 1u))
+            stats_open(reinterpret_cast<StatsAccView *>(stats + (long long)blockIdx.y * 3 + threadIdx.x), (int)threadIdx.x);
+        if (threadIdx.x == 0 && missed) atomicAdd(missed, 1u);
+    }
     __shared__ unsigned long long s_scan[4];
     __shared__ double s_val[4];
     __shared__ double s_p[2];
@@ -99,20 +107,9 @@
     for (int j = 0; j < PER; ++j) local += h[tid * PER + j];
     const unsigned long long before = wg_exscan<256>(local, s_scan);
 
-    const double nm1 = (double)(npix - 1);
     double tq[2];
     long long rank[4];
-    for (int k = 0; k < 2; ++k) {
-        const double q = (k == 0 ? 2.0 : 98.0) / 100.0;
-        const double vi = nm1 * q;
-        const double fl = floor(vi);
-        long long lo = (long long)fl;
-        long long hi = lo + 1;
-        if (hi > npix - 1) hi = npix - 1;
-        rank[2 * k] = lo;
-        rank[2 * k + 1] = hi;
-        tq[k] = vi - fl;
-    }
+    for (int k = 0; k < 2; ++k) wb_mark_ranks(npix, k, rank[2 * k], rank[2 * k + 1], tq[k]);
     unsigned long long cum = before;
     for (int j = 0; j < PER; ++j) {
         const unsigned long long c = h[tid * PER + j];
@@ -125,18 +122,14 @@
     }
     __syncthreads();
     if (tid < 2) {
-        const double a = s_val[2 * tid], b = s_val[2 * tid + 1], t = tq[tid];
-        const double d = b - a;
-        double r = a + d * t;
-        if (t >= 0.5) r = b - d * (1.0 - t);
+        const double r = wb_lerp(s_val[2 * tid], s_val[2 * tid + 1], tq[tid]);
         s_p[tid] = r;
         if (pcts) pcts[slot * 2 + tid] = r;
     }
     __syncthreads();
     const double p_lo = s_p[0], p_hi = s_p[1];
     if (NVAL == 256) {
-        uint8_t *out = table + slot * 256;
-        out[tid] = (uint8_t)wb_level(tid, p_lo, p_hi, rgn_variant);
+        wb_fill_table_u8(table + slot * 256, tid, p_lo, p_hi, rgn_variant);
     } else {
         u16_fill_blob(table + (long long)blockIdx.y * LARS_U16_BLOB_BYTES, (int)blockIdx.x, p_lo, p_hi, rgn_variant, s_thr, tid);
     }
@@ -148,12 +141,7 @@
     if (i >= nrec) return;
     const int k = (int)(i % 3);
     if (!((mask >> k) & 1u)) return;
-    StatsAccView *a = reinterpret_cast<StatsAccView *>(stats + i);
-    a->sum_fx = 0; a->sumsq_fx = 0; a->count = 0; a->above = 0; a->nans = 0;
-    a->min_key = ~0ull; a->max_key = 0ull;
-    a->threshold = (k == LARS_NDWI) ? 0.0 : (double)0.2f;
-    a->index_id = (unsigned)k; a->reserved = 0;
-    for (int b = 0; b < LARS_HIST_BINS; ++b) a->hist[b] = 0;
+    stats_open(reinterpret_cast<StatsAccView *>(stats + i), k);
 }
 
 __global__ void k_stats_finalize(lars_stats *stats, long long nrec, unsigned int mask, long long npix)
@@ -283,13 +271,17 @@
 }
 
 
-template <typename PIX, unsigned MASK, bool WB, int STATS, int CH = 3, int POLICY = LOAD_PLAIN>
+template <typename PIX, unsigned MASK, bool WB, int STATS, int CH = 3, int VERIFY = 0, int POLICY = LOAD_PLAIN>
 __global__ __launch_bounds__(256)
-__attribute__((amdgpu_waves_per_eu(1, (sizeof(PIX) == 1 && CH == 3 && MASK != 0u && STATS <= 1) ? 3 : 8))) void k_fused_u8c3(FusedParams P)
+__attribute__((amdgpu_waves_per_eu(VERIFY ? 2 : 1, (sizeof(PIX) == 1 && CH == 3 && MASK != 0u && STATS <= 1) ? 3 : 8))) void k_fused_u8c3(FusedParams P, WbGate G)
 {
     constexpr bool U16 = sizeof(PIX) == 2;
     static_assert(CH == 3 || (CH == 4 && !U16), "4-channel fast path: uint8 tiles");
-    __shared__ uint8_t s_lut[U16 ? 16 : 3 * 256];
+    static_assert(!VERIFY || (!U16 && CH == 3 && WB && STATS <= 1), "the verifying form: uint8 RGNir, white balance, at most basic statistics");
+    if (VERIFY && G.mode == WB_GATE_MISSED && !wb_gate_open(G, P.npix, blockIdx.y)) return;
+    __shared__ unsigned int s_lutv[VERIFY ? 3 * 256 : 1];
+    __shared__ unsigned int s_cnt[VERIFY ? 4 * 12 : 1];
+    __shared__ uint8_t s_lut[(U16 || VERIFY) ? 16 : 3 * 256];
     __shared__ unsigned int s_thr[U16 ? 3 * 260 : 4];
     __shared__ double s_par[U16 ? 6 : 1];
     constexpr int HIST_COPIES = 16;
@@ -311,6 +303,14 @@
             const double *par = reinterpret_cast<const double *>(blob + LARS_U16_PAR_OFFSET);
             for (int i = tid; i < 3 * 260; i += 256) s_thr[i] = thr[i];
             if (tid < 6) s_par[tid] = par[tid];
+        } else if (VERIFY) {
+            const uint8_t *t = P.wb_table + tile * 768;
+            const uint8_t *pv = G.predv + tile * 8;
+            for (int i = tid; i < 768; i += 256) {
+                const unsigned int x = (unsigned int)i & 255u, lo = pv[(i >> 8) * 2], hi = pv[(i >> 8) * 2 + 1];
+                s_lutv[i] = ((unsigned int)t[i] << 24) | (x < lo ? 1u : 0u) | (x <= lo ? 1u << 6 : 0u) | (x < hi ? 1u << 12 : 0u) |
+                            (x <= hi ? 1u << 18 : 0u);
+            }
         } else {
             const uint8_t *t = P.wb_table + tile * 768;
             for (int i = tid; i < 768; i += 256) s_lut[i] = t[i];
@@ -322,7 +322,22 @@
     }
     if (WB || STATS >= 2) __syncthreads();
 
+    unsigned int vpack[3] = {0u, 0u, 0u};
+    unsigned int vcnt[12] = {0u, 0u, 0u, 0u, 0u, 0u, 0u, 0u, 0u, 0u, 0u, 0u};
+    auto verify_unpack = [&]() {
+#pragma unroll
+        for (int c = 0; c < 3; ++c) {
+            vcnt[c * 4] += vpack[c] & 63u; vcnt[c * 4 + 1] += (vpack[c] >> 6) & 63u;
+            vcnt[c * 4 + 2] += (vpack[c] >> 12) & 63u; vcnt[c * 4 + 3] += (vpack[c] >> 18) & 63u;
+            vpack[c] = 0u;
+        }
+    };
     auto wb_map = [&](unsigned int v, int c) -> unsigned int {
+        if (VERIFY) {
+            const unsigned int e = s_lutv[c * 256 + v];
+            asm("v_add_u32 %0, %0, %1" : "+v"(vpack[c]) : "v"(e));
+            return e >> 24;
+        }
         if (!U16) return s_lut[c * 256 + v];
         const double y = ((double)v - s_par[2 * c]) * s_par[2 * c + 1];
         int g = (int)y;
@@ -386,7 +401,7 @@
             for (int i = 0; i < 12; ++i) b[i] = t[i];
         }
         if (WB) {
-            const bool need_r = (MASK & 1u) || owb, need_g = (MASK & 6u) || owb;
+            const bool need_r = (MASK & 1u) || owb || VERIFY, need_g = (MASK & 6u) || owb || VERIFY;
 #pragma unroll
             for (int i = 0; i < 12; ++i)
                 if (i % 3 == 2 || (i % 3 == 0 && need_r) || (i % 3 == 1 && need_g)) b[i] = wb_map(b[i], i % 3);
@@ -421,7 +436,7 @@
                                                                   lut2[cmap_index(v2[2])], lut2[cmap_index(v2[3])]);
     };
 
-    constexpr int RUN = (!U16 && CH == 3 && MASK == 7u && STATS == 1) ? 16 : (U16 && MASK == 1u && STATS <= 1) ? 8 : 4;
+    constexpr int RUN = (!U16 && CH == 3 && MASK == 7u && STATS == 1) ? (VERIFY ? 12 : 16) : (U16 && MASK == 1u && STATS <= 1) ? 8 : 4;
     const long long nsteps = (nquads + 64 * RUN - 1) / (64 * RUN);
     const long long wstride = (long long)gx * 4;
     const unsigned int lane = (unsigned int)tid & 63u;
@@ -443,6 +458,7 @@
                 if (q < nquads) { load_quad(q, w[0]); do_quad(q, w[0]); }
             }
         }
+        if (VERIFY) verify_unpack();
     }
     if (bx == 0 && tid < (int)(npix & 3)) {
         const long long i = nquads * 4 + tid;
@@ -460,6 +476,22 @@
         if ((MASK & 1u) && oc0) reinterpret_cast<unsigned int *>(oc0)[i] = lut0[cmap_index(a)];
         if ((MASK & 2u) && oc1) reinterpret_cast<unsigned int *>(oc1)[i] = lut1[cmap_index(bq)];
         if ((MASK & 4u) && oc2) reinterpret_cast<unsigned int *>(oc2)[i] = lut2[cmap_index(c)];
+    }
+
+    if (VERIFY && G.mode != WB_GATE_MISSED) {
+        verify_unpack();
+#pragma unroll
+        for (int i = 0; i < 12; ++i)
+            for (int off = 32; off >= 1; off >>= 1) vcnt[i] += __shfl_xor(vcnt[i], off);
+        if ((tid & 63) == 0) {
+#pragma unroll
+            for (int i = 0; i < 12; ++i) s_cnt[(tid >> 6) * 12 + i] = vcnt[i];
+        }
+        __syncthreads();
+        if (tid < 12) {
+            const unsigned int v = s_cnt[tid] + s_cnt[12 + tid] + s_cnt[24 + tid] + s_cnt[36 + tid];
+            if (v) atomicAdd(&G.counts[tile * 12 + tid], v);
+        }
     }
 
     if (STATS >= 1) {
@@ -661,9 +693,11 @@
     hipStream_t s = pick_stream(c, stream);
     dim3 grid(3, (unsigned)ntiles);
     if (dtype == LARS_U8)
-        hipLaunchKernelGGL((k_wb_table<256>), grid, dim3(256), 0, s, hist, (long long)npix, table, percentiles, rgn_variant);
+        hipLaunchKernelGGL((k_wb_table<256>), grid, dim3(256), 0, s, hist, (long long)npix, table, percentiles, rgn_variant, WbGate(),
+                           (lars_stats *)nullptr, 0u, (unsigned int *)nullptr);
     else if (dtype == LARS_U16)
-        hipLaunchKernelGGL((k_wb_table<65536>), grid, dim3(256), 0, s, hist, (long long)npix, table, percentiles, rgn_variant);
+        hipLaunchKernelGGL((k_wb_table<65536>), grid, dim3(256), 0, s, hist, (long long)npix, table, percentiles, rgn_variant, WbGate(),
+                           (lars_stats *)nullptr, 0u, (unsigned int *)nullptr);
     else
         return fail(LARS_ERR_INVALID, "lars_d_wb_table: dtype");
     return launch_check("lars_d_wb_table");
@@ -672,10 +706,10 @@
 template <typename PIX, unsigned MASK, bool WB, int CH, int POLICY>
 static void launch_fast_stats(int stats_mode, dim3 grid, hipStream_t s, const FusedParams &P)
 {
-    if (stats_mode == 0) hipLaunchKernelGGL((k_fused_u8c3<PIX, MASK, WB, 0, CH, POLICY>), grid, dim3(256), 0, s, P);
-    else if (stats_mode == 1) hipLaunchKernelGGL((k_fused_u8c3<PIX, MASK, WB, 1, CH, POLICY>), grid, dim3(256), 0, s, P);
-    else if (stats_mode == 3) hipLaunchKernelGGL((k_fused_u8c3<PIX, MASK, WB, 3, CH, POLICY>), grid, dim3(256), 0, s, P);
-    else hipLaunchKernelGGL((k_fused_u8c3<PIX, MASK, WB, 2, CH, POLICY>), grid, dim3(256), 0, s, P);
+    if (stats_mode == 0) hipLaunchKernelGGL((k_fused_u8c3<PIX, MASK, WB, 0, CH, 0, POLICY>), grid, dim3(256), 0, s, P, WbGate());
+    else if (stats_mode == 1) hipLaunchKernelGGL((k_fused_u8c3<PIX, MASK, WB, 1, CH, 0, POLICY>), grid, dim3(256), 0, s, P, WbGate());
+    else if (stats_mode == 3) hipLaunchKernelGGL((k_fused_u8c3<PIX, MASK, WB, 3, CH, 0, POLICY>), grid, dim3(256), 0, s, P, WbGate());
+    else hipLaunchKernelGGL((k_fused_u8c3<PIX, MASK, WB, 2, CH, 0, POLICY>), grid, dim3(256), 0, s, P, WbGate());
 }
 template <typename PIX, unsigned MASK, int CH, int POLICY>
 static void launch_fast_wb(bool wb, int stats_mode, dim3 grid, hipStream_t s, const FusedParams &P)
@@ -687,7 +721,7 @@
 static void launch_fast_policy(unsigned mask, bool wb, int stats_mode, dim3 grid, hipStream_t s, const FusedParams &P)
 {
     switch (mask) {
-    case 0u: hipLaunchKernelGGL((k_fused_u8c3<PIX, 0u, true, 0, CH, POLICY>), grid, dim3(256), 0, s, P); break;
+    case 0u: hipLaunchKernelGGL((k_fused_u8c3<PIX, 0u, true, 0, CH, 0, POLICY>), grid, dim3(256), 0, s, P, WbGate()); break;
     case 1u: launch_fast_wb<PIX, 1u, CH, POLICY>(wb, stats_mode, grid, s, P); break;
     case 2u: launch_fast_wb<PIX, 2u, CH, POLICY>(wb, stats_mode, grid, s, P); break;
     case 4u: launch_fast_wb<PIX, 4u, CH, POLICY>(wb, stats_mode, grid, s, P); break;
@@ -701,7 +735,56 @@
     else launch_fast_policy<PIX, CH, LOAD_PLAIN>(mask, wb, stats_mode, grid, s, P);
 }
 
-extern "C" int lars_d_fused(const lars_fused_args *a)
+template <int POLICY>
+static void launch_verify_policy(unsigned mask, int stats_mode, dim3 grid, hipStream_t s, const FusedParams &P, const WbGate &G)
+{
+#define LARS_VERIFY_CASE(M)                                                                                              \
+    case M:                                                                                                              \
+        if (stats_mode) hipLaunchKernelGGL((k_fused_u8c3<uint8_t, M, true, 1, 3, 1, POLICY>), grid, dim3(256), 0, s, P, G);  \
+        else hipLaunchKernelGGL((k_fused_u8c3<uint8_t, M, true, 0, 3, 1, POLICY>), grid, dim3(256), 0, s, P, G);           \
+        break;
+    switch (mask) {
+        LARS_VERIFY_CASE(1u)
+        LARS_VERIFY_CASE(2u)
+        LARS_VERIFY_CASE(4u)
+    default:
+        LARS_VERIFY_CASE(7u)
+    }
+#undef LARS_VERIFY_CASE
+}
+static void launch_verify(unsigned mask, int stats_mode, dim3 grid, hipStream_t s, const FusedParams &P, const WbGate &G, bool default_nt)
+{
+    if (stream_loads_nt(default_nt)) launch_verify_policy<LOAD_NT>(mask, stats_mode, grid, s, P, G);
+    else launch_verify_policy<LOAD_PLAIN>(mask, stats_mode, grid, s, P, G);
+}
+
+namespace lars {
+void wb_exact_gated_launch(const uint8_t *tiles, long long ntiles, long long npix, unsigned int *hist, uint8_t *table, double *pcts,
+                           int rgn_variant, const WbGate &gate, lars_stats *stats, unsigned int stats_mask, unsigned int *missed, hipStream_t s)
+{
+    long long want = tuning().blocks_per_tile > 0 ? tuning().blocks_per_tile : (1024 + ntiles - 1) / ntiles;
+    const long long cap = (npix / 4 + 1023) / 1024;
+    if (want > cap) want = cap;
+    if (want < 1) want = 1;
+    chan_hist_v2_launch(tiles, npix, hist, dim3((unsigned)want, (unsigned)ntiles), s, 3, gate);
+    hipLaunchKernelGGL((k_wb_table<256>), dim3(3, (unsigned)ntiles), dim3(256), 0, s, hist, npix, table, pcts, rgn_variant, gate, stats,
+                       stats_mask, missed);
+}
+}
+
+static int fused_run(const lars_fused_args *a, const lars_wb_verify *v);
+
+extern "C" int lars_d_fused(const lars_fused_args *a) { return fused_run(a, nullptr); }
+
+extern "C" int lars_d_fused_verified(const lars_fused_args *a, const lars_wb_verify *v)
+{
+    if (!v || !v->scratch || !v->hist || !v->percentiles || v->batch_tiles <= 0 || v->tile_start < 0 || !a || a->ntiles <= 0 ||
+        v->tile_start + a->ntiles > v->batch_tiles || !a->wb_table)
+        return fail(LARS_ERR_INVALID, "lars_d_fused_verified: bad arguments");
+    return fused_run(a, v);
+}
+
+static int fused_run(const lars_fused_args *a, const lars_wb_verify *v)
 {
     ThreadCtx *c;
     LARS_TRY(ensure_ctx(&c));
@@ -756,7 +839,37 @@
     if (impl == 0) impl = (any_out && mask != 0u) ? 1 : 2;
     const bool small_tile = (long long)a->npix * 6 < (1ll << 30);
     int &ran = tuning().last_fused_kernel;
-    if (fast && a->dtype == LARS_U8 && a->channels == 3 && impl >= 2 && small_tile) {
+    const bool verify = v && fast && a->dtype == LARS_U8 && a->channels == 3 && !(impl >= 2 && small_tile) && a->wb_table && stats_mode <= 1 &&
+                        tmask != 0u && a->npix < (1ll << 31);
+    WbPredictScratch ps{};
+    WbGate G;
+    unsigned int *v_hist = nullptr;
+    double *v_pcts = nullptr;
+    if (v) {
+        ps = wb_predict_carve(v->scratch, v->batch_tiles);
+        G.pred = ps.pred + v->tile_start; G.predv = ps.predv + v->tile_start * 8; G.counts = ps.counts + v->tile_start * 12;
+        v_hist = v->hist + v->tile_start * 768;
+        v_pcts = v->percentiles + v->tile_start * 6;
+        if (!verify) {
+            G.mode = WB_GATE_PREDICTED;
+            wb_exact_gated_launch(static_cast<const uint8_t *>(a->tiles), a->ntiles, a->npix, v_hist, const_cast<uint8_t *>(a->wb_table), v_pcts,
+                                  v->rgn_variant, G, nullptr, 0u, nullptr, s);
+            LARS_HIP_TRY(hipMemsetAsync(ps.pred + v->tile_start, 0, (size_t)a->ntiles * sizeof(unsigned int), s));
+        }
+    }
+    if (verify) {
+        dim3 grid(blocks_per_tile(a->npix / 4 + 1, a->ntiles, 256, 32768), (unsigned)a->ntiles);
+        const bool three_planes_stats = tmask == 7u && stats_mode == 1 && P.out_index[0] && P.out_index[1] && P.out_index[2];
+        G.mode = -1;
+        launch_verify(tmask, stats_mode, grid, s, P, G, three_planes_stats);
+        G.mode = WB_GATE_MISSED;
+        wb_exact_gated_launch(static_cast<const uint8_t *>(a->tiles), a->ntiles, a->npix, v_hist, const_cast<uint8_t *>(a->wb_table), v_pcts,
+                              v->rgn_variant, G, stats_mode ? a->stats : nullptr, mask, ps.head + 1, s);
+        const dim3 repair_grid(grid.x < 32u ? grid.x : 32u, grid.y);
+        launch_verify(tmask, stats_mode, repair_grid, s, P, G, three_planes_stats);
+        LARS_HIP_TRY(hipMemsetAsync(ps.pred + v->tile_start, 0, (size_t)a->ntiles * sizeof(unsigned int), s));
+        ran = 1;
+    } else if (fast && a->dtype == LARS_U8 && a->channels == 3 && impl >= 2 && small_tile) {
         dim3 grid(blocks_per_tile(a->npix / 4 + 1, a->ntiles, fused_v2_threads(any_out || mask == 0u)), (unsigned)a->ntiles);
         fused_v2_launch(tmask, a->wb_table != nullptr, stats_mode, tuning().nt_stores != 0, grid, s, P);
         ran = 2;
diff --git a/lars_image_processing_amd/csrc/fused_v2.hip b/lars_image_processing_amd/csrc/fused_v2.hip
--- a/lars_image_processing_amd/csrc/fused_v2.hip
+++ b/lars_image_processing_amd/csrc/fused_v2.hip
@@ -3,6 +3,7 @@
 #include <type_traits>
 
 #include "v2_device.h"
+#include "wb_predict_device.h"
 
 namespace lars {
 
@@ -27,9 +28,10 @@
 
 template <int CH, int POLICY = LOAD_PLAIN>
 __global__ __launch_bounds__(1024) void k_chan_hist_u8c3_v2(const uint8_t *__restrict__ tiles, long long npix,
-                                                            unsigned int *__restrict__ hist)
+                                                            unsigned int *__restrict__ hist, WbGate gate)
 {
     __shared__ unsigned int s_h[3 * 256 * 32];
+    if (!wb_gate_open(gate, npix, blockIdx.y)) return;
     const int tid = threadIdx.x;
     for (int i = tid; i < 3 * 256 * 32; i += 1024) s_h[i] = 0;
     __syncthreads();
@@ -515,13 +517,13 @@
     });
 }
 
-void chan_hist_v2_launch(const uint8_t *tiles, long long npix, unsigned int *hist, dim3 grid, hipStream_t s, int channels)
+void chan_hist_v2_launch(const uint8_t *tiles, long long npix, unsigned int *hist, dim3 grid, hipStream_t s, int channels, const WbGate &gate)
 {
     const bool nt = stream_loads_nt(true);
-    if (channels == 4 && nt) hipLaunchKernelGGL((k_chan_hist_u8c3_v2<4, LOAD_NT>), grid, dim3(1024), 0, s, tiles, npix, hist);
-    else if (channels == 4) hipLaunchKernelGGL((k_chan_hist_u8c3_v2<4, LOAD_PLAIN>), grid, dim3(1024), 0, s, tiles, npix, hist);
-    else if (nt) hipLaunchKernelGGL((k_chan_hist_u8c3_v2<3, LOAD_NT>), grid, dim3(1024), 0, s, tiles, npix, hist);
-    else hipLaunchKernelGGL((k_chan_hist_u8c3_v2<3, LOAD_PLAIN>), grid, dim3(1024), 0, s, tiles, npix, hist);
+    if (channels == 4 && nt) hipLaunchKernelGGL((k_chan_hist_u8c3_v2<4, LOAD_NT>), grid, dim3(1024), 0, s, tiles, npix, hist, gate);
+    else if (channels == 4) hipLaunchKernelGGL((k_chan_hist_u8c3_v2<4, LOAD_PLAIN>), grid, dim3(1024), 0, s, tiles, npix, hist, gate);
+    else if (nt) hipLaunchKernelGGL((k_chan_hist_u8c3_v2<3, LOAD_NT>), grid, dim3(1024), 0, s, tiles, npix, hist, gate);
+    else hipLaunchKernelGGL((k_chan_hist_u8c3_v2<3, LOAD_PLAIN>), grid, dim3(1024), 0, s, tiles, npix, hist, gate);
 }
 
 int quot_check_launch(unsigned int max_den, unsigned long long *mismatches_dev, unsigned int *first_bad_dev, hipStream_t s)
diff --git a/lars_image_processing_amd/csrc/runtime.cpp b/lars_image_processing_amd/csrc/runtime.cpp
--- a/lars_image_processing_amd/csrc/runtime.cpp
+++ b/lars_image_processing_amd/csrc/runtime.cpp
@@ -119,6 +119,10 @@
     {"tiff_strip_bytes", &Tuning::tiff_strip_bytes, Knob::SET, [](int v) { return v >= 1 && v <= (1 << 30); }, "1 .. 1073741824"},
     {"deflate_matching", &Tuning::deflate_matching, Knob::SET, [](int v) { return v == 0 || v == 1; }, "0 or 1"},
     {"zone_split_pixels", &Tuning::zone_split_pixels, Knob::SET, [](int v) { return v >= 64 && v <= (1 << 30); }, "64 .. 1073741824"},
+    {"wb_predict", &Tuning::wb_predict, Knob::SET, [](int v) { return v >= 0 && v <= 3; }, "0 .. 3"},
+    {"wb_predict_sixteenths", &Tuning::wb_predict_sixteenths, Knob::SET, [](int v) { return v >= 2 && v <= 4; }, "2 .. 4"},
+    {"wb_predict_k", &Tuning::wb_predict_k, Knob::SET, [](int v) { return v >= 1 && v <= 16; }, "1 .. 16"},
+    {"wb_predict_min_pixels", &Tuning::wb_predict_min_pixels, Knob::SET, [](int v) { return v >= 1; }, "1 or more"},
     {"last_fused_kernel", &Tuning::last_fused_kernel, Knob::READ_ONLY, nullptr, nullptr},
     {"jpeg_last_rounds", &Tuning::jpeg_last_rounds, Knob::READ_ONLY, nullptr, nullptr},
 };
diff --git a/lars_image_processing_amd/csrc/wb_predict.hip b/lars_image_processing_amd/csrc/wb_predict.hip
--- /dev/null
+++ b/lars_image_processing_amd/csrc/wb_predict.hip
@@ -0,0 +1,255 @@
+#include "common.h"
+#include "device_common.h"
+#include "wg_device.h"
+#include "wb_predict_device.h"
+
+namespace lars {
+
+constexpr int WBP_GROUPS = 16;
+constexpr unsigned int WBP_SEG_BYTES = 4096;
+
+__host__ __device__ inline unsigned int wbp_mix(unsigned int x)
+{
+    x ^= x >> 16; x *= 0x7FEB352Du; x ^= x >> 15; x *= 0x846CA68Bu; x ^= x >> 16;
+    return x;
+}
+__host__ __device__ inline unsigned int wbp_segment(unsigned int tile, unsigned int i, unsigned int nseg, unsigned int nsample)
+{
+    const unsigned int start = (unsigned int)(((unsigned long long)i * nseg) / nsample);
+    const unsigned int end = (unsigned int)(((unsigned long long)(i + 1) * nseg) / nsample);
+    return start + wbp_mix(i * 0x9E3779B9u + tile * 0x85EBCA6Bu + 0x1234567u) % (end - start);
+}
+
+template <int POLICY>
+__global__ __launch_bounds__(1024) void k_wb_sample_hist(const uint8_t *__restrict__ tiles, long long npix, unsigned int nseg,
+                                                         unsigned int nsample, unsigned int *__restrict__ ghist)
+{
+    __shared__ unsigned int s_h[3 * 256 * 32];
+    const int tid = threadIdx.x;
+    for (int i = tid; i < 3 * 256 * 32; i += 1024) s_h[i] = 0;
+    __syncthreads();
+
+    const unsigned int tile = blockIdx.y, group = blockIdx.x;
+    const uint8_t *base = tiles + (long long)tile * npix * 3;
+    const __amdgpu_buffer_rsrc_t rsrc =
+        __builtin_amdgcn_make_buffer_rsrc(const_cast<uint8_t *>(base), 0, (int)(nseg * WBP_SEG_BYTES), 0x00020000);
+    const unsigned int wave = (unsigned int)tid >> 6, lane = (unsigned int)tid & 63u;
+    const unsigned int sub = wave >> 2, quarter = wave & 3u;
+    const unsigned int per_group = nsample / WBP_GROUPS;
+    const unsigned int lane_off = ((unsigned int)tid & 31u) << 2;
+    char *hb = reinterpret_cast<char *>(s_h);
+#define WBP_ADD(word, shift, choff)                                                                     \
+    atomicAdd(reinterpret_cast<unsigned int *>(hb + (choff) + ((((word) >> (shift)) & 0xFFu) << 7) + lane_off), 1u)
+    for (unsigned int k0 = sub; k0 < per_group; k0 += 16u) {
+        sl_u32x4 w[4];
+        unsigned int ph[4];
+#pragma unroll
+        for (int j = 0; j < 4; ++j) {
+            const unsigned int k = k0 + 4u * (unsigned int)j;
+            if (k < per_group) {
+                const unsigned int seg = wbp_segment(tile, k * WBP_GROUPS + group, nseg, nsample);
+                w[j] = stream_load_b128<POLICY>(rsrc, seg * WBP_SEG_BYTES + quarter * 1024u + lane * 16u, 0);
+                ph[j] = (seg + quarter + lane) % 3u;
+            }
+        }
+#pragma unroll
+        for (int j = 0; j < 4; ++j) {
+            if (k0 + 4u * (unsigned int)j < per_group) {
+                const unsigned int c0 = ph[j] * 32768u, c1 = ((ph[j] + 1u) % 3u) * 32768u, c2 = ((ph[j] + 2u) % 3u) * 32768u;
+                WBP_ADD(w[j].x, 0, c0); WBP_ADD(w[j].x, 8, c1); WBP_ADD(w[j].x, 16, c2); WBP_ADD(w[j].x, 24, c0);
+                WBP_ADD(w[j].y, 0, c1); WBP_ADD(w[j].y, 8, c2); WBP_ADD(w[j].y, 16, c0); WBP_ADD(w[j].y, 24, c1);
+                WBP_ADD(w[j].z, 0, c2); WBP_ADD(w[j].z, 8, c0); WBP_ADD(w[j].z, 16, c1); WBP_ADD(w[j].z, 24, c2);
+                WBP_ADD(w[j].w, 0, c0); WBP_ADD(w[j].w, 8, c1); WBP_ADD(w[j].w, 16, c2); WBP_ADD(w[j].w, 24, c0);
+            }
+        }
+    }
+#undef WBP_ADD
+    __syncthreads();
+    if (tid < 768) {
+        const unsigned int *row = s_h + tid * 32;
+        unsigned int v = 0;
+        for (int j = 0; j < 32; ++j) v += row[(j + tid) & 31];
+        ghist[((long long)tile * WBP_GROUPS + group) * 768 + tid] = v;
+    }
+}
+
+__global__ __launch_bounds__(256) void k_wb_decide(const unsigned int *__restrict__ ghist, int kk, int hook, int rgn_variant,
+                                                   unsigned int *__restrict__ head, unsigned int *__restrict__ pred,
+                                                   uint8_t *__restrict__ predv, unsigned int *__restrict__ counts,
+                                                   uint8_t *__restrict__ table, double *__restrict__ pcts)
+{
+    __shared__ unsigned int s_g[WBP_GROUPS][768];
+    __shared__ unsigned int s_scan[4];
+    __shared__ unsigned int s_v[6], s_before[6], s_bin[6], s_n[3];
+    __shared__ double s_f[12][WBP_GROUPS];
+    __shared__ int s_ok[12];
+    __shared__ int s_conf;
+    const int tid = threadIdx.x;
+    const long long tile = blockIdx.x;
+    const unsigned int *g = ghist + tile * WBP_GROUPS * 768;
+    for (int i = tid; i < WBP_GROUPS * 768; i += 256) (&s_g[0][0])[i] = g[i];
+    __syncthreads();
+    for (int c = 0; c < 3; ++c) {
+        unsigned int local = 0;
+        for (int j = 0; j < WBP_GROUPS; ++j) local += s_g[j][c * 256 + tid];
+        unsigned int total = 0;
+        const unsigned int before = wg_exscan<256>(local, s_scan, &total);
+        if (tid == 0) s_n[c] = total;
+        for (int k = 0; k < 2; ++k) {
+            long long lo, hi;
+            double t;
+            wb_mark_ranks(total ? (long long)total : 1, k, lo, hi, t);
+            if (local && (unsigned long long)lo >= before && (unsigned long long)lo < (unsigned long long)before + local) {
+                s_v[c * 2 + k] = (unsigned int)tid; s_before[c * 2 + k] = before; s_bin[c * 2 + k] = local;
+            }
+        }
+    }
+    __syncthreads();
+    if (tid < 12 * WBP_GROUPS) {
+        const int m = tid / (2 * WBP_GROUPS), e = (tid / WBP_GROUPS) & 1, j = tid % WBP_GROUPS, c = m >> 1;
+        const unsigned int *h = &s_g[j][c * 256];
+        const unsigned int end = s_n[c] ? s_v[m] + (unsigned int)e : 0u;
+        unsigned int cum = 0, all = 0;
+        for (unsigned int b = 0; b < 256u; ++b) {
+            const unsigned int x = h[(b + (unsigned int)j * 8u) & 255u];
+            all += x;
+            cum += ((b + (unsigned int)j * 8u) & 255u) < end ? x : 0u;
+        }
+        s_f[m * 2 + e][j] = all ? (double)cum / (double)all : -1.0;
+    }
+    __syncthreads();
+    if (tid < 12) {
+        const int m = tid >> 1, e = tid & 1, c = m >> 1;
+        const double q = ((m & 1) == 0 ? 2.0 : 98.0) / 100.0;
+        bool ok = s_n[c] != 0u;
+        double mean = 0.0;
+        for (int j = 0; j < WBP_GROUPS; ++j) { ok = ok && s_f[tid][j] >= 0.0; mean += s_f[tid][j]; }
+        mean /= WBP_GROUPS;
+        double ss = 0.0;
+        for (int j = 0; j < WBP_GROUPS; ++j) ss += (s_f[tid][j] - mean) * (s_f[tid][j] - mean);
+        if (ok) {
+            const double n = (double)s_n[c];
+            double se = sqrt(ss / (double)(WBP_GROUPS * (WBP_GROUPS - 1)));
+            const double floor_se = sqrt(q * (1.0 - q) / n);
+            if (se < floor_se) se = floor_se;
+            const double f = ((double)s_before[m] + (e ? (double)s_bin[m] : 0.0)) / n;
+            const double margin = e ? f - q : q - f;
+            ok = (e == 0 && s_v[m] == 0u) || (e == 1 && s_v[m] == 255u) || margin >= (double)kk * se;
+        }
+        s_ok[tid] = ok ? 1 : 0;
+    }
+    __syncthreads();
+    if (tid == 0) {
+        bool conf = s_n[0] && s_n[1] && s_n[2];
+        for (int i = 0; i < 12; ++i) conf = conf && (s_ok[i] || hook == 3);
+        if (conf && hook == 2)
+            for (int m = 0; m < 6; ++m) s_v[m] = s_v[m] < 255u ? s_v[m] + 1u : 254u;
+        s_conf = conf ? 1 : 0;
+        pred[tile] = conf ? 1u : 0u;
+        if (conf) atomicAdd(&head[0], 1u);
+    }
+    __syncthreads();
+    if (tid < 12) counts[tile * 12 + tid] = 0u;
+    if (tid < 8) predv[tile * 8 + tid] = tid < 6 ? (uint8_t)s_v[tid] : (uint8_t)0;
+    if (!s_conf) return;
+    if (tid < 6) pcts[tile * 6 + tid] = (double)s_v[tid];
+    for (int c = 0; c < 3; ++c)
+        wb_fill_table_u8(table + (tile * 3 + c) * 256, tid, (double)s_v[c * 2], (double)s_v[c * 2 + 1], rgn_variant);
+}
+
+WbPredictScratch wb_predict_carve(void *base, long long ntiles)
+{
+    Carver cv(base);
+    WbPredictScratch p;
+    p.head = cv.take<unsigned int>(4);
+    p.pred = cv.take<unsigned int>((size_t)ntiles);
+    p.predv = cv.take<uint8_t>((size_t)ntiles * 8);
+    p.counts = cv.take<unsigned int>((size_t)ntiles * 12);
+    p.ghist = cv.take<unsigned int>((size_t)ntiles * WBP_GROUPS * 768);
+    p.bytes = cv.bytes();
+    return p;
+}
+
+static unsigned int wbp_sample_segments(long long npix, unsigned int *nseg_out)
+{
+    const long long nseg = npix * 3 / WBP_SEG_BYTES;
+    *nseg_out = (unsigned int)nseg;
+    if (nseg < WBP_GROUPS) return 0;
+    long long n = (nseg * tuning().wb_predict_sixteenths / 16 + WBP_GROUPS - 1) / WBP_GROUPS * WBP_GROUPS;
+    if (n < WBP_GROUPS) n = WBP_GROUPS;
+    if (n > nseg) n = nseg / WBP_GROUPS * WBP_GROUPS;
+    return (unsigned int)n;
+}
+
+}
+
+using namespace lars;
+
+extern "C" size_t lars_wb_predict_scratch_bytes(int64_t ntiles)
+{
+    return ntiles > 0 ? wb_predict_carve(nullptr, ntiles).bytes : 0;
+}
+
+extern "C" int lars_d_wb_predict(const void *tiles, int64_t ntiles, int64_t npix, int channels, int dtype, uint32_t *hist, uint8_t *table,
+                                 double *percentiles, int rgn_variant, void *scratch, int *predicted, void *stream)
+{
+    ThreadCtx *c;
+    LARS_TRY(ensure_ctx(&c));
+    if (!tiles || !hist || !table || !percentiles || !scratch || !predicted || ntiles <= 0 || ntiles > 65535 || npix <= 0 || channels < 3 ||
+        dtype != LARS_U8)
+        return fail(LARS_ERR_INVALID, "lars_d_wb_predict: bad arguments");
+    hipStream_t s = pick_stream(c, stream);
+    const WbPredictScratch ps = wb_predict_carve(scratch, ntiles);
+    unsigned int nseg = 0;
+    const unsigned int nsample = wbp_sample_segments(npix, &nseg);
+    const bool can = tuning().wb_predict != 0 && channels == 3 && (ntiles == 1 || (npix & 3) == 0) &&
+                     (reinterpret_cast<uintptr_t>(tiles) & 3) == 0 && (long long)npix * 3 < (1ll << 30) && tuning().hist_impl != 1 &&
+                     npix >= tuning().wb_predict_min_pixels && nsample > 0;
+    *predicted = can ? 1 : 0;
+    LARS_HIP_TRY(hipMemsetAsync(ps.head, 0, (size_t)(reinterpret_cast<char *>(ps.predv) - reinterpret_cast<char *>(ps.head)), s));
+    if (!can) {
+        LARS_TRY(lars_d_channel_hist(tiles, ntiles, npix, channels, dtype, hist, stream));
+        return lars_d_wb_table(hist, ntiles, npix, dtype, table, percentiles, rgn_variant, stream);
+    }
+    LARS_HIP_TRY(hipMemsetAsync(hist, 0, (size_t)ntiles * 768 * sizeof(uint32_t), s));
+    const dim3 grid(WBP_GROUPS, (unsigned)ntiles);
+    if (stream_loads_nt(true))
+        hipLaunchKernelGGL((k_wb_sample_hist<LOAD_NT>), grid, dim3(1024), 0, s, static_cast<const uint8_t *>(tiles), (long long)npix, nseg, nsample, ps.ghist);
+    else
+        hipLaunchKernelGGL((k_wb_sample_hist<LOAD_PLAIN>), grid, dim3(1024), 0, s, static_cast<const uint8_t *>(tiles), (long long)npix, nseg, nsample, ps.ghist);
+    hipLaunchKernelGGL(k_wb_decide, dim3((unsigned)ntiles), dim3(256), 0, s, ps.ghist, tuning().wb_predict_k, tuning().wb_predict, rgn_variant,
+                       ps.head, ps.pred, ps.predv, ps.counts, table, percentiles);
+    WbGate G;
+    G.pred = ps.pred; G.predv = ps.predv; G.counts = ps.counts; G.mode = WB_GATE_REFUSED;
+    wb_exact_gated_launch(static_cast<const uint8_t *>(tiles), ntiles, npix, hist, table, percentiles, rgn_variant, G, nullptr, 0u, nullptr, s);
+    return launch_check("lars_d_wb_predict");
+}
+
+extern "C" int lars_d_wb_settle(const void *tiles, int64_t ntiles, int64_t npix, uint32_t *hist, uint8_t *table, double *percentiles,
+                                int rgn_variant, void *scratch, void *stream)
+{
+    ThreadCtx *c;
+    LARS_TRY(ensure_ctx(&c));
+    if (!tiles || !hist || !table || !percentiles || !scratch || ntiles <= 0 || ntiles > 65535 || npix <= 0)
+        return fail(LARS_ERR_INVALID, "lars_d_wb_settle: bad arguments");
+    hipStream_t s = pick_stream(c, stream);
+    const WbPredictScratch ps = wb_predict_carve(scratch, ntiles);
+    WbGate G;
+    G.pred = ps.pred; G.predv = ps.predv; G.counts = ps.counts; G.mode = WB_GATE_PREDICTED;
+    wb_exact_gated_launch(static_cast<const uint8_t *>(tiles), ntiles, npix, hist, table, percentiles, rgn_variant, G, nullptr, 0u, nullptr, s);
+    LARS_HIP_TRY(hipMemsetAsync(ps.pred, 0, (size_t)ntiles * sizeof(unsigned int), s));
+    return launch_check("lars_d_wb_settle");
+}
+
+extern "C" int lars_wb_predict_report(const void *scratch, int64_t ntiles, int64_t *confident, int64_t *missed)
+{
+    if (!scratch || ntiles <= 0 || !confident || !missed) return fail(LARS_ERR_INVALID, "lars_wb_predict_report: bad arguments");
+    ThreadCtx *c;
+    LARS_TRY(ensure_ctx(&c));
+    unsigned int head[4] = {0, 0, 0, 0};
+    LARS_HIP_TRY(hipMemcpyAsync(head, wb_predict_carve(const_cast<void *>(scratch), ntiles).head, sizeof(head), hipMemcpyDeviceToHost, c->stream));
+    LARS_HIP_TRY(hipStreamSynchronize(c->stream));
+    *confident = head[0];
+    *missed = head[1];
+    return LARS_OK;
+}
diff --git a/lars_image_processing_amd/csrc/wb_predict_device.h b/lars_image_processing_amd/csrc/wb_predict_device.h
--- /dev/null
+++ b/lars_image_processing_amd/csrc/wb_predict_device.h
@@ -0,0 +1,66 @@
+#pragma once
+#include "common.h"
+#include "device_common.h"
+
+namespace lars {
+
+__device__ inline void wb_mark_ranks(long long npix, int k, long long &lo, long long &hi, double &t)
+{
+    const double q = (k == 0 ? 2.0 : 98.0) / 100.0;
+    const double vi = (double)(npix - 1) * q;
+    const double fl = floor(vi);
+    lo = (long long)fl;
+    hi = lo + 1;
+    if (hi > npix - 1) hi = npix - 1;
+    t = vi - fl;
+}
+
+__device__ inline double wb_lerp(double a, double b, double t)
+{
+    const double d = b - a;
+    double r = a + d * t;
+    if (t >= 0.5) r = b - d * (1.0 - t);
+    return r;
+}
+
+__device__ inline bool wb_mark_exact(long long npix, int k, unsigned int lt, unsigned int le)
+{
+    long long lo, hi;
+    double t;
+    wb_mark_ranks(npix, k, lo, hi, t);
+    const long long top = t == 0.0 ? lo : hi;
+    return (long long)lt <= lo && (long long)le >= top + 1;
+}
+
+__device__ inline bool wb_tile_exact(long long npix, const unsigned int *counts)
+{
+    bool ok = true;
+    for (int c = 0; c < 3; ++c)
+        for (int k = 0; k < 2; ++k) ok = ok && wb_mark_exact(npix, k, counts[c * 4 + 2 * k], counts[c * 4 + 2 * k + 1]);
+    return ok;
+}
+
+__device__ inline bool wb_gate_open(const WbGate &g, long long npix, long long tile)
+{
+    if (!g.pred) return true;
+    const bool predicted = g.pred[tile] != 0u;
+    if (g.mode == WB_GATE_REFUSED) return !predicted;
+    if (g.mode == WB_GATE_PREDICTED) return predicted;
+    return predicted && !wb_tile_exact(npix, g.counts + tile * 12);
+}
+
+__device__ inline void wb_fill_table_u8(uint8_t *out, int tid, double p_lo, double p_hi, int rgn_variant)
+{
+    out[tid] = (uint8_t)wb_level(tid, p_lo, p_hi, rgn_variant);
+}
+
+__device__ inline void stats_open(StatsAccView *a, int k)
+{
+    a->sum_fx = 0; a->sumsq_fx = 0; a->count = 0; a->above = 0; a->nans = 0;
+    a->min_key = ~0ull; a->max_key = 0ull;
+    a->threshold = (k == LARS_NDWI) ? 0.0 : (double)0.2f;
+    a->index_id = (unsigned)k; a->reserved = 0;
+    for (int b = 0; b < LARS_HIST_BINS; ++b) a->hist[b] = 0;
+}
+
+}
```

Result: faster. 380,700, median of 6 (+5.7%).
